# csiro-robotics/syropod_highlevel_controller

Measured on AMD Instinct MI355X. Metric: control-cycles/sec (all legs IK-solved), higher is better.
Workload: dtype f64

## Files before the change

### syropod_highlevel_controller_amd/csrc/shc_cycle.hpp

```cpp
#pragma once

#include "../../include/shc_batch.h"
#include "shc_leg.hpp"

namespace shc {

enum : int { WS_STARTING = 0, WS_MOVING = 1, WS_STOPPING = 2, WS_STOPPED = 3 };
enum : int { SS_SWING = 0, SS_STANCE = 1, SS_FORCE_STANCE = 2, SS_FORCE_STOP = 3 };
enum : int { PS_POSING = 0, PS_STOP_POSING = 1, PS_POSING_COMPLETE = 2 };
enum : int { PM_NONE = 0, PM_SWING = 1, PM_STANCE = 2, PM_STOP = 3 };

constexpr int LW_ACP = 1 << 2, LW_CFS = 1 << 3, LW_PM_SHIFT = 4, LW_NEG = 1 << 6, LW_IKFAIL = 1 << 7, LW_PHASE_SHIFT = 8,
              LW_PHASE_MASK = 0xFFFFF, LW_ZBV = 1 << 28, LW_ATT = 1 << 29, LW_ROTDEF = 1 << 30,
              LW_TARGROT = int(1u << 31);
constexpr int RW_LACP_SHIFT = 2, RW_LCFS_SHIFT = 6, RW_RTDA = 1 << 10, RW_APS_SHIFT = 11;

constexpr int kMaxAutoPosers = 8;
constexpr int kSwingTable = 64;
enum : unsigned { DIRTY_WALK_PLANE = 1, DIRTY_MANUAL = 2, DIRTY_SWING_ORG = 4, DIRTY_STANCE_ORG = 8,
                  DIRTY_TARG_DIR = 16,
                  DIRTY_LAST = DIRTY_TARG_DIR };
enum : unsigned { RT_MANUAL_LIVE = 1, RT_TOUCHDOWN = 2, RT_EXTERNAL = 4, RT_MANUAL_LEGS = 8, RT_EFFORT_LIVE = 16, RT_SKIP_MARKED = 32, RT_POSE_MARKED = 64 };

enum : unsigned { F_MANUAL = 1, F_AUTO = 2, F_INCL = 4, F_IMU = 8, F_ADM = 16, F_TIPF = 32, F_ODOM = 64, F_DYN = 1u << 31,
                  F_ROT = 1u << 30,
                  F_ROUGH = 1u << 29,
                  F_TALIGN = 1u << 28,
                  F_MLEGS = 1u << 27,
                  F_TERRAIN = F_ROUGH | F_TALIGN | F_MLEGS };
template <int NJ, unsigned F>
constexpr bool rot_enabled() { return (F & F_ROT) != 0 && (NJ > 3 || (F & F_MLEGS) != 0); }

struct CycleParams {
  double dt;
  int32_t period, swing_period, stance_period, stance_end, swing_start, swing_end, stance_start;
  int32_t remap_old_period;
  int32_t swing_iterations;
  int32_t stance_iterations;
  double swing_delta_t;
  double inv_dt;
  double dt_over_swing_dt;
  double stance_dt;
  double stride_scale;
  double swing_height, swing_width, body_clearance;
  double swing_progress_scaler;
  int32_t swing_c_count;
  int32_t swing_c_valid;
  int32_t velocity_input_mode;
  int32_t manual_posing, auto_posing, inclination_posing, imu_posing, admittance_control, dynamic_stiffness, use_joint_effort;
  int32_t clamp_joint_positions, clamp_joint_velocities, force_normal_touchdown;
  int32_t tip_force;
  int32_t debug_skip;
  int32_t odometry;
  int32_t gravity_aligned;
  int32_t rough_terrain;
  int32_t tip_align;
  int32_t gravity_target;
  int32_t joint_control;
  double step_depth;
  double target_dir[3];
  double max_translation[3], max_rotation[3], max_translation_velocity, max_rotation_velocity;
  double pid_p, pid_i, pid_d;
  double adm_m00, adm_m01, adm_m10, adm_m11, adm_g0, adm_g1;
  double force_gain, virtual_stiffness, swing_stiffness_scaler, load_stiffness_scaler;
  double pose_force_gain, pose_swing_height;
  int32_t n_auto_posers, pose_phase_length, pose_sync, auto_pose_reference_leg;
  alignas(16) int32_t ap_start[kMaxAutoPosers];
  int32_t ap_end[kMaxAutoPosers];
  double ap_amp[kMaxAutoPosers][7];
};

template <int L, int NJ>
struct alignas(16) SharedConsts {
  LegConst<NJ> leg[L];
  alignas(16) double limit[9][4];
  double swing_c[kSwingTable];
  alignas(16) CycleParams P;
};

template <int NJ>
struct Fields {
  static constexpr int NJE = (NJ + 1) & ~1;
  static constexpr int Q = 0, QD = NJ, TIP = 2 * NJ, TVEL = TIP + 3, SORG = TVEL + 3, SVEL = SORG + 3, TORG = SVEL + 3,
                       DFLT = TORG + 3, TARG = DFLT + 3, STRD = TARG + 3,
                       CORE_END = STRD + 3,
                       ADM = CORE_END, ADM_END = ADM + 2,
                       TF = ADM_END, TF_END = TF + 4,
                       FORCE_IN = TF_END, EFFORT_IN = FORCE_IN + 4,
                       POSER_TIP = EFFORT_IN + NJE, MODEL_TIP = POSER_TIP + 4, ADM_DELTA = MODEL_TIP + 4,
                       ORG_DIR = ADM_DELTA + 4, CUR_DIR = ORG_DIR + 3,
                       TARG_DIR = CUR_DIR + 3,
                       DES_TIP = TARG_DIR + 4, DES_DIR = DES_TIP + 4,
                       SEQ_ORG = DES_DIR + 4, SEQ_DIR = SEQ_ORG + 4, SEQ_Q0 = SEQ_DIR + 4,
                       STEP_PLANE = SEQ_Q0 + NJE,
                       MEAS_Q = STEP_PLANE + 4, COUNT = MEAS_Q + NJE;
  static_assert(CORE_END % 2 == 0 && SORG % 2 == 0 && COUNT % 2 == 0, "field groups must align to 16-byte planes");
};
SHC_HD int64_t leg_field_index(int f, int64_t slot, int64_t n_slots) { return (int64_t(f >> 1) * n_slots + slot) * 2 + (f & 1); }
struct RobotFields {
  static constexpr int VLIN = 0, VANG = 2, PLANE = 3, PNORM = 6, PLANE_PREV = 9, PNORM_PREV = 12, OWPP = 15, VIN = 22, WIN = 24,
                       CORE_END = 25;
  static constexpr int MPOSE = 25, TVI = 32, RVI = 35, MANUAL_END = 38;
  static constexpr int ABSE = 38, VERR = 41, GYRO = 44, IMU_END = 47;
  static constexpr int IMUQ = 47, IMUQ_END = 51;
  static constexpr int APREV = 51, APREV_END = 55;
  static constexpr int CPOSE = 55, CPOSE_END = 62;
  static constexpr int WPP = 62, WPP_END = 69;
  static constexpr int ODOM = 69, ODOM_END = 73;
  static constexpr int INCL = 73, INCL_END = 75;
  static constexpr int TALIGN = 75, OTALIGN = 82, COUNT = 89;
  static constexpr int I_WORD = 0, I_APOSER = 1, I_POSE_PHASE = 2, I_RESET_MODE = 3, I_COUNT = 4;
};

struct ExtFields {
  static constexpr int T_POSE = 0, T_TRANSFORM = 7, T_CLEARANCE = 14, T_FLAGS = 15,
                       D_POSE = 16, D_TRANSFORM = 23, D_FLAGS = 30,
                       P_POSE = 32, P_TRANSFORM = 39, P_CLEARANCE = 46, P_FLAGS = 47, COUNT = 48;
};

enum : int { LS_WALKING = 0, LS_MANUAL = 1, LS_WALKING_TO_MANUAL = -1, LS_MANUAL_TO_WALKING = -2 };
struct ManualRobot {
  int32_t leg_state[SHC_MAX_LEGS];
  int32_t manual_leg_count, primary_leg, secondary_leg;
  int32_t skip_cycle;
  double primary_velocity[3], secondary_velocity[3];
  double primary_position[3], secondary_position[3];
};

struct DevState {
  double *legd;
  int32_t *legi;
  double *robd;
  int32_t *robi;
  int64_t n_slots, n_rob_pad, n_robots;
  double *ext;
  ManualRobot *manual;
  const double *span;
};

struct SpanTable {
  static constexpr int kPlanes = 14;
  static constexpr int kStride = 2 + 2 * kPlanes;
};
SHC_HD double set_precision3(double v) { return round_to_int(v * 1000.0) / 1000.0; }
SHC_HD double stance_span_change_y(const double *table, int leg, double default_shift_z) {
  const double *t = table + leg * SpanTable::kStride;
  const int n = int(t[0]);
  const double target = set_precision3(default_shift_z);
  int lower = -1, upper = -1;
  for (int k = 0; k < n; ++k) {
    const double h = t[2 + 2 * k];
    if (h > target && (upper < 0 || h < t[2 + 2 * upper])) upper = k;
    if (h <= target && (lower < 0 || h > t[2 + 2 * lower])) lower = k;
  }
  if (lower < 0 || upper < 0) return 0.0;
  const double uh = set_precision3(t[2 + 2 * upper]), lh = set_precision3(t[2 + 2 * lower]);
  const double i = (target - lh) / (uh - lh);
  const double radius = t[3 + 2 * lower] * (1.0 - i) + t[3 + 2 * upper] * i;
  return radius * t[1];
}

#if defined(__HIPCC__)

template <int L, int NJ, unsigned F>
constexpr bool phase_fences() {
#if defined(SHC_FENCE)
  return true;
#else
  constexpr bool exact = (F & (0x80000000u  | 0x40000000u )) == 0;
  constexpr bool octo_tipf = L == 8 && NJ == 5 && (F & 32u ) != 0 && (F & 16u ) == 0;
  return exact && ((NJ == 4 && (L == 4 || L == 8)) || octo_tipf);
#endif
}
#define SHC_PHASE_FENCE() do { if constexpr (phase_fences<L, NJ, F>()) __builtin_amdgcn_sched_barrier(0); } while (0)
#if defined(SHC_RES2_TIMING) && !defined(SHC_RES2_BUSY_ONLY)
__shared__ long long shc_ticks_lds[96];
__shared__ long long shc_acc_lds[96];
#define SHC_TICK(i) do { __builtin_amdgcn_sched_barrier(0); if (blockIdx.x == 1 && (threadIdx.x & 127) == 0) shc_ticks_lds[(threadIdx.x >> 7) * 32 + (i)] = __builtin_readcyclecounter(); __builtin_amdgcn_sched_barrier(0); } while (0)
#else
#define SHC_TICK(i) do {} while (0)
#endif
#ifdef SHC_ABLATE
#define SHC_DBG(P) ((P).debug_skip)
#else
#define SHC_DBG(P) 0
#endif
__device__ __forceinline__ int uni(int v) { return __builtin_amdgcn_readfirstlane(v); }

template <unsigned F>
struct Feat {
  __device__ __forceinline__ static bool manual(const CycleParams &P) { return (F & F_DYN) ? P.manual_posing != 0 : (F & F_MANUAL) != 0; }
  __device__ __forceinline__ static bool autop(const CycleParams &P) { return (F & F_DYN) ? P.auto_posing != 0 : (F & F_AUTO) != 0; }
  __device__ __forceinline__ static bool incl(const CycleParams &P) { return (F & F_DYN) ? P.inclination_posing != 0 : (F & F_INCL) != 0; }
  __device__ __forceinline__ static bool imu(const CycleParams &P) { return (F & F_DYN) ? P.imu_posing != 0 : (F & F_IMU) != 0; }
  __device__ __forceinline__ static bool adm(const CycleParams &P) { return (F & F_DYN) ? P.admittance_control != 0 : (F & F_ADM) != 0; }
  __device__ __forceinline__ static bool tipf(const CycleParams &P) { return (F & F_DYN) ? P.tip_force != 0 : (F & F_TIPF) != 0; }
  __device__ __forceinline__ static bool odom(const CycleParams &P) { return (F & F_DYN) ? P.odometry != 0 : (F & F_ODOM) != 0; }
};

template <int L>
struct Group {
  int base;
  __device__ __forceinline__ int get(int v, int j) const { return __shfl(v, base + j, 64); }
  __device__ __forceinline__ double get(double v, int j) const { return __shfl(v, base + j, 64); }
  __device__ __forceinline__ double sum(double v) const {
    double s = 0.0;
#pragma unroll
    for (int j = 0; j < L; ++j) s += get(v, j);
    return s;
  }
};

template <int RPW>
struct RobTile {
  double *d;
  int32_t *i;
  int grp;
  __device__ __forceinline__ double get(int f) const { return d[f * RPW + grp]; }
  __device__ __forceinline__ V3 get3(int f) const { return V3{d[f * RPW + grp], d[(f + 1) * RPW + grp], d[(f + 2) * RPW + grp]}; }
  __device__ __forceinline__ Quat getq(int f) const {
    return Quat{d[f * RPW + grp], d[(f + 1) * RPW + grp], d[(f + 2) * RPW + grp], d[(f + 3) * RPW + grp]};
  }
  __device__ __forceinline__ Pose getpose(int f) const { return Pose{get3(f), getq(f + 3)}; }
  __device__ __forceinline__ void put(int f, double v) const { d[f * RPW + grp] = v; }
  __device__ __forceinline__ void put3(int f, V3 v) const {
    d[f * RPW + grp] = v.x;
    d[(f + 1) * RPW + grp] = v.y;
    d[(f + 2) * RPW + grp] = v.z;
  }
  __device__ __forceinline__ void putq(int f, Quat q) const {
    d[f * RPW + grp] = q.w;
    d[(f + 1) * RPW + grp] = q.x;
    d[(f + 2) * RPW + grp] = q.y;
    d[(f + 3) * RPW + grp] = q.z;
  }
  __device__ __forceinline__ void putpose(int f, const Pose &p) const {
    put3(f, p.p);
    putq(f + 3, p.r);
  }
  __device__ __forceinline__ int geti(int f) const { return i[f * RPW + grp]; }
  __device__ __forceinline__ void puti(int f, int v) const { i[f * RPW + grp] = v; }
};

template <int NJ>
struct LegRegs {
  static constexpr bool kKeepJacobian = NJ <= 3;
  double q[NJ], qd[NJ];
  double sn[NJ], cs[NJ];
  V3 lin[NJ], pe;
  V3 tip, tvel, targ, strd;
  double adm0, adm1;
  double stiff;
  V3 tf, tipx;
  V3 org_dir, cur_dir, targ_dir;
  int word;
};

enum : int { PK_SORG = 0, PK_SVEL = 3, PK_TORG = 6, PK_DFLT = 9, PK_COUNT = 12 };
#ifndef SHC_PARK_REGS
struct Park {
  double *d;
  int lane;
  __device__ __forceinline__ V3 get3(int f) const { return V3{d[f * 64 + lane], d[(f + 1) * 64 + lane], d[(f + 2) * 64 + lane]}; }
  __device__ __forceinline__ void put3(int f, V3 v) const {
    d[f * 64 + lane] = v.x;
    d[(f + 1) * 64 + lane] = v.y;
    d[(f + 2) * 64 + lane] = v.z;
  }
  __device__ __forceinline__ double at(int k) const { return d[k * 64 + lane]; }
  __device__ __forceinline__ void set(int k, double v) const { d[k * 64 + lane] = v; }
};
#else
struct Park {
  double *d;
  int lane;
  mutable double r[12];
  __device__ __forceinline__ V3 get3(int f) const { return V3{r[f], r[f + 1], r[f + 2]}; }
  __device__ __forceinline__ void put3(int f, V3 v) const { r[f] = v.x, r[f + 1] = v.y, r[f + 2] = v.z; }
  __device__ __forceinline__ double at(int k) const { return r[k]; }
  __device__ __forceinline__ void set(int k, double v) const { r[k] = v; }
};
#endif

__device__ __forceinline__ V3 external_default(const double *ext, int64_t ns, uint32_t slot, V3 terrain_following) {
  if (ext == nullptr) return terrain_following;
  const double2 *X = reinterpret_cast<const double2 *>(ext);
  if ((int(X[(ExtFields::D_FLAGS / 2) * ns + slot].x) & 1) == 0) return terrain_following;
  double v[14];
#pragma unroll
  for (int k = 0; k < 7; ++k) {
    const double2 d = X[(ExtFields::D_POSE / 2 + k) * ns + slot];
    v[2 * k] = d.x, v[2 * k + 1] = d.y;
  }
  return V3{v[0], v[1], v[2]} + rotate(Quat{v[3], v[4], v[5], v[6]}, -V3{v[7], v[8], v[9]});
}

struct LegOut {
  V3 poser_tip, model_tip, adm_delta;
};

__device__ __forceinline__ double swing_progress_of(int word, const CycleParams &P) {
  int pm = (word >> LW_PM_SHIFT) & 3;
  if (pm != PM_SWING) return -1.0;
  int phase = (word >> LW_PHASE_SHIFT) & LW_PHASE_MASK;
  return clampd(double(phase - P.swing_start + 1) / double(P.swing_end - P.swing_start), 0.0, 1.0);
}

__device__ __forceinline__ int bearing_bracket(double y, double x) {
  if (x == 0.0 && y == 0.0) return 0;
  constexpr double kC = 0.99996192306417128874, kS = 0.0087265354983739347;
  double xr = kC * x - kS * y, yr = kS * x + kC * y;
  double ax = fabs(xr), ay = fabs(yr);
  bool upper = yr > 0.0 || (yr == 0.0 && xr > 0.0);
  if (upper) return xr > 0.0 ? (ay < ax ? 0 : 1) : (ay > ax ? 2 : 3);
  return xr < 0.0 ? (ay < ax ? 4 : 5) : (ay > ax ? 6 : 7);
}

template <int NJ>
struct LegInPlanes {
  const double *legd;
  int64_t ns;
  uint32_t slot;
  __device__ __forceinline__ V3 force() const {
    const double2 f01 = reinterpret_cast<const double2 *>(legd)[(Fields<NJ>::FORCE_IN / 2) * ns + slot];
    const double2 f2_ = reinterpret_cast<const double2 *>(legd)[(Fields<NJ>::FORCE_IN / 2 + 1) * ns + slot];
    return V3{f01.x, f01.y, f2_.x};
  }
  __device__ __forceinline__ void effort(double (&e)[NJ]) const {
#pragma unroll
    for (int i = 0; i < NJ; i += 2) {
      const double2 e2 = reinterpret_cast<const double2 *>(legd)[((Fields<NJ>::EFFORT_IN + i) / 2) * ns + slot];
      e[i] = e2.x;
      if (i + 1 < NJ) e[i + 1] = e2.y;
    }
  }
};
struct NoHook {
  __device__ __forceinline__ void operator()() const {}
};

struct UniFlags {
  int clamp_joint_velocities, clamp_joint_positions, swing_c_count;
  int velocity_input_mode, force_normal_touchdown;
};
__device__ __forceinline__ UniFlags load_uni_flags(const CycleParams &P) {
  const int c = P.clamp_joint_velocities, d = P.clamp_joint_positions, e = P.swing_c_count;
  const int f = P.velocity_input_mode, h = P.force_normal_touchdown;
  return UniFlags{uni(c), uni(d), uni(e), uni(f), uni(h)};
}

struct FrontToBack {
  V3 desired_dir;
  bool rot_def;
  int my_leg_state;
  bool plane_prev_changed;
  bool pose_only;
  V3 odom_vel;
  bool odom_run;
  bool joint_moved;
  V3 held_pe, held_dir;
  bool planes_in_sync = false;
  UniFlags uf;
  int limit_bracket = -1;
  double limit_value[4] = {0.0, 0.0, 0.0, 0.0};
};

struct OdomCache {
  double ha = 0.0, sh = 0.0, ch = 1.0;
  bool valid = false;
};
__device__ __forceinline__ void odometry_advance(double &ox, double &oy, double &ow, double &oz, const CycleParams &P, double vx, double vy, double vw,
                                                 OdomCache *cache = nullptr) {
  double sh, ch;
  const double ha = 0.5 * (vw * P.dt);
  if (cache != nullptr && cache->valid && __all(ha == cache->ha)) {
    sh = cache->sh, ch = cache->ch;
  } else {
    if (__all(fabs(ha) <= 0.5)) sincos_joint<false>(ha, &sh, &ch);
    else sincos_joint(ha, &sh, &ch);
    if (cache != nullptr) cache->ha = ha, cache->sh = sh, cache->ch = ch, cache->valid = true;
  }
  {
#pragma clang fp contract(off)
    const double a = vx * P.dt, b = vy * P.dt;
    double ux = -(oz * b), uy = oz * a;
    ux = ux + ux;
    uy = uy + uy;
    const double nx = ox + fma(-oz, uy, fma(ux, ow, a)), ny = oy + fma(oz, ux, fma(uy, ow, b));
    const double nw = fma(ow, ch, -(oz * sh)), nz = fma(ow, sh, oz * ch);
    ox = nx, oy = ny, ow = nw, oz = nz;
  }
}
template <int RPW>
__device__ __forceinline__ void odometry_step(const RobTile<RPW> &rb, const CycleParams &P, double vx, double vy, double vw, OdomCache *cache = nullptr) {
  using R = RobotFields;
  double ox = rb.get(R::ODOM), oy = rb.get(R::ODOM + 1), ow = rb.get(R::ODOM + 2), oz = rb.get(R::ODOM + 3);
  odometry_advance(ox, oy, ow, oz, P, vx, vy, vw, cache);
  rb.put(R::ODOM, ox);
  rb.put(R::ODOM + 1, oy);
  rb.put(R::ODOM + 2, ow);
  rb.put(R::ODOM + 3, oz);
}

template <int L, int NJ>
__device__ __forceinline__ double walk_plane_control_input(const int own_word, const SharedConsts<L, NJ> &C, const CycleParams &P, const Group<L> g,
                                                           const int swing_c_count_u) {
  double c = 0.0;
  bool sel = false;
  if (swing_c_count_u > 0) {
    const int it_own = min(max(((own_word >> LW_PHASE_SHIFT) & LW_PHASE_MASK) - P.swing_start, 0), P.swing_c_count - 1);
    const bool ok_own = ((own_word >> LW_PM_SHIFT) & 3) == PM_SWING && it_own < P.swing_c_valid;
    const unsigned legs_ok = unsigned((__ballot(ok_own) >> g.base) & ((1ull << L) - 1));
    sel = legs_ok != 0;
    const int last = sel ? 31 - __clz(int(legs_ok)) : 0;
    int it_sel = g.get(it_own, last);
    it_sel = sel ? it_sel : 0;
    if (__any(sel)) c = sel ? C.swing_c[it_sel] : 0.0;
  } else {
    double c_own = -1.0;
    const double sp = swing_progress_of(own_word, P) * P.swing_progress_scaler;
    if (sp >= 0 && sp <= 1.0) c_own = smooth_step(sp);
#pragma unroll
    for (int j = 0; j < L; ++j) {
      const double cj = g.get(c_own, j);
      if (cj >= 0.0) {
        c = cj;
        sel = true;
      }
    }
  }
  return sel ? c : -1.0;
}

template <int L, int NJ>
__device__ __forceinline__ double walk_plane_control_candidate(const int own_word, const SharedConsts<L, NJ> &C, const CycleParams &P, const int swing_c_count_u) {
  if (swing_c_count_u > 0) {
    const int it_own = min(max(((own_word >> LW_PHASE_SHIFT) & LW_PHASE_MASK) - P.swing_start, 0), P.swing_c_count - 1);
    const bool ok_own = ((own_word >> LW_PM_SHIFT) & 3) == PM_SWING && it_own < P.swing_c_valid;
    const double c = C.swing_c[it_own];
    return ok_own ? c : -1.0;
  }
  const double sp = swing_progress_of(own_word, P) * P.swing_progress_scaler;
  return (sp >= 0 && sp <= 1.0) ? smooth_step(sp) : -1.0;
}

template <int L>
__device__ __forceinline__ V3 quat_to_euler_zyx_grouped(Quat q, const Group<L> g, const int leg) {
  static_assert(L >= 3, "three lanes per robot");
  double tx = 2.0 * q.x, ty = 2.0 * q.y, tz = 2.0 * q.z;
  double twx = tx * q.w, twy = ty * q.w, twz = tz * q.w;
  double txx = tx * q.x, txy = ty * q.x, txz = tz * q.x;
  double tyy = ty * q.y, tyz = tz * q.y, tzz = tz * q.z;
  double m00 = 1.0 - (tyy + tzz), m01 = txy - twz, m02 = txz + twy;
  double m10 = txy + twz, m11 = 1.0 - (txx + tzz), m12 = tyz - twx;
  double m20 = txz - twy, m21 = tyz + twx, m22 = 1.0 - (txx + tyy);
  const double c2 = sqrt(m22 * m22 + m21 * m21);
  const bool neg = m10 < 0.0 || (m10 == 0.0 && __builtin_signbit(m10) && __builtin_signbit(m00));
  const bool second = leg == 1;
  const double t = atan2(second ? -m20 : m10, second ? (neg ? -c2 : c2) : m00);
  double r0 = g.get(t, 0), r1 = g.get(t, 1);
  if (__builtin_expect(__any((r0 < 0.0) != neg), 0)) r1 = atan2(-m20, r0 < 0.0 ? -c2 : c2);
  if (r0 < 0.0) r0 += kPi;
  double s1, c1;
  sincos_joint(r0, &s1, &c1);
  double r2 = atan2(s1 * m02 - c1 * m12, c1 * m11 - s1 * m01);
  if (fabs(r1) > kPi / 2 || fabs(r2) > kPi / 2) {
    r0 -= kPi;
    if (r1 > kPi / 2.0) r1 = -r1 + kPi;
    else if (r1 < kPi / 2.0) r1 = -r1 - kPi;
    if (r2 > kPi / 2.0) r2 -= kPi;
    else if (r2 < kPi / 2.0) r2 += kPi;
  }
  return V3{r2, r1, r0};
}
template <int L>
__device__ __forceinline__ Quat euler_to_quat_zyx_grouped(V3 e, const Group<L> g, const int leg) {
  static_assert(L >= 3, "three lanes per robot");
  double sn, cs;
  sincos_joint(0.5 * (leg == 0 ? e.x : (leg == 1 ? e.y : e.z)), &sn, &cs);
  const double sx = g.get(sn, 0), cx = g.get(cs, 0), sy = g.get(sn, 1), cy = g.get(cs, 1), sz = g.get(sn, 2), cz = g.get(cs, 2);
  Quat qx{cx, sx, 0, 0}, qy{cy, 0, sy, 0}, qz{cz, 0, 0, sz};
  return (qz * qy) * qx;
}

template <int L, int NJ, unsigned F, bool OWN_WORD = false>
__device__ __forceinline__ Pose cycle_pose(LegRegs<NJ> &s, const SharedConsts<L, NJ> &C, const CycleParams &P, const LegConst<NJ> &lc, const RobTile<64 / L> &rb,
                                           const Group<L> g, const int leg, const int (&lw)[L], int &rword, const int walk_state, unsigned &dirty, const bool manual_live,
                                           Pose &auto_pose, Pose &leg_auto, const V3 plane_prev, const V3 pnorm_prev, const int swing_c_count_u,
                                           const int own_word = 0, Pose *owpp_cache = nullptr, const double *c_given = nullptr) {
  static_assert(!OWN_WORD || ((F & (F_DYN | F_AUTO | F_TALIGN)) == 0), "the other legs' words are needed by auto posing and the tip-align pose");
  using R = RobotFields;
  using FT = Feat<F>;
  const V3 UZ{0, 0, 1};
  Pose cp;
  {
    Pose wpp;
    {
      double c = 0.0;
      bool sel = false;
      if constexpr (OWN_WORD) {
        const double ce = c_given != nullptr ? *c_given : walk_plane_control_input<L, NJ>(own_word, C, P, g, swing_c_count_u);
        sel = ce >= 0.0;
        c = sel ? ce : 0.0;
      } else if (swing_c_count_u > 0) {
        int it_sel = 0;
#pragma unroll
        for (int j = 0; j < L; ++j) {
          const int it = min(max(((lw[j] >> LW_PHASE_SHIFT) & LW_PHASE_MASK) - P.swing_start, 0), P.swing_c_count - 1);
          const bool ok = ((lw[j] >> LW_PM_SHIFT) & 3) == PM_SWING && it < P.swing_c_valid;
          it_sel = ok ? it : it_sel;
          sel = sel || ok;
        }
        if (__any(sel)) c = sel ? C.swing_c[it_sel] : 0.0;
      } else {
        double c_own = -1.0;
        {
          double sp = swing_progress_of(s.word, P) * P.swing_progress_scaler;
          if (sp >= 0 && sp <= 1.0) c_own = smooth_step(sp);
        }
#pragma unroll
        for (int j = 0; j < L; ++j) {
          double cj = g.get(c_own, j);
          if (cj >= 0.0) {
            c = cj;
            sel = true;
          }
        }
      }
      V3 wplane = sel ? plane_prev : V3{0, 0, 0};
      V3 wnorm = sel ? pnorm_prev : UZ;
      Pose owpp = owpp_cache != nullptr ? *owpp_cache : rb.getpose(R::OWPP);
      bool flat = wnorm.x == 0.0 && wnorm.y == 0.0 && wnorm.z == 1.0 && owpp.r.w == 1.0 && owpp.r.x == 0.0 && owpp.r.y == 0.0 &&
                  owpp.r.z == 0.0;
      if (__builtin_expect(__all(flat), 1)) {
        double s0 = 1.0 - c;
        V3 npp{0.0, 0.0, P.body_clearance + wplane.z};
        wpp.p = npp * c + owpp.p * s0;
        wpp.r = Quat{s0 * 1.0 + c * 1.0, s0 * 0.0 + c * 0.0, s0 * 0.0 + c * 0.0, s0 * 0.0 + c * 0.0};
      } else {
        Pose np;
        np.r = correct_rotation(from_two_vectors(UZ, wnorm), quat_identity());
        np.p = rotate(np.r, V3{0, 0, P.body_clearance});
        np.p.z += wplane.z;
        wpp = interpolate_pose(owpp, c, np);
      }
      if (c == 1.0) {
        const bool same = wpp.p.x == owpp.p.x && wpp.p.y == owpp.p.y && wpp.p.z == owpp.p.z && wpp.r.w == owpp.r.w && wpp.r.x == owpp.r.x &&
                          wpp.r.y == owpp.r.y && wpp.r.z == owpp.r.z;
        if (__any(!same)) {
          rb.putpose(R::OWPP, wpp);
          if (owpp_cache != nullptr) *owpp_cache = wpp;
          dirty |= DIRTY_WALK_PLANE;
        }
      }
      rb.putpose(R::WPP, wpp);
    }
    cp = wpp;
    Quat manual_r = quat_identity();
    if (FT::manual(P) && manual_live) {
      V3 tvi_in = rb.get3(R::TVI), rvi_in = rb.get3(R::RVI);
      int reset_mode = rb.geti(R::I_RESET_MODE);
      bool idle = reset_mode == 0 && tvi_in.x == 0.0 && tvi_in.y == 0.0 && tvi_in.z == 0.0 && rvi_in.x == 0.0 && rvi_in.y == 0.0 &&
                  rvi_in.z == 0.0;
      Pose mpose = rb.getpose(R::MPOSE);
      if (__any(!idle)) {
        if (!idle) {
          if (reset_mode == 5) {
            mpose = pose_identity();
          } else {
            double cpos[3] = {mpose.p.x, mpose.p.y, mpose.p.z};
            V3 ce = quat_to_euler(mpose.r, true);
            double crot[3] = {ce.x, ce.y, ce.z};
            double tvi[3] = {tvi_in.x, tvi_in.y, tvi_in.z}, rvi[3] = {rvi_in.x, rvi_in.y, rvi_in.z};
            bool rt[3] = {false, false, false}, rr[3] = {false, false, false};
            switch (reset_mode) {
              case 1: rt[2] = true; rr[2] = true; break;
              case 2: rt[0] = true; rt[1] = true; break;
              case 3: rr[0] = true; rr[1] = true; break;
              case 4: rt[0] = rt[1] = rt[2] = true; rr[0] = rr[1] = rr[2] = true; break;
              default: break;
            }
            double dpos[3], drot[3];
#pragma unroll
            for (int i = 0; i < 3; ++i) {
#pragma clang fp contract(off)
              if (rt[i]) {
                double diff = cpos[i] - 0.0;
                if (diff < 0) tvi[i] = 1.0; else if (diff > 0) tvi[i] = -1.0;
              }
              if (rr[i]) {
                double diff = crot[i] - 0.0;
                if (diff < 0) rvi[i] = 1.0; else if (diff > 0) rvi[i] = -1.0;
              }
              double tv = tvi[i] * P.max_translation_velocity;
              double rv = rvi[i] * P.max_rotation_velocity;
              double dp = cpos[i] + tv * P.dt;
              double dr = crot[i] + rv * P.dt;
              double tl = signd(tv) * P.max_translation[i];
              if (rt[i] && 0.0 < P.max_translation[i] && 0.0 > -P.max_translation[i]) tl = 0.0;
              bool ptv = signd(tv) > 0;
              if ((ptv && dp > tl) || (!ptv && dp < tl)) tv = (tl - cpos[i]) / P.dt;
              double rl = signd(rv) * P.max_rotation[i];
              if (rr[i] && 0.0 < P.max_rotation[i] && 0.0 > -P.max_rotation[i]) rl = 0.0;
              bool prv = signd(rv) > 0;
              if ((prv && dr > rl) || (!prv && dr < rl)) rv = (rl - crot[i]) / P.dt;
              dpos[i] = cpos[i] + tv * P.dt;
              drot[i] = crot[i] + rv * P.dt;
            }
            rb.put3(R::TVI, V3{tvi[0], tvi[1], tvi[2]});
            rb.put3(R::RVI, V3{rvi[0], rvi[1], rvi[2]});
            mpose.p = V3{dpos[0], dpos[1], dpos[2]};
            mpose.r = correct_rotation(euler_to_quat(V3{drot[0], drot[1], drot[2]}, true), quat_identity());
          }
          rb.putpose(R::MPOSE, mpose);
        }
        dirty |= DIRTY_MANUAL;
      }
      manual_r = mpose.r;
      bool unposed = mpose.p.x == 0.0 && mpose.p.y == 0.0 && mpose.p.z == 0.0 && mpose.r.w == 1.0 && mpose.r.x == 0.0 &&
                     mpose.r.y == 0.0 && mpose.r.z == 0.0;
      if (!__all(unposed)) cp = add_pose(cp, mpose);
    }
    if (FT::incl(P)) {
      Quat aprev = FT::autop(P) ? rb.getq(R::APREV) : quat_identity();
      Quat comb = normalized(manual_r * aprev);
      Quat removed = normalized(rb.getq(R::IMUQ) * inverse(comb));
      V3 e = quat_to_euler(removed, false);
      double lon = clampd(-P.body_clearance * tan(e.y), -P.max_translation[0], P.max_translation[0]);
      double lat = clampd(P.body_clearance * tan(e.x), -P.max_translation[1], P.max_translation[1]);
      cp = add_pose(cp, Pose{V3{lon, lat, 0.0}, quat_identity()});
      if ((F & F_MLEGS) != 0) {
        rb.put(R::INCL, lon);
        rb.put(R::INCL + 1, lat);
      }
    }
    if (FT::imu(P)) {
      Quat cur = correct_rotation(rb.getq(R::IMUQ), quat_identity());
      Quat tgt = correct_rotation(manual_r, quat_identity());
#ifdef SHC_POSE_R5
      Quat err = normalized(cur * inverse(tgt));
#else
      const double tgt_n2 = dot(tgt, tgt);
      Quat err = normalized(cur * (__all(tgt_n2 == 1.0) ? conj(tgt) : inverse(tgt)));
#endif
#ifdef SHC_POSE_R5
      V3 pe = quat_to_euler(err, false);
#else
      V3 pe = quat_to_euler_zyx_grouped<L>(err, g, leg);
#endif
      pe.z = 0.0;
      V3 abse = rb.get3(R::ABSE) + pe * P.dt;
      V3 verr = (-rb.get3(R::GYRO)) * 0.15 + rb.get3(R::VERR) * (1 - 0.15);
      rb.put3(R::ABSE, abse);
      rb.put3(R::VERR, verr);
      V3 corr = -(verr * P.pid_d + pe * P.pid_p + abse * P.pid_i);
      corr.x = clampd(corr.x, -P.max_rotation[0], P.max_rotation[0]);
      corr.y = clampd(corr.y, -P.max_rotation[1], P.max_rotation[1]);
      bool tgt_identity = tgt.w == 1.0 && tgt.x == 0.0 && tgt.y == 0.0 && tgt.z == 0.0;
      corr.z = 0.0;
      if (__any(!tgt_identity)) {
        if (!tgt_identity) corr.z = quat_to_euler(tgt, false).z;
      }
#ifdef SHC_POSE_R5
      Quat ir = correct_rotation(euler_to_quat(corr, false), tgt);
#else
      Quat ir = correct_rotation(euler_to_quat_zyx_grouped<L>(corr, g, leg), tgt);
#endif
      cp = add_pose(cp, Pose{V3{0, 0, 0}, ir});
    } else if (FT::autop(P)) {
      int ref = lw[P.auto_pose_reference_leg];
      bool zbv = (ref & LW_ZBV) != 0;
      int aps = (rword >> RW_APS_SHIFT) & 3;
      if (walk_state == WS_STARTING || walk_state == WS_MOVING) aps = PS_POSING;
      else if ((zbv && walk_state == WS_STOPPING) || walk_state == WS_STOPPED) aps = PS_STOP_POSING;
      int master_phase;
      if (P.pose_sync) {
        master_phase = (ref >> LW_PHASE_SHIFT) & LW_PHASE_MASK;
        rb.puti(R::I_POSE_PHASE, master_phase);
      } else {
        master_phase = rb.geti(R::I_POSE_PHASE);
        rb.puti(R::I_POSE_PHASE, (master_phase + 1) % P.pose_phase_length);
      }
      int aposer = rb.geti(R::I_APOSER);
      int complete = 0;
      for (int i = 0; i < P.n_auto_posers; ++i) {
        int fl = (aposer >> (4 * i)) & 15;
        bool start_check = fl & 1, end1 = fl & 2, end2 = fl & 4, allow = fl & 8;
        int phase = master_phase, sp = P.ap_start[i], ep = P.ap_end[i];
        if (sp > ep) {
          ep += P.pose_phase_length;
          if (phase < sp) phase += P.pose_phase_length;
        }
        start_check = !P.pose_sync || (!start_check && aps == PS_POSING && phase == sp);
        end1 = end1 || (aps == PS_STOP_POSING && phase == sp);
        end2 = end2 || (aps == PS_STOP_POSING && phase == ep && end1);
        if (!allow && start_check) {
          allow = true;
          end1 = end2 = false;
        } else if (allow && P.pose_sync && end1 && end2) {
          allow = false;
          start_check = false;
        }
        aposer = (aposer & ~(15 << (4 * i))) | ((int(start_check) | int(end1) << 1 | int(end2) << 2 | int(allow) << 3) << (4 * i));
        complete += allow ? 0 : 1;
        if (phase >= sp && phase < ep && allow) {
          int iteration = phase - sp + 1, num = ep - sp;
          bool first_half = iteration <= num / 2;
          double delta_t = 1.0 / (num / 2.0);
          int offset = int(first_half ? 0 : num / 2.0);
          double t = (iteration - offset) * delta_t;
          double u = 1.0 - t;
          double wgt = first_half ? (4.0 * t * t * t * u + t * t * t * t) : (u * u * u * u + 4.0 * t * u * u * u);
          V3 pos;
          if (P.ap_amp[i][3] != 0.0) {
            V3 e = quat_to_euler(rb.getq(R::IMUQ), false);
            V3 gv{0, 0, kGravity};
            gv = rotate(angle_axis_y(-e.y), gv);
            gv = rotate(angle_axis_x(-e.x), gv);
            pos = normalized(gv) * (P.ap_amp[i][3] * wgt);
          } else {
            pos = V3{P.ap_amp[i][0] * wgt, P.ap_amp[i][1] * wgt, P.ap_amp[i][2] * wgt};
          }
          V3 rot{P.ap_amp[i][4] * wgt, P.ap_amp[i][5] * wgt, P.ap_amp[i][6] * wgt};
          auto_pose = add_pose(auto_pose, Pose{pos, euler_to_quat(rot, false)});
        }
      }
      rb.puti(R::I_APOSER, aposer);
      if (complete == P.n_auto_posers) aps = PS_POSING_COMPLETE;
      rword = (rword & ~(3 << RW_APS_SHIFT)) | (aps << RW_APS_SHIFT);
      {
        int sp = lc.neg_start, ep = lc.neg_end, np = master_phase;
        if (sp > ep) {
          ep += P.pose_phase_length;
          if (np < sp) np += P.pose_phase_length;
        }
        int st = s.word & 3;
        bool neg = (s.word & LW_NEG) != 0;
        if (st != SS_FORCE_STANCE && st != SS_FORCE_STOP && np == sp) neg = true;
        if (np < sp || np > ep) neg = false;
        s.word = neg ? (s.word | LW_NEG) : (s.word & ~LW_NEG);
        leg_auto = auto_pose;
        if (neg) {
          int iteration = np - sp + 1, num = ep - sp;
          bool first_half = iteration <= num / 2;
          double ci = 1.0;
          if (lc.neg_ratio > 0.0) {
            if (first_half) ci = fmin(1.0, iteration / (num * lc.neg_ratio));
            else ci = fmin(1.0, (num - iteration) / (num * lc.neg_ratio));
          }
          ci = smooth_step(ci);
          Pose negation = interpolate_pose(pose_identity(), ci, auto_pose);
          leg_auto = remove_pose(auto_pose, negation);
        }
      }
      cp = add_pose(cp, auto_pose);
      if (FT::incl(P)) rb.putq(R::APREV, auto_pose.r);
    }
    if ((F & F_TALIGN) != 0 && uni(P.tip_align)) {
      Chain<NJ> ch0;
      chain_from_sincos<NJ>(lc, s.sn, s.cs, ch0);
      V3 last_joint = ch0.p[NJ - 1];
      if constexpr (NJ > 3) {
#pragma unroll
        for (int k = NJ - 2; k >= 2; --k) last_joint = lc.jactive[k + 1] != 0.0 ? last_joint : ch0.p[k];
      }
      const V3 t2j_own = base_rotate(lc, last_joint - ch0.pe);
      Pose ta = rb.getpose(R::TALIGN), ota = rb.getpose(R::OTALIGN);
      const V3 n = pnorm_prev;
      const Quat wrot = from_two_vectors(UZ, n);
#pragma unroll
      for (int j = 0; j < L; ++j) {
        const V3 t2j{g.get(t2j_own.x, j), g.get(t2j_own.y, j), g.get(t2j_own.z, j)};
        const double sp = swing_progress_of(lw[j], P);
        if (sp != -1.0) {
          const double link_length = norm(-t2j);
          V3 a = rotate(wrot, t2j), b = n * link_length;
          const V3 to_alignment = -(a - b * (dot(a, b) / dot(b, b)));
          a = ta.p;
          b = n;
          V3 target = (a - b * (dot(a, b) / dot(b, b))) + to_alignment;
          target.x = clampd(target.x, -P.max_translation[0], P.max_translation[1]);
          target.y = clampd(target.y, -P.max_translation[1], P.max_translation[1]);
          target.z = clampd(target.z, -P.max_translation[2], P.max_translation[1]);
          double c = smooth_step(sp);
          if (sp < 0.5) {
            c = smooth_step(c * 2.0);
            ta = interpolate_pose(ota, c, pose_identity());
          } else {
            c = smooth_step((c - 0.5) * 2.0);
            ta = interpolate_pose(pose_identity(), c, Pose{target, quat_identity()});
          }
          if (sp == 1.0) ota = ta;
        }
      }
      rb.putpose(R::TALIGN, ta);
      rb.putpose(R::OTALIGN, ota);
      cp = add_pose(cp, ta);
    }
    rb.putpose(R::CPOSE, cp);
  }
  return cp;
}

template <int NJ, typename IN>
__device__ __forceinline__ void cycle_admittance(LegRegs<NJ> &s, LegOut &out, const CycleParams &P, const IN &in) {
  const V3 force_in = in.force();
  V3 f = (P.use_joint_effort ? s.tf : force_in) * P.pose_force_gain;
  double fi[3] = {f.x, f.y, f.z}, d[3];
#pragma unroll
  for (int i = 0; i < 3; ++i) {
    double u = fmax(fi[i], 0.0);
    double x0 = P.adm_m00 * s.adm0 + P.adm_m01 * s.adm1 + P.adm_g0 * u;
    double x1 = P.adm_m10 * s.adm0 + P.adm_m11 * s.adm1 + P.adm_g1 * u;
    s.adm0 = x0;
    s.adm1 = x1;
    d[i] = clampd(-x0, -0.2, 0.2);
  }
  out.adm_delta = projection(V3{d[0], d[1], d[2]}, s.tipx);
}

template <int L, int NJ, unsigned F, bool ADM_HERE, typename IN, bool ODOM_HERE = true, bool POSE_HERE = true, typename POSEWAIT = NoHook>
__device__ __forceinline__ void cycle_front(LegRegs<NJ> &s, LegOut &out, const SharedConsts<L, NJ> &C, const RobTile<64 / L> &rb, const Park &pk,
                                            const Group<L> g, int leg, const double *__restrict__ legd, int64_t ns, uint32_t slot, unsigned &dirty,
                                            const bool manual_live, const bool touchdown_detection, double *ext, const ManualRobot *mr, const IN &in,
                                            FrontToBack &fb, const double *span = nullptr, const POSEWAIT &pose_wait = POSEWAIT()) {
  using R = RobotFields;
  using FT = Feat<F>;
  static_assert(POSE_HERE || ((F & F_DYN) == 0 && (F & F_AUTO) == 0 && (F & F_TERRAIN) == 0), "the pose can run elsewhere only without auto posing / terrain paths");
  int zero = 0;
  asm volatile("" : "+v"(zero));
  const CycleParams &P = (&C.P)[zero];
  const LegConst<NJ> &lc = C.leg[leg + zero];
  const V3 UZ{0, 0, 1};
  constexpr bool rot_on = rot_enabled<NJ, F>();
  constexpr bool rot_walk = rot_on && NJ > 3;
  bool rot_def = (s.word & LW_ROTDEF) != 0;
  bool targ_rot = (s.word & LW_TARGROT) != 0;
  fb.odom_run = false;
  fb.plane_prev_changed = false;
  fb.joint_moved = false;
  SHC_TICK(2);

  int rword = rb.geti(R::I_WORD);
  int walk_state = rword & 3;
  const double vin_x = rb.get(R::VIN), vin_y = rb.get(R::VIN + 1), win = rb.get(R::WIN);
  bool may_stop = walk_state == WS_STOPPING;
  if (walk_state == WS_MOVING) {
    const double ax = fabs(vin_x), ay = fabs(vin_y), aw = win;
    may_stop = !(aw != 0.0 || ax > 1e-100 || ay > 1e-100);
  }
  s.word &= ~(LW_ZBV | LW_ATT);
  if (!(SHC_DBG(P) & 128) && __any(may_stop)) {
    int w = s.word;
    if (dot(s.strd, s.strd) == 0.0) w |= LW_ZBV;
    const V3 pnp = rb.get3(R::PNORM_PREV);
    V3 err = s.tip - s.targ;
    if (__all(pnp.x == 0.0 && pnp.y == 0.0 && pnp.z == 1.0)) err.z = 0.0;
    else err = rejection(err, pnp);
    if (dot(err, err) < kTipTolerance * kTipTolerance) w |= LW_ATT;
    s.word = w;
  }
  int lw[L];
  const bool lw_early = POSE_HERE || uni(FT::adm(P) ? 1 : 0) != 0;
  if (lw_early) {
#pragma unroll
    for (int j = 0; j < L; ++j) lw[j] = g.get(s.word, j);
  } else {
#pragma unroll
    for (int j = 0; j < L; ++j) lw[j] = 0;
  }

  SHC_PHASE_FENCE();
  SHC_TICK(3);
  int my_leg_state = LS_WALKING;
  bool frozen = false;
  if ((F & F_MLEGS) != 0 && mr != nullptr) {
    my_leg_state = mr->leg_state[leg];
#pragma unroll
    for (int j = 0; j < L; ++j) frozen = frozen || g.get(my_leg_state, j) != LS_WALKING;
  }

  Pose cp;
  Pose auto_pose = pose_identity();
  Pose leg_auto = pose_identity();
  if (POSE_HERE && !(SHC_DBG(P) & 1)) {
    cp = cycle_pose<L, NJ, F>(s, C, P, lc, rb, g, leg, lw, rword, walk_state, dirty, manual_live, auto_pose, leg_auto, rb.get3(R::PLANE_PREV), rb.get3(R::PNORM_PREV),
                              fb.uf.swing_c_count);
  } else if (POSE_HERE) {
    cp = rb.getpose(R::CPOSE);
  }
  SHC_PHASE_FENCE();
  SHC_TICK(4);
  int pose_state = (rword >> RW_APS_SHIFT) & 3;

  out.adm_delta = V3{0, 0, 0};
  if (FT::adm(P)) {
    if (uni(P.dynamic_stiffness) && walk_state != WS_STOPPED) {
      const bool swing = (s.word & 3) == SS_SWING;
      const double k = P.virtual_stiffness;
      const double ref = fabs((s.tip.z - pk.get3(PK_DFLT).z) / P.pose_swing_height);
      const double load = swing ? k * (ref * (P.load_stiffness_scaler - 1)) : 0.0;
      double v = swing ? k * (ref * (P.swing_stiffness_scaler - 1) + 1) : k;
      const int lo = leg == 0 ? L - 1 : leg - 1, hi = leg == L - 1 ? 0 : leg + 1;
#pragma unroll
      for (int i = 0; i < L; ++i) {
        const double li = g.get(load, i);
        const bool si = (lw[i] & 3) == SS_SWING;
        if (si && (i == lo || i == hi) && (!swing || i > leg)) v += li;
      }
      s.stiff = v;
    }
    if (ADM_HERE) cycle_admittance<NJ>(s, out, P, in);
  }
  if ((F & F_MLEGS) != 0 && fb.pose_only) {
    rb.puti(R::I_WORD, rword);
    return;
  }

  SHC_PHASE_FENCE();
  double lim[4] = {0.05, 0.3, 0.02, 0.1};
  if (!(SHC_DBG(P) & 2)) {
    double sx = vin_x + win * (-s.tip.y), sy = vin_y + win * s.tip.x;
    int idx = bearing_bracket(sy, sx);
    if (__all(idx == fb.limit_bracket)) {
#pragma unroll
      for (int k = 0; k < 4; ++k) lim[k] = fb.limit_value[k];
    } else {
#pragma unroll
      for (int k = 0; k < 4; ++k) lim[k] = kUnassigned;
#pragma unroll
      for (int j = 0; j < L; ++j) {
        int ij = g.get(idx, j);
#pragma unroll
        for (int k = 0; k < 4; ++k) lim[k] = fmin(lim[k], C.limit[ij][k]);
      }
      fb.limit_bracket = idx;
#pragma unroll
      for (int k = 0; k < 4; ++k) fb.limit_value[k] = lim[k];
    }
  }
  SHC_PHASE_FENCE();
  SHC_TICK(5);
  double vx = rb.get(R::VLIN), vy = rb.get(R::VLIN + 1), vw = rb.get(R::VANG);
  const double lin_n2 = vin_x * vin_x + vin_y * vin_y;
  double lin_norm;
  const int velocity_input_mode = fb.uf.velocity_input_mode;
  if (velocity_input_mode == 0 && __all(lin_n2 <= 1.0)) lin_norm = lin_n2 != 0.0 ? 0.5 : 0.0;
  else lin_norm = sqrt(lin_n2);
  if (!(SHC_DBG(P) & 32)) {
    double nvx, nvy, nw;
    if (velocity_input_mode == 0) {
      double k = 1.0;
      if (__any(lin_norm > 1.0)) k = lin_norm > 1.0 ? 1.0 / lin_norm : 1.0;
      const double cx = lin_norm > 1.0 ? vin_x * k : vin_x, cy = lin_norm > 1.0 ? vin_y * k : vin_y;
      nw = clampd(win, -1.0, 1.0) * lim[1];
      const double sc = 1.0 - fabs(win);
      nvx = (cx * lim[0]) * sc;
      nvy = (cy * lim[0]) * sc;
    } else {
      const bool over = lin_norm > lim[0];
      const double k = lim[0] / lin_norm;
      const double cx = over ? vin_x * k : vin_x, cy = over ? vin_y * k : vin_y;
      nw = clampd(win, -lim[1], lim[1]);
      const double sc = lim[1] != 0.0 ? (1.0 - fabs(nw / lim[1])) : 0.0;
      nvx = cx * sc;
      nvy = cy * sc;
    }
    if (walk_state == WS_STOPPING) nvx = nvy = nw = 0.0;
    if (frozen) nvx = vx, nvy = vy, nw = vw;
    const double ax = nvx - vx, ay = nvy - vy;
    const double an2 = ax * ax + ay * ay;
    const double an = __all(an2 == 0.0) ? 0.0 : sqrt(an2);
    const double cap = lim[2] * P.dt;
    if (__all(an < cap)) {
      vx += ax;
      vy += ay;
    } else {
      const double inv = an2 > 0.0 ? an : 1.0;
      const double sx_ = (ax / inv) * lim[2] * P.dt, sy_ = (ay / inv) * lim[2] * P.dt;
      vx += an < cap ? ax : sx_;
      vy += an < cap ? ay : sy_;
    }
    const double aa = nw - vw;
    vw += fabs(aa) < lim[3] * P.dt ? aa : signd(aa) * lim[3] * P.dt;
    rb.put(R::VLIN, vx);
    rb.put(R::VLIN + 1, vy);
    rb.put(R::VANG, vw);
  }
  const bool has_cmd = (lin_norm != 0.0) || (win != 0.0);

  SHC_PHASE_FENCE();
  SHC_TICK(6);
  if constexpr ((F & F_DYN) != 0) {
    const int remap_from = uni(P.remap_old_period);
    if (remap_from > 0) {
      if (walk_state == WS_MOVING) {
        int ph = (s.word >> LW_PHASE_SHIFT) & LW_PHASE_MASK, st = s.word & 3;
        const double step_progress = double(ph) / double(remap_from);
        ph = int(step_progress * double(P.period));
        if (st != SS_FORCE_STOP) {
          if (ph >= P.swing_start && ph < P.swing_end && st != SS_FORCE_STANCE) st = SS_SWING;
          else if (ph < P.stance_end || ph >= P.stance_start) st = SS_STANCE;
        }
        s.word = (s.word & ~(3 | (LW_PHASE_MASK << LW_PHASE_SHIFT))) | st | (ph << LW_PHASE_SHIFT);
      }
      if (lw_early) {
#pragma unroll
        for (int j = 0; j < L; ++j) lw[j] = g.get(s.word, j);
      }
    }
  }
  int lacp = (rword >> RW_LACP_SHIFT) & 15, lcfs = (rword >> RW_LCFS_SHIFT) & 15;
  bool rtda = (rword & RW_RTDA) != 0;
  bool early_return = false;
  int my_state = s.word & 3, my_phase = (s.word >> LW_PHASE_SHIFT) & LW_PHASE_MASK;
  bool my_acp = (s.word & LW_ACP) != 0, my_cfs = (s.word & LW_CFS) != 0;
  bool my_update_default = false;
  bool any_stepping = false;
  const bool steady = __all(!frozen && walk_state == WS_MOVING && has_cmd) && !(SHC_DBG(P) & 16384);
  if (steady) {
    my_acp = false;
    any_stepping = ((__ballot((s.word & 3) != SS_FORCE_STOP) >> g.base) & ((1ull << L) - 1)) != 0;
  } else if (SHC_DBG(P) & 16384) {
    my_acp = false;
    any_stepping = true;
  } else if (frozen) {
    early_return = true;
  } else if (walk_state == WS_STOPPED && has_cmd) {
    walk_state = WS_STARTING;
    my_acp = false;
    my_cfs = false;
    my_phase = lc.phase_offset;
    my_state = SS_STANCE;
    if (my_phase >= P.swing_start && my_phase < P.swing_end) my_state = SS_SWING;
    early_return = true;
  } else {
    if (walk_state == WS_STARTING && lacp == L && lcfs == L) {
      lacp = 0;
      lcfs = 0;
      walk_state = WS_MOVING;
    } else if (walk_state == WS_MOVING && !has_cmd) {
      walk_state = WS_STOPPING;
    } else if (walk_state == WS_STOPPING && lacp == L && pose_state == PS_POSING_COMPLETE) {
      lacp = 0;
      walk_state = WS_STOPPED;
    }
    if (__all(walk_state == WS_MOVING)) {
      my_acp = false;
      any_stepping = ((__ballot((s.word & 3) != SS_FORCE_STOP) >> g.base) & ((1ull << L) - 1)) != 0;
    } else {
    if (!lw_early) {
#pragma unroll
      for (int j = 0; j < L; ++j) lw[j] = g.get(s.word, j);
    }
#pragma unroll
    for (int j = 0; j < L; ++j) {
      int wj = lw[j];
      int st = wj & 3, ph = (wj >> LW_PHASE_SHIFT) & LW_PHASE_MASK;
      bool acp = (wj & LW_ACP) != 0, cfs = (wj & LW_CFS) != 0, upd = false;
      if (walk_state == WS_STARTING) {
        if (lacp == L) {
          if (ph == P.swing_end && !cfs) {
            cfs = true;
            lcfs++;
          }
        }
        if (!acp) {
          if (C.leg[j].starts_in_swing && ph != P.swing_end) {
            st = SS_FORCE_STANCE;
          } else {
            lacp++;
            acp = true;
          }
        }
      } else if (walk_state == WS_MOVING) {
        acp = false;
      } else if (walk_state == WS_STOPPING) {
        if ((wj & LW_ZBV) && !acp && ph == P.swing_end) {
          if ((wj & LW_ATT) || rtda) {
            rtda = false;
            upd = true;
            st = SS_FORCE_STOP;
            acp = true;
            lacp++;
          } else {
            rtda = true;
          }
        }
      } else {
        st = SS_FORCE_STOP;
        ph = 0;
      }
      any_stepping = any_stepping || (st != SS_FORCE_STOP);
      if (j == leg) {
        my_state = st;
        my_phase = ph;
        my_acp = acp;
        my_cfs = cfs;
        my_update_default = upd;
      }
    }
    }
  }
  if (POSE_HERE || !steady) {
    rword = (rword & ~(3 | (15 << RW_LACP_SHIFT) | (15 << RW_LCFS_SHIFT) | RW_RTDA)) | walk_state | (lacp << RW_LACP_SHIFT) |
            (lcfs << RW_LCFS_SHIFT) | (rtda ? RW_RTDA : 0);
    rb.puti(R::I_WORD, rword);
  }
  SHC_TICK(7);
  int my_pm = (s.word >> LW_PM_SHIFT) & 3;
  SHC_PHASE_FENCE();

  if (!early_return) {
    bool default_changed = false;
    if (__any(my_update_default)) {
      if (my_update_default) {
        if (!POSE_HERE) pose_wait();
        Pose wpp = rb.getpose(R::WPP);
        const double span_y = ((F & F_ROUGH) != 0 && span != nullptr) ? stance_span_change_y(span, leg, pk.get3(PK_DFLT).z) : lc.span_shift;
        V3 idp = transform_vector(wpp, V3{lc.stance_x, lc.stance_y + span_y, 0.0});
        V3 proj = projection(pk.get3(PK_TORG) - idp, rb.get3(R::PNORM_PREV));
        pk.put3(PK_DFLT, external_default(ext, ns, slot, idp + proj));
        default_changed = true;
        dirty |= DIRTY_STANCE_ORG;
      }
    }
    bool standard = (my_state == SS_SWING) || my_cfs;
    int msp = standard ? P.stance_period : lc.first_stance_period;
    int stance_iter = standard ? P.stance_iterations : lc.first_stance_iterations;
    int mss = standard ? P.stance_start : lc.phase_offset;
    double stance_dt = standard ? P.stance_dt : lc.first_stance_dt;
    (void)stance_iter;
    const V3 dflt = pk.get3(PK_DFLT);
    s.targ = dflt + s.strd * 0.5;
    bool stepping = my_state != SS_FORCE_STOP;
    const bool rough = (F & F_ROUGH) != 0 && uni(P.rough_terrain) != 0;
    bool rough_update_default = false;
    V3 model_tip_prev{0, 0, 0};
    if (rough) {
      if (LegRegs<NJ>::kKeepJacobian) {
        model_tip_prev = tip_robot_frame(lc, s.pe);
      } else {
        Chain<NJ> ch0;
        chain_from_sincos<NJ>(lc, s.sn, s.cs, ch0);
        model_tip_prev = tip_robot_frame(lc, ch0.pe);
      }
    }
    const int force_normal_touchdown = fb.uf.force_normal_touchdown;
#ifdef SHC_NO_STRAIGHT
    const bool straight = false;
#else
    const bool straight = (F & F_ROUGH) == 0 && !(SHC_DBG(P) & 4) && force_normal_touchdown == 0;
#endif
    if (straight) {
      const V3 sorg_p = pk.get3(PK_SORG), svel_p = pk.get3(PK_SVEL), torg_p = pk.get3(PK_TORG);
      const bool swing = my_state == SS_SWING;
      const bool step_sw = stepping && swing, step_st = stepping && !swing;
      const V3 sv{vx - vw * s.tip.y, vy + vw * s.tip.x, 0.0};
      const V3 strd_new = scaled(sv, P.stride_scale);
      s.strd = sel3(stepping, strd_new, s.strd);
      V3 pn = rb.get3(R::PNORM);
      const bool flat_n = pn.x == 0.0 && pn.y == 0.0 && pn.z == 1.0;
      if (!__all(flat_n)) pn = normalized(pn);
      const V3 clearance = scaled(pn, P.swing_height);
      const int it_sw = my_phase - P.swing_start + 1;
      const bool first_half = it_sw <= P.swing_iterations / 2;
      const bool first_sw = step_sw && it_sw == 1;
      const V3 sorg = sel3(first_sw, s.tip, sorg_p), svel = sel3(first_sw, s.tvel, svel_p);
      pk.put3(PK_SORG, sorg);
      pk.put3(PK_SVEL, svel);
      dirty |= first_sw ? unsigned(DIRTY_SWING_ORG) : 0u;
      V3 mid{(sorg.x + s.targ.x) / 2.0, (sorg.y + s.targ.y) / 2.0, fmax(sorg.z, s.targ.z)};
      mid = mid + clearance;
      mid.y += (lc.stance_y > 0.0) ? P.swing_width : -P.swing_width;
      const V3 sep1 = scaled(svel * 0.25, P.dt_over_swing_dt);
      const V3 n1_0 = sorg, n1_1 = sorg + sep1, n1_2 = sorg + scaled(sep1, 2.0);
      const V3 n1_3{(mid.x + n1_2.x) / 2.0, (mid.y + n1_2.y) / 2.0, mid.z};
      const V3 n1_4 = mid;
      const V3 fv = scaled(-s.strd, stance_dt * P.inv_dt);
      const V3 sep2 = scaled(fv * 0.25, P.dt_over_swing_dt);
      const V3 n2_0 = n1_4, n2_1 = n1_4 - (n1_3 - n1_4), n2_2 = s.targ - scaled(sep2, 2.0), n2_3 = s.targ - sep2, n2_4 = s.targ;
      const double t_sw = first_half ? P.swing_delta_t * it_sw : P.swing_delta_t * (it_sw - P.swing_iterations / 2);
      const V3 b0 = sel3(first_half, n1_0, n2_0), b1 = sel3(first_half, n1_1, n2_1), b2 = sel3(first_half, n1_2, n2_2), b3 = sel3(first_half, n1_3, n2_3),
               b4 = sel3(first_half, n1_4, n2_4);
      const V3 dpos_sw = scaled(quartic_bezier_dot(b0, b1, b2, b3, b4, t_sw), P.swing_delta_t);
      int it_st = my_phase + (P.period - mss);
      if (it_st >= P.period) it_st -= P.period;
      if (it_st < 0 || it_st >= P.period) it_st = mod_i(it_st, P.period);
      it_st += 1;
      const bool first_st = step_st && it_st == 1;
      const V3 torg = sel3(first_st, s.tip, torg_p);
      pk.put3(PK_TORG, torg);
      dirty |= first_st ? unsigned(DIRTY_STANCE_ORG) : 0u;
      const double stride_scaler = standard ? 1.0 : lc.first_stride_scaler;
      const V3 sep = scaled((-s.strd) * stride_scaler, 0.25);
      const double t_st = it_st * stance_dt;
      const V3 dpos_st = scaled(quartic_bezier_dot(torg, torg + sep, torg + scaled(sep, 2.0), torg + scaled(sep, 3.0), torg + scaled(sep, 4.0), t_st), stance_dt);
      const V3 dpos = sel3(swing, dpos_sw, dpos_st);
      const V3 tip_new = s.tip + dpos, tvel_new = dpos * P.inv_dt;
      s.tip = sel3(stepping, tip_new, s.tip);
      s.tvel = sel3(stepping, tvel_new, s.tvel);
    } else if (stepping && !(SHC_DBG(P) & 4)) {
      V3 sv{vx - vw * s.tip.y, vy + vw * s.tip.x, 0.0};
      s.strd = scaled(sv, P.stride_scale);
      V3 pn = rb.get3(R::PNORM);
      bool flat_n = pn.x == 0.0 && pn.y == 0.0 && pn.z == 1.0;
      if (!__all(flat_n)) pn = normalized(pn);
      V3 clearance = scaled(pn, P.swing_height);
      V3 dpos;
      if (my_state == SS_SWING) {
        int iteration = my_phase - P.swing_start + 1;
        bool first_half = iteration <= P.swing_iterations / 2;
        V3 sorg, svel;
        if (iteration == 1) {
          sorg = s.tip;
          svel = s.tvel;
          pk.put3(PK_SORG, sorg);
          pk.put3(PK_SVEL, svel);
          dirty |= DIRTY_SWING_ORG;
          rough_update_default = rough;
        } else {
          sorg = pk.get3(PK_SORG);
          svel = pk.get3(PK_SVEL);
        }
        bool ground_contact = false;
        if (rough) {
          const double2 sp01 = reinterpret_cast<const double2 *>(legd)[(Fields<NJ>::STEP_PLANE / 2) * ns + slot];
          const double2 sp23 = reinterpret_cast<const double2 *>(legd)[(Fields<NJ>::STEP_PLANE / 2 + 1) * ns + slot];
          ground_contact = sp23.y != 0.0;
          bool external = false;
          if (ext != nullptr) {
            const double2 *X = reinterpret_cast<const double2 *>(ext);
            const double2 cf = X[(ExtFields::T_CLEARANCE / 2) * ns + slot];
            const int flags = int(cf.y);
            external = (flags & 1) != 0;
            if (external) {
              double v[14];
#pragma unroll
              for (int k = 0; k < 7; ++k) {
                const double2 d = X[(ExtFields::T_POSE / 2 + k) * ns + slot];
                v[2 * k] = d.x, v[2 * k + 1] = d.y;
              }
              s.targ = V3{v[0], v[1], v[2]} + rotate(Quat{v[3], v[4], v[5], v[6]}, -V3{v[7], v[8], v[9]});
              if (rot_walk) {
                const Quat tr = Quat{v[3], v[4], v[5], v[6]} * inverse(Quat{v[10], v[11], v[12], v[13]});
                targ_rot = !(tr.w == 0.0 && tr.x == 0.0 && tr.y == 0.0 && tr.z == 0.0);
                if (targ_rot) s.targ_dir = rotate(tr, V3{1, 0, 0}), dirty |= DIRTY_TARG_DIR;
              }
              clearance = normalized(clearance) * cf.x;
              if (flags & 2) {
                const double time_to_swing_end = (P.swing_iterations - iteration) * P.dt;
                s.targ = s.targ - V3{vx, vy, 0.0} * time_to_swing_end;
              }
            }
          }
          if (external) {
          } else if (touchdown_detection) {
            if (ground_contact) {
              const V3 step_plane_position = V3{sp01.x, sp01.y, sp23.x} - model_tip_prev;
              const V3 difference = (s.tip + step_plane_position) - s.targ;
              s.targ = s.targ + projection(difference, rb.get3(R::PNORM));
            } else {
              s.targ.z -= P.step_depth;
            }
          }
        }
        V3 mid{(sorg.x + s.targ.x) / 2.0, (sorg.y + s.targ.y) / 2.0, fmax(sorg.z, s.targ.z)};
        mid = mid + clearance;
        mid.y += (lc.stance_y > 0.0) ? P.swing_width : -P.swing_width;
        V3 sep1 = scaled(svel * 0.25, P.dt_over_swing_dt);
        V3 n1_0 = sorg, n1_1 = sorg + sep1, n1_2 = sorg + scaled(sep1, 2.0);
        V3 n1_3{(mid.x + n1_2.x) / 2.0, (mid.y + n1_2.y) / 2.0, mid.z};
        V3 n1_4 = mid;
        V3 fv = scaled(-s.strd, stance_dt * P.inv_dt);
        V3 sep2 = scaled(fv * 0.25, P.dt_over_swing_dt);
        V3 n2_0 = n1_4, n2_1 = n1_4 - (n1_3 - n1_4), n2_2 = s.targ - scaled(sep2, 2.0), n2_3 = s.targ - sep2, n2_4 = s.targ;
        if (rough && ground_contact && !first_half) {
          n2_0 = s.tip, n2_1 = s.tip + sep2, n2_2 = s.tip + scaled(sep2, 2.0), n2_3 = s.tip + scaled(sep2, 3.0), n2_4 = s.tip + scaled(sep2, 4.0);
        }
        if (force_normal_touchdown && !(rough && ground_contact)) {
          V3 bo = s.targ - scaled(sep2, 4.0);
          bo.z = fmax(sorg.z, s.targ.z);
          bo = bo + clearance;
          n1_4 = bo;
          n2_0 = bo;
          n2_2 = s.targ - scaled(sep2, 2.0);
          V3 half = scaled(n2_2 - bo, 0.5);
          n1_3 = n2_0 - half;
          n2_1 = n2_0 + half;
        }
        if (first_half) {
          double t = P.swing_delta_t * iteration;
          dpos = scaled(quartic_bezier_dot(n1_0, n1_1, n1_2, n1_3, n1_4, t), P.swing_delta_t);
        } else {
          double t = P.swing_delta_t * (iteration - P.swing_iterations / 2);
          dpos = scaled(quartic_bezier_dot(n2_0, n2_1, n2_2, n2_3, n2_4, t), P.swing_delta_t);
        }
      } else {
        int iteration = my_phase + (P.period - mss);
        if (iteration >= P.period) iteration -= P.period;
        if (iteration < 0 || iteration >= P.period) iteration = mod_i(iteration, P.period);
        iteration += 1;
        V3 torg;
        if (iteration == 1) {
          torg = s.tip;
          pk.put3(PK_TORG, torg);
          dirty |= DIRTY_STANCE_ORG;
          rough_update_default = rough;
          if (ext != nullptr) {
            double &flags = ext[((ExtFields::T_CLEARANCE / 2) * ns + slot) * 2 + 1];
            flags = double(int(flags) & ~1);
          }
        } else {
          torg = pk.get3(PK_TORG);
        }
        double stride_scaler = standard ? 1.0 : lc.first_stride_scaler;
        (void)msp;
        V3 sep = scaled((-s.strd) * stride_scaler, 0.25);
        double t = iteration * stance_dt;
        dpos = scaled(quartic_bezier_dot(torg, torg + sep, torg + scaled(sep, 2.0), torg + scaled(sep, 3.0), torg + scaled(sep, 4.0), t), stance_dt);
      }
      s.tip = s.tip + dpos;
      s.tvel = dpos * P.inv_dt;
      if (rough && __any(rough_update_default)) {
        if (rough_update_default) {
          if (!POSE_HERE) pose_wait();
          Pose wpp = rb.getpose(R::WPP);
          const double span_y = span != nullptr ? stance_span_change_y(span, leg, pk.get3(PK_DFLT).z) : 0.0;
          V3 idp = transform_vector(wpp, V3{lc.stance_x, lc.stance_y + span_y, 0.0});
          V3 proj = projection(pk.get3(PK_TORG) - idp, rb.get3(R::PNORM));
          V3 new_default = external_default(ext, ns, slot, idp + proj);
          pk.put3(PK_DFLT, new_default);
          default_changed = true;
          dirty |= DIRTY_STANCE_ORG;
        }
      }
    }
    SHC_TICK(16);
    if (rot_on) {
      const int pm0 = (s.word >> LW_PM_SHIFT) & 3;
      const double sp = swing_progress_of(s.word, P);
      bool more_than_3_joints = NJ > 3;
      if constexpr (NJ > 3) more_than_3_joints = lc.jactive[3] != 0.0;
      if (rot_walk && more_than_3_joints && (pm0 == PM_STANCE || pm0 == PM_STOP || sp >= 0.5)) {
        if (uni(P.gravity_target) && !targ_rot) {
          V3 gv{0, 0, kGravity};
          if (FT::imu(P) || FT::incl(P) || FT::autop(P)) {
            const V3 e = quat_to_euler(rb.getq(R::IMUQ), false);
            gv = rotate(angle_axis_y(-e.y), gv);
            gv = rotate(angle_axis_x(-e.x), gv);
          }
          s.targ_dir = normalized(gv);
          dirty |= DIRTY_TARG_DIR;
          targ_rot = true;
        }
        if (!targ_rot) {
          rot_def = false;
        } else {
          s.cur_dir = s.targ_dir;
          if (sp >= 0.5) {
            const double c = smooth_step(fmin(1.0, 2.0 * (sp - 0.5)));
            s.cur_dir = normalized(lerp3(s.org_dir, s.targ_dir, c));
          }
          rot_def = true;
        }
      } else {
        s.org_dir = s.tipx;
        rot_def = false;
      }
    }
    my_phase = my_phase + 1 == P.period ? 0 : my_phase + 1;
    if (my_phase > P.period) my_phase = my_phase % P.period;
    if (my_state != SS_FORCE_STOP) {
      if (my_phase >= P.swing_start && my_phase < P.swing_end && my_state != SS_FORCE_STANCE) my_state = SS_SWING;
      else if (my_phase < P.stance_end || my_phase >= P.stance_start) my_state = SS_STANCE;
    }
    if (my_state == SS_SWING) my_pm = PM_SWING;
    else if (my_state == SS_STANCE) my_pm = PM_STANCE;
    else if (my_state == SS_FORCE_STOP) my_pm = PM_STOP;
    if (!fb.planes_in_sync) {
      const V3 pl = rb.get3(R::PLANE), pn_ = rb.get3(R::PNORM), plp = rb.get3(R::PLANE_PREV), pnp_ = rb.get3(R::PNORM_PREV);
      const bool same = pl.x == plp.x && pl.y == plp.y && pl.z == plp.z && pn_.x == pnp_.x && pn_.y == pnp_.y && pn_.z == pnp_.z;
      if (any_stepping) {
        if (__any(!same)) {
          rb.put3(R::PLANE_PREV, pl);
          rb.put3(R::PNORM_PREV, pn_);
          dirty |= DIRTY_WALK_PLANE;
          fb.plane_prev_changed = true;
        }
      }
      fb.planes_in_sync = __all(same || any_stepping);
    }
    if (__any(default_changed)) {
      fb.planes_in_sync = false;
      dirty |= DIRTY_WALK_PLANE;
      const V3 nd = pk.get3(PK_DFLT);
      double x = nd.x, y = nd.y, z = nd.z;
      double sxx = g.sum(x * x), sxy = g.sum(x * y), sx = g.sum(x), syy = g.sum(y * y), sy = g.sum(y);
      double sxz = g.sum(x * z), syz = g.sum(y * z), sz = g.sum(z);
      double a00 = sxx, a01 = sxy, a02 = sx, a11 = syy, a12 = sy, a22 = double(L);
      double c00 = a11 * a22 - a12 * a12, c01 = a02 * a12 - a01 * a22, c02 = a01 * a12 - a02 * a11;
      double c11 = a00 * a22 - a02 * a02, c12 = a01 * a02 - a00 * a12, c22 = a00 * a11 - a01 * a01;
      double det = a00 * c00 + a01 * c01 + a02 * c02;
      double pa = (c00 * sxz + c01 * syz + c02 * sz) / det;
      double pb = (c01 * sxz + c11 * syz + c12 * sz) / det;
      double pc = (c02 * sxz + c12 * syz + c22 * sz) / det;
      rb.put3(R::PLANE, V3{pa, pb, pc});
      rb.put3(R::PNORM, normalized(V3{-pa, -pb, 1.0}));
    }
    if (FT::odom(P) && !(SHC_DBG(P) & 1024)) {
      if (ODOM_HERE) odometry_step(rb, P, vx, vy, vw);
      fb.odom_vel = V3{vx, vy, vw};
      fb.odom_run = true;
    }
  }
  if ((F & F_MLEGS) != 0 && mr != nullptr && my_leg_state == LS_MANUAL) {
    const bool primary = leg == mr->primary_leg, secondary = !primary && leg == mr->secondary_leg;
    V3 vin{0, 0, 0}, pin{0, 0, 0};
    if (primary) {
      vin = V3{mr->primary_velocity[0], mr->primary_velocity[1], mr->primary_velocity[2]};
      pin = V3{mr->primary_position[0], mr->primary_position[1], mr->primary_position[2]};
    } else if (secondary) {
      vin = V3{mr->secondary_velocity[0], mr->secondary_velocity[1], mr->secondary_velocity[2]};
      pin = V3{mr->secondary_position[0], mr->secondary_position[1], mr->secondary_position[2]};
    }
    if (norm(vin) != 0.0 && uni(P.joint_control) != 0) {
      bool three_joints = NJ == 3;
      if constexpr (NJ > 3) three_joints = lc.jactive[3] == 0.0;
      if constexpr (rot_on) if (three_joints) {
        Chain<NJ> ch;
        chain_from_sincos<NJ>(lc, s.sn, s.cs, ch);
        fb.joint_moved = true;
        fb.held_pe = ch.pe;
        fb.held_dir = s.tipx;
        s.q[0] += vin.y * P.max_rotation_velocity * P.dt;
        s.q[2] += vin.x * P.max_rotation_velocity * P.dt;
        joint_sincos<NJ>(lc, s.q, s.sn, s.cs);
        chain_from_sincos<NJ>(lc, s.sn, s.cs, ch);
        s.tip = tip_robot_frame(lc, ch.pe);
        s.cur_dir = base_rotate(lc, ch.xe);
        rot_def = true;
      }
    } else if (norm(vin) != 0.0) {
      V3 prev_tip;
      if (LegRegs<NJ>::kKeepJacobian) {
        prev_tip = tip_robot_frame(lc, s.pe);
      } else {
        Chain<NJ> ch0;
        chain_from_sincos<NJ>(lc, s.sn, s.cs, ch0);
        prev_tip = tip_robot_frame(lc, ch0.pe);
      }
      const double2 d01 = reinterpret_cast<const double2 *>(legd)[(Fields<NJ>::DES_TIP / 2) * ns + slot];
      const double2 d23 = reinterpret_cast<const double2 *>(legd)[(Fields<NJ>::DES_TIP / 2 + 1) * ns + slot];
      const V3 ik_error = V3{d01.x, d01.y, d23.x} - prev_tip;
      V3 change = vin * (P.max_translation_velocity * P.dt);
      if (norm(ik_error) >= kIkTolerance) change = (-normalized(ik_error)) * norm(change);
      s.tip = s.tip + change;
      rot_def = false;
    }
    if (norm(pin) != 0.0 && uni(P.joint_control) == 0) {
      s.tip = pin;
      rot_def = false;
    }
  }
  s.word = (s.word & ~(3 | LW_ACP | LW_CFS | (3 << LW_PM_SHIFT) | (LW_PHASE_MASK << LW_PHASE_SHIFT) | LW_ZBV | LW_ATT | LW_IKFAIL | LW_ROTDEF | LW_TARGROT)) |
           my_state | (my_acp ? LW_ACP : 0) | (my_cfs ? LW_CFS : 0) | (my_pm << LW_PM_SHIFT) | (my_phase << LW_PHASE_SHIFT) |
           (rot_def ? LW_ROTDEF : 0) | (targ_rot ? LW_TARGROT : 0);

  SHC_PHASE_FENCE();
  SHC_TICK(8);
  V3 desired_dir{1, 0, 0};
  {
    if (!POSE_HERE && !(SHC_DBG(P) & 32768)) {
      pose_wait();
      SHC_TICK(17);
      cp = rb.getpose(R::CPOSE);
    } else if (!POSE_HERE) {
      cp = pose_identity();
    }
    Pose bp = cp;
    if (FT::autop(P) && !FT::imu(P)) {
      bp = remove_pose(bp, auto_pose);
      bp = add_pose(bp, leg_auto);
    }
    out.poser_tip = (SHC_DBG(P) & 256) ? s.tip : inverse_transform_vector(bp, s.tip);
    if ((F & F_MLEGS) != 0 && (my_leg_state == LS_MANUAL || my_leg_state == LS_WALKING_TO_MANUAL)) out.poser_tip = s.tip;
    if (rot_on && rot_def) desired_dir = rotate(inverse(bp.r), s.cur_dir);
    if (rot_on && rot_def && (F & F_MLEGS) != 0 && (my_leg_state == LS_MANUAL || my_leg_state == LS_WALKING_TO_MANUAL)) desired_dir = s.cur_dir;
  }

  fb.desired_dir = desired_dir;
  fb.rot_def = rot_def;
  fb.my_leg_state = my_leg_state;
  SHC_PHASE_FENCE();
  SHC_TICK(15);
}

template <int L, int NJ, unsigned F, typename IN>
__device__ __forceinline__ void cycle_back(LegRegs<NJ> &s, LegOut &out, const SharedConsts<L, NJ> &C, int leg, const double *__restrict__ legd, int64_t ns,
                                           uint32_t slot, const ManualRobot *mr, const IN &in, const FrontToBack &fb) {
  using FT = Feat<F>;
  int zero = 0;
  asm volatile("" : "+v"(zero));
  const CycleParams &P = (&C.P)[zero];
  const LegConst<NJ> &lc = C.leg[leg + zero];
  constexpr bool rot_on = rot_enabled<NJ, F>();
  const V3 desired_dir = fb.desired_dir;
  const bool rot_def = fb.rot_def;
  const int my_leg_state = fb.my_leg_state;
  {
    SHC_TICK(9);
    V3 desired = out.poser_tip + out.adm_delta;
    if ((F & F_MLEGS) != 0 && (my_leg_state == LS_MANUAL || my_leg_state == LS_WALKING_TO_MANUAL))
      desired = out.poser_tip;
    if ((F & F_MLEGS) != 0 && mr != nullptr) {
      double *dd = const_cast<double *>(legd);
      reinterpret_cast<double2 *>(dd)[(Fields<NJ>::DES_TIP / 2) * ns + slot] = double2{desired.x, desired.y};
      dd[((Fields<NJ>::DES_TIP / 2 + 1) * ns + slot) * 2] = desired.z;
    }
    Chain<NJ> chain;
    bool retried = false;
    if (rot_on) {
      const bool cv = fb.uf.clamp_joint_velocities != 0, cp_ = fb.uf.clamp_joint_positions != 0;
      chain_from_sincos<NJ>(lc, s.sn, s.cs, chain);
      V3 current_dir = chain.xe;
      double dq[NJ];
      V3 lin[NJ];
      if ((F & F_MLEGS) != 0 && fb.joint_moved) {
        current_dir = base_rotate_inv(lc, fb.held_dir);
        jacobian_columns<NJ>(chain, lin);
        ik_step_cols<NJ>(lc, lin, fb.held_pe, s.q, s.qd, desired, dq);
      } else {
        ik_step<NJ>(lc, chain, s.q, s.qd, desired, dq);
      }
      if (rot_def) {
        update_joints<NJ>(lc, dq, P.dt, P.inv_dt, false, cp_, s.q, s.qd);
        joint_sincos<NJ>(lc, s.q, s.sn, s.cs);
        chain_from_sincos<NJ>(lc, s.sn, s.cs, chain);
        jacobian_columns<NJ>(chain, lin);
        ik_step_rotation<NJ>(lc, chain, lin, s.q, s.qd, tip_rotation_delta(current_dir, base_rotate_inv(lc, desired_dir)), dq);
      }
      double success = update_joints<NJ>(lc, dq, P.dt, P.inv_dt, cv, cp_, s.q, s.qd);
      joint_sincos<NJ>(lc, s.q, s.sn, s.cs);
      chain_from_sincos<NJ>(lc, s.sn, s.cs, chain);
      {
        V3 e = tip_robot_frame(lc, chain.pe) - desired;
        if (fabs(e.x) > kIkTolerance || fabs(e.y) > kIkTolerance || fabs(e.z) > kIkTolerance) {
          success = 0.0;
          s.word |= LW_IKFAIL;
        }
      }
      if (rot_def && success == 0.0) {
        retried = true;
        ik_step<NJ>(lc, chain, s.q, s.qd, desired, dq);
        update_joints<NJ>(lc, dq, P.dt, P.inv_dt, cv, cp_, s.q, s.qd);
        joint_sincos<NJ>(lc, s.q, s.sn, s.cs);
      }
    } else if (!(SHC_DBG(P) & 8)) {
      double dq[NJ];
      if (LegRegs<NJ>::kKeepJacobian) {
        ik_step_cols<NJ>(lc, s.lin, s.pe, s.q, s.qd, desired, dq);
      } else {
        chain_from_sincos<NJ>(lc, s.sn, s.cs, chain);
        ik_step<NJ>(lc, chain, s.q, s.qd, desired, dq);
      }
      update_joints<NJ>(lc, dq, P.dt, P.inv_dt, fb.uf.clamp_joint_velocities != 0, fb.uf.clamp_joint_positions != 0, s.q, s.qd);
    }
    SHC_PHASE_FENCE();
    SHC_TICK(10);
    if (!(SHC_DBG(P) & 16) && !rot_on) joint_sincos<NJ>(lc, s.q, s.sn, s.cs);
    if (!(SHC_DBG(P) & 512)) chain_from_sincos<NJ>(lc, s.sn, s.cs, chain);
    V3 lin[NJ];
    jacobian_columns<NJ>(chain, lin);
    if (LegRegs<NJ>::kKeepJacobian) {
#pragma unroll
      for (int i = 0; i < NJ; ++i) s.lin[i] = lin[i];
      s.pe = chain.pe;
    }
    SHC_PHASE_FENCE();
    SHC_TICK(11);
    out.model_tip = (SHC_DBG(P) & 512) ? desired : tip_robot_frame(lc, chain.pe);
    if (FT::adm(P) || rot_on) s.tipx = base_rotate(lc, chain.xe);
    V3 e = out.model_tip - desired;
    if (fabs(e.x) > kIkTolerance || fabs(e.y) > kIkTolerance || fabs(e.z) > kIkTolerance) s.word |= LW_IKFAIL;
    if (FT::tipf(P) && !(SHC_DBG(P) & 8192)) {
      double effort[NJ];
      in.effort(effort);
      V3 raw = tip_force_cols<NJ>(lc, chain, lin, effort);
      if constexpr (rot_on) {
        const double gk = 0.15 * P.force_gain;
        s.tf = V3{fma(raw.x, gk, s.tf.x * (1 - 0.15)), fma(raw.y, gk, s.tf.y * (1 - 0.15)), fma(raw.z, gk, s.tf.z * (1 - 0.15))};
        if (retried) s.tf = V3{fma(raw.x, gk, s.tf.x * (1 - 0.15)), fma(raw.y, gk, s.tf.y * (1 - 0.15)), fma(raw.z, gk, s.tf.z * (1 - 0.15))};
      } else {
        s.tf = raw * (0.15 * P.force_gain) + s.tf * (1 - 0.15);
      }
    }
  }
  SHC_TICK(12);
}

template <int L, int NJ, unsigned F, typename IN = LegInPlanes<NJ>, typename MID = NoHook>
__device__ __forceinline__ void cycle(LegRegs<NJ> &s, LegOut &out, const SharedConsts<L, NJ> &C, const RobTile<64 / L> &rb, const Park &pk,
                                      const Group<L> g, int leg, const double *__restrict__ legd, int64_t ns, uint32_t slot, unsigned &dirty,
                                      const bool manual_live, const bool touchdown_detection, double *ext, const ManualRobot *mr, const IN &in,
                                      const MID &mid = MID(), const double *span = nullptr, const bool pose_only = false) {
  FrontToBack fb;
  fb.planes_in_sync = false;
  fb.limit_bracket = -1;
  fb.uf = load_uni_flags(C.P);
  fb.pose_only = pose_only;
  cycle_front<L, NJ, F, true>(s, out, C, rb, pk, g, leg, legd, ns, slot, dirty, manual_live, touchdown_detection, ext, mr, in, fb, span);
  if ((F & F_MLEGS) != 0 && pose_only) return;
  mid();
  cycle_back<L, NJ, F>(s, out, C, leg, legd, ns, slot, mr, in, fb);
}

#endif

}
```

### syropod_highlevel_controller_amd/csrc/shc_cycle_kernel.hpp

```cpp
#pragma once

#include "shc_cycle.hpp"
#include "shc_cycle_launch.hpp"

#include <hip/hip_runtime.h>

#include <type_traits>

namespace shc {

#ifndef SHC_WAVES_PER_SIMD
#define SHC_WAVES_PER_SIMD 2
#endif
#ifndef SHC_ROT_WAVES_PER_SIMD
#define SHC_ROT_WAVES_PER_SIMD 1
#endif
#ifndef SHC_TERRAIN_WAVES_PER_SIMD
#define SHC_TERRAIN_WAVES_PER_SIMD 2
#endif

struct LegPlanes {
  double2 *base;
  int64_t ns;
  uint32_t slot;
// ... 628 lines not shown
        }
      }
      if ((++iter & 1023) == 0 && lane == 0) st_sys(&A.host->heartbeat, iter);
    }
    if (leave) break;
    __builtin_amdgcn_s_sleep(1);
  }
}

template <int L, int NJ, unsigned F, bool RES, int HALF = ROLE_ALL, bool BATCH = false>
__device__ __forceinline__ void cycle_wave(const DevState &st, const SharedConsts<L, NJ> *gc, int n_cycles, unsigned rt_flags, const int64_t wave,
                                           const ResidentArgs *ra) {
  static_assert(HALF == ROLE_ALL || (!RES && (F & (F_DYN | F_TERRAIN | F_MLEGS | F_AUTO)) == 0), "half-step launches: feature-exact kernels without auto posing / terrain paths");
  using R = RobotFields;
  using FT = Feat<F>;
  constexpr int RPW = 64 / L;
  __shared__ SharedConsts<L, NJ> C;
  extern __shared__ double wave_lds[];
  constexpr int kWaveDoubles = R::COUNT * RPW + PK_COUNT * 64 + (R::I_COUNT * RPW + 1) / 2;
  SHC_TICK(0);
  const bool manual_live = (rt_flags & RT_MANUAL_LIVE) != 0;
  const bool touchdown_detection = (rt_flags & RT_TOUCHDOWN) != 0;
  const int lane = threadIdx.x & 63;
  const int wib = threadIdx.x >> 6;
  const int64_t rob0 = wave * RPW;
  const int64_t left = st.n_robots - rob0;
  const int robots_here = left < RPW ? (left < 0 ? 0 : int(left)) : RPW;
  int grp = lane / L;
  const int leg = lane - grp * L;
  const bool live = grp < robots_here;
  if (grp >= robots_here) grp = robots_here > 0 ? robots_here - 1 : 0;
  const uint32_t slot = uint32_t(wave * 64 + grp * L + leg);
  double *const my_lds = wave_lds + wib * kWaveDoubles;
  Park pk{my_lds + R::COUNT * RPW, lane};
  LegRegs<NJ> s;
  const CycleParams &GP = gc->P;
  double *tile = my_lds;
  int32_t *tile_i = reinterpret_cast<int32_t *>(my_lds + R::COUNT * RPW + PK_COUNT * 64);
  double *gtile = st.robd + wave * (R::COUNT * RPW);
  int32_t *gtile_i = st.robi + wave * (R::I_COUNT * RPW);
  LegLoad<NJ> ll;
  double th[NJ];
  const bool any_robot = robots_here > 0;
  double2 hand[4] = {double2{0.0, 0.0}, double2{0.0, 0.0}, double2{0.0, 0.0}, double2{0.0, 0.0}};
  double hpose[7] = {0.0, 0.0, 0.0, 1.0, 0.0, 0.0, 0.0};
  double2 qpl[(NJ + 1) / 2];
  int word_back = 0;
  if (any_robot) {
#pragma unroll
    for (int k = 0; k < NJ; ++k) th[k] = gc->leg[leg].link_th[k];
    load_leg_issue<NJ, F, HALF>(ll, st, GP, slot);
    if constexpr (HALF == ROLE_FRONT) {
#pragma unroll
      for (int p = 0; p < (NJ + 1) / 2; ++p) qpl[p] = reinterpret_cast<const double2 *>(st.legd)[p * st.n_slots + slot];
    }
    if constexpr (HALF == ROLE_BACK) {
      word_back = st.legi[slot];
      using FDh = Fields<NJ>;
      static_assert(FDh::TIP % 2 == 0 && FDh::CUR_DIR == FDh::ORG_DIR + 3 && FDh::ORG_DIR % 2 == 0, "plane layout of the walker tip / tip direction");
      const double2 *planes = reinterpret_cast<const double2 *>(st.legd);
      hand[0] = planes[(FDh::TIP / 2) * st.n_slots + slot];
      hand[1] = planes[(FDh::TIP / 2 + 1) * st.n_slots + slot];
      hand[2] = planes[(FDh::ORG_DIR / 2 + 1) * st.n_slots + slot];
      hand[3] = planes[(FDh::ORG_DIR / 2 + 2) * st.n_slots + slot];
#pragma unroll
      for (int k = 0; k < 7; ++k) hpose[k] = gtile[(R::CPOSE + k) * RPW + grp];
    }
  }
  using SC = SharedConsts<L, NJ>;
  static_assert(sizeof(SC) % 16 == 0 && (offsetof(SC, P) + offsetof(CycleParams, ap_start)) % 16 == 0, "const block is copied in 16-byte words");
  constexpr int n16_all = sizeof(SC) / 16;
  constexpr int n16_core = (offsetof(SC, P) + offsetof(CycleParams, ap_start)) / 16;
  const int n16 = FT::autop(GP) ? n16_all : n16_core;
  constexpr int citers = (n16_all + 63) / 64;
  double2 creg[citers];
  {
    const double2 *src = reinterpret_cast<const double2 *>(gc);
    const int nt = blockDim.x;
#pragma unroll
    for (int it = 0; it < citers; ++it) {
      int i = it * nt + threadIdx.x;
      creg[it] = i < n16 ? src[i] : double2{0.0, 0.0};
    }
  }
  double t_core[(R::CORE_END * RPW + 63) / 64], t_man[((R::MANUAL_END - R::MPOSE) * RPW + 63) / 64],
      t_imu[((R::IMU_END - R::ABSE) * RPW + 63) / 64], t_imuq[((R::IMUQ_END - R::IMUQ) * RPW + 63) / 64],
      t_aprev[((R::APREV_END - R::APREV) * RPW + 63) / 64], t_align[((R::COUNT - R::TALIGN) * RPW + 63) / 64], t_odom[((R::ODOM_END - R::ODOM) * RPW + 63) / 64],
      t_cpose[((R::CPOSE_END - R::CPOSE) * RPW + 63) / 64], t_incl[((R::INCL_END - R::INCL) * RPW + 63) / 64];
  const bool skip_marked = (F & F_MLEGS) != 0 && (rt_flags & RT_SKIP_MARKED) != 0 && (rt_flags & RT_MANUAL_LEGS) != 0;
  const bool pose_marked = (F & F_MLEGS) != 0 && (rt_flags & RT_POSE_MARKED) != 0 && (rt_flags & RT_MANUAL_LEGS) != 0;
  constexpr int int_iters = (R::I_COUNT * RPW + 63) / 64;
  int32_t t_int[int_iters];
  if (any_robot && HALF == ROLE_BACK) {
#pragma unroll
    for (int k = 0; k < NJ; ++k) sincos_joint(th[k] + ll.flat[Fields<NJ>::Q + k], &s.sn[k], &s.cs[k]);
    load_leg_finish<NJ, HALF>(s, pk, ll);
    s.word = word_back;
  }
  if (any_robot && HALF != ROLE_BACK) {
    load_rob_fields<RPW, 0, R::CORE_END>(t_core, gtile, lane);
    if (FT::manual(GP) && manual_live) load_rob_fields<RPW, R::MPOSE, R::MANUAL_END>(t_man, gtile, lane);
    if (FT::imu(GP)) load_rob_fields<RPW, R::ABSE, R::IMU_END>(t_imu, gtile, lane);
    if (FT::imu(GP) || FT::incl(GP) || FT::autop(GP)) load_rob_fields<RPW, R::IMUQ, R::IMUQ_END>(t_imuq, gtile, lane);
    if (FT::incl(GP) && FT::autop(GP)) load_rob_fields<RPW, R::APREV, R::APREV_END>(t_aprev, gtile, lane);
    if (FT::odom(GP)) load_rob_fields<RPW, R::ODOM, R::ODOM_END>(t_odom, gtile, lane);
    if (skip_marked || pose_marked) load_rob_fields<RPW, R::CPOSE, R::CPOSE_END>(t_cpose, gtile, lane);
    if (pose_marked && FT::incl(GP)) load_rob_fields<RPW, R::INCL, R::INCL_END>(t_incl, gtile, lane);
    if ((F & F_TALIGN) != 0 && GP.tip_align) load_rob_fields<RPW, R::TALIGN, R::COUNT>(t_align, gtile, lane);
#pragma unroll
    for (int it = 0; it < int_iters; ++it) t_int[it] = it * 64 + lane < R::I_COUNT * RPW ? gtile_i[it * 64 + lane] : 0;
#pragma unroll
    for (int k = 0; k < NJ; ++k) {
      double qk = ll.flat[Fields<NJ>::Q + k];
      if constexpr (HALF == ROLE_FRONT) qk = (k & 1) ? qpl[k / 2].y : qpl[k / 2].x;
      sincos_joint(th[k] + qk, &s.sn[k], &s.cs[k]);
    }
    load_leg_finish<NJ, HALF>(s, pk, ll);
  }
  {
    double2 *dst = reinterpret_cast<double2 *>(&C);
    const int nt = blockDim.x;
#pragma unroll
    for (int it = 0; it < citers; ++it) {
      int i = it * nt + threadIdx.x;
      if (i < n16) dst[i] = creg[it];
    }
  }
  if (any_robot && HALF != ROLE_BACK) {
    put_rob_fields<RPW, 0, R::CORE_END>(t_core, tile, lane);
    if (FT::manual(GP) && manual_live) put_rob_fields<RPW, R::MPOSE, R::MANUAL_END>(t_man, tile, lane);
    if (FT::imu(GP)) put_rob_fields<RPW, R::ABSE, R::IMU_END>(t_imu, tile, lane);
    if (FT::imu(GP) || FT::incl(GP) || FT::autop(GP)) put_rob_fields<RPW, R::IMUQ, R::IMUQ_END>(t_imuq, tile, lane);
    if (FT::incl(GP) && FT::autop(GP)) put_rob_fields<RPW, R::APREV, R::APREV_END>(t_aprev, tile, lane);
    if (FT::odom(GP)) put_rob_fields<RPW, R::ODOM, R::ODOM_END>(t_odom, tile, lane);
    if (skip_marked || pose_marked) put_rob_fields<RPW, R::CPOSE, R::CPOSE_END>(t_cpose, tile, lane);
    if (pose_marked && FT::incl(GP)) put_rob_fields<RPW, R::INCL, R::INCL_END>(t_incl, tile, lane);
    if ((F & F_TALIGN) != 0 && GP.tip_align) put_rob_fields<RPW, R::TALIGN, R::COUNT>(t_align, tile, lane);
#pragma unroll
    for (int it = 0; it < int_iters; ++it)
      if (it * 64 + lane < R::I_COUNT * RPW) tile_i[it * 64 + lane] = t_int[it];
  }
  SHC_TICK(18);
  __syncthreads();
  SHC_TICK(19);
  if (robots_here == 0) return;
  const CycleParams &P = C.P;
  Group<L> g{grp * L};
  RobTile<RPW> rb{tile, tile_i, grp};
  s.tipx = V3{1, 0, 0};
  constexpr bool rot_on = rot_enabled<NJ, F>();
  if (FT::adm(P) || LegRegs<NJ>::kKeepJacobian || rot_on) {
    Chain<NJ> ch;
    chain_from_sincos<NJ>(C.leg[leg], s.sn, s.cs, ch);
    if (LegRegs<NJ>::kKeepJacobian) {
      jacobian_columns<NJ>(ch, s.lin);
      s.pe = ch.pe;
    }
    if (FT::adm(P) || rot_on) s.tipx = base_rotate(C.leg[leg], ch.xe);
  }
  LegOut out;
  SHC_TICK(1);
  unsigned dirty = 0;
  double *const ext = ((F & F_ROUGH) != 0 && (rt_flags & RT_EXTERNAL) != 0) ? st.ext : nullptr;
  const ManualRobot *const mr = ((F & F_MLEGS) != 0 && (rt_flags & RT_MANUAL_LEGS) != 0 && any_robot) ? st.manual + (rob0 + grp) : nullptr;
  const bool marked = mr != nullptr && mr->skip_cycle != 0;
  const bool skip = (skip_marked && marked) || (pose_marked && !marked);
  const bool pose_only = pose_marked && marked;
  ResidentHeld held;
  if constexpr (RES) {
    resident_loop<L, NJ, F, BATCH>(*ra, st, s, out, C, rb, pk, g, leg, slot, lane, wave, live, tile, tile_i, dirty, manual_live, held, touchdown_detection, ext);
  } else if constexpr (HALF == ROLE_FRONT) {
    FrontToBack fb;
    fb.planes_in_sync = false;
    fb.limit_bracket = -1;
    fb.uf = load_uni_flags(C.P);
    fb.pose_only = false;
    cycle_front<L, NJ, F, (F & F_ADM) == 0>(s, out, C, rb, pk, g, leg, st.legd, st.n_slots, slot, dirty, manual_live, touchdown_detection, ext, mr,
                                            LegInPlanes<NJ>{st.legd, st.n_slots, slot}, fb);
  } else if constexpr (HALF == ROLE_BACK) {
    FrontToBack fb;
    fb.uf = load_uni_flags(C.P);
    fb.pose_only = false;
    fb.joint_moved = false;
    fb.my_leg_state = 0;
    fb.rot_def = (s.word & LW_ROTDEF) != 0;
    {
      const Pose bp{V3{hpose[0], hpose[1], hpose[2]}, Quat{hpose[3], hpose[4], hpose[5], hpose[6]}};
      out.poser_tip = inverse_transform_vector(bp, V3{hand[0].x, hand[0].y, hand[1].x});
      fb.desired_dir = V3{1, 0, 0};
      if (fb.rot_def) fb.desired_dir = rotate(inverse(bp.r), V3{hand[2].y, hand[3].x, hand[3].y});
    }
    out.adm_delta = V3{0.0, 0.0, 0.0};
    if (FT::adm(P)) {
      cycle_admittance<NJ>(s, out, P, LegInPlanes<NJ>{st.legd, st.n_slots, slot});
      if (live && !skip) store_admittance_early<NJ>(s, out, st, slot);
    }
    cycle_back<L, NJ, F>(s, out, C, leg, st.legd, st.n_slots, slot, mr, LegInPlanes<NJ>{st.legd, st.n_slots, slot}, fb);
  } else if (!skip) {
    for (int c = 0; c < n_cycles; ++c)
      cycle<L, NJ, F>(s, out, C, rb, pk, g, leg, st.legd, st.n_slots, slot, dirty, manual_live, touchdown_detection, ext, mr,
                      LegInPlanes<NJ>{st.legd, st.n_slots, slot}, NoHook(), (F & F_ROUGH) != 0 ? st.span : nullptr, pose_only);
    if ((F & F_MLEGS) != 0 && pose_only && FT::autop(P) && !FT::imu(P)) {
      const double2 *planes = reinterpret_cast<const double2 *>(st.legd);
      const double2 a = planes[(Fields<NJ>::POSER_TIP / 2) * st.n_slots + slot], b = planes[(Fields<NJ>::POSER_TIP / 2 + 1) * st.n_slots + slot];
      out.poser_tip = V3{a.x, a.y, b.x};
    }
  }
  {
    unsigned d = 0;
#pragma unroll
    for (unsigned b = 1; b <= DIRTY_LAST; b <<= 1)
      if (__any((dirty & b) != 0)) d |= b;
    dirty = d;
  }
  if (live && !skip) store_leg<NJ, F, HALF, HALF != ROLE_ALL>(s, out, pk, st, P, slot, dirty);
  if constexpr (HALF == ROLE_BACK) {
    if (live) st.legi[slot] = s.word;
    return;
  }
  SHC_TICK(13);
  __builtin_amdgcn_wave_barrier();
  store_rob_fields<RPW, 0, R::PLANE>(tile, gtile, lane);
  if (dirty & DIRTY_WALK_PLANE) store_rob_fields<RPW, R::PLANE, R::VIN>(tile, gtile, lane);
  if (FT::manual(P) && manual_live && (dirty & DIRTY_MANUAL)) store_rob_fields<RPW, R::MPOSE, R::MANUAL_END>(tile, gtile, lane);
  if (FT::imu(P)) store_rob_fields<RPW, R::ABSE, R::GYRO>(tile, gtile, lane);
  if (FT::incl(P) && FT::autop(P)) store_rob_fields<RPW, R::APREV, R::APREV_END>(tile, gtile, lane);
  if ((F & F_MLEGS) != 0 && FT::incl(P) && pose_marked) store_rob_fields<RPW, R::INCL, R::INCL_END>(tile, gtile, lane);
  store_rob_fields<RPW, R::CPOSE, R::CPOSE_END>(tile, gtile, lane);
  if (FT::odom(P)) store_rob_fields<RPW, R::ODOM, R::ODOM_END>(tile, gtile, lane);
  if ((F & F_TALIGN) != 0 && P.tip_align) store_rob_fields<RPW, R::TALIGN, R::COUNT>(tile, gtile, lane);
  static_assert((R::I_POSE_PHASE + 1) * RPW <= 64, "the written-back int fields (word, poser latches, pose phase) fit one wave-wide store");
  if (lane < (R::I_POSE_PHASE + 1) * RPW) gtile_i[lane] = tile_i[lane];
  if constexpr (RES) resident_epilogue<L, NJ, F>(*ra, st, slot, lane, live, tile, tile_i, gtile, gtile_i, held);
  SHC_TICK(14);
}

template <int L, int NJ, unsigned F>
__global__ void __launch_bounds__(256, (F & F_ROT) ? SHC_ROT_WAVES_PER_SIMD : ((F & F_DYN) && (F & F_TERRAIN)) ? SHC_TERRAIN_WAVES_PER_SIMD : SHC_WAVES_PER_SIMD) shc_cycle_kernel(DevState st, const SharedConsts<L, NJ> *gc, int n_cycles,
                                                                                             unsigned rt_flags, int64_t wave0) {
  cycle_wave<L, NJ, F, false>(st, gc, n_cycles, rt_flags, wave0 + ((int64_t(blockIdx.x) * blockDim.x + threadIdx.x) >> 6), nullptr);
}

template <int L, int NJ, unsigned F, int HALF>
__global__ void __launch_bounds__(256, 2) shc_cycle_half_kernel(DevState st, const SharedConsts<L, NJ> *gc, unsigned rt_flags, int64_t wave0) {
  cycle_wave<L, NJ, F, false, HALF>(st, gc, 1, rt_flags, wave0 + ((int64_t(blockIdx.x) * blockDim.x + threadIdx.x) >> 6), nullptr);
}

template <int L, int NJ, unsigned F>
__global__ void __launch_bounds__(64, (F & (F_ROT | F_ROUGH)) ? 1 : SHC_WAVES_PER_SIMD) shc_resident_kernel(DevState st, const SharedConsts<L, NJ> *gc, ResidentArgs ra, unsigned rt_flags) {
  if (blockIdx.x == 0) {
    resident_relay<PART_BOTH>(ra);
    return;
  }
  cycle_wave<L, NJ, F, true>(st, gc, 0, rt_flags, int64_t(blockIdx.x) - 1, &ra);
}

template <int L, int NJ, unsigned F>
__global__ void __launch_bounds__(256, (F & F_ROT) ? SHC_ROT_WAVES_PER_SIMD : SHC_WAVES_PER_SIMD) shc_batch_kernel(DevState st, const SharedConsts<L, NJ> *gc, ResidentArgs ra, unsigned rt_flags) {
  cycle_wave<L, NJ, F, true, ROLE_ALL, true>(st, gc, 0, rt_flags, ra.batch_wave0 + ((int64_t(blockIdx.x) * blockDim.x + threadIdx.x) >> 6), &ra);
}

enum : int { IT_REAL = 1, IT_BUBBLE = 2, IT_EXIT = 3 };
template <int RPW>
struct PoseWait {
  unsigned *flag_at;
  unsigned want;
  u64 ticks_per_ms;
  bool *fault;
  __device__ __forceinline__ bool give_up(unsigned &spins, u64 &t0) const {
    __builtin_amdgcn_s_sleep(1);
    if ((++spins & 4095u) == 0) {
      const u64 now = wall_clock64();
      if (t0 == 0) t0 = now;
      else if (now - t0 > 1000 * ticks_per_ms) {
        *fault = true;
        return true;
      }
    }
    return false;
  }
  __device__ __forceinline__ void operator()() const {
    volatile unsigned *flag = flag_at;
    unsigned spins = 0;
    u64 t0 = 0;
    while (*flag != want)
      if (give_up(spins, t0)) break;
    __builtin_amdgcn_fence(__ATOMIC_ACQUIRE, "workgroup");
  }
};
template <int L, int NJ>
struct Resident2Lds {
  double mailbox[2][2][13][64];
  double pose_c[2][2][64];
  unsigned pose_done[2];
  unsigned model_dirty[2], model_seen[2], model_fault[2];
  double stiff[2][64];
  int ikfail[2][64];
  unsigned long long ctrl[4][4];
};
template <int L, int NJ>
struct Resident3Lds : Resident2Lds<L, NJ> {
  int leg_word[2][2][64];
  unsigned back_seen[2];
};

template <int L, int NJ, unsigned F, bool HELPER = false>
__global__ void __launch_bounds__(HELPER ? 384 : 256, 1) shc_resident2_kernel(DevState st, const SharedConsts<L, NJ> *gc, ResidentArgs A, unsigned rt_flags) {
  using R = RobotFields;
  using FD = Fields<NJ>;
  using FT = Feat<F>;
  constexpr int RPW = 64 / L;
  constexpr int kThreads = HELPER ? 384 : 256;
  if (blockIdx.x == 0) {
    if (threadIdx.x < 64) resident_relay<PART_GATE>(A);
    else if (threadIdx.x < 128) resident_relay<PART_DONE>(A);
    return;
  }
  __shared__ SharedConsts<L, NJ> C;
  extern __shared__ double wave_lds[];
  constexpr int kWaveDoubles = R::COUNT * RPW + PK_COUNT * 64 + (R::I_COUNT * RPW + 1) / 2;
  using Lds = std::conditional_t<HELPER, Resident3Lds<L, NJ>, Resident2Lds<L, NJ>>;
  Lds &X = *reinterpret_cast<Lds *>(wave_lds + 2 * kWaveDoubles);
  const bool manual_live = (rt_flags & RT_MANUAL_LIVE) != 0;
  const int lane = threadIdx.x & 63;
  const int wib = __builtin_amdgcn_readfirstlane(threadIdx.x >> 6);
  const int pair = wib & 1;
  const bool walker = HELPER ? (wib >> 1) == 1 : wib < 2, helper = HELPER && wib >= 4, leader = wib == (HELPER ? 4 : 2);
  const int64_t wave = (int64_t(blockIdx.x) - 1) * 2 + pair;
  const bool active = wave < A.n_waves;
  const int64_t rob0 = wave * RPW;
  const int64_t left = st.n_robots - rob0;
  const int robots_here = !active ? 0 : (left < RPW ? (left < 0 ? 0 : int(left)) : RPW);
  int grp = lane / L;
  const int leg = lane - grp * L;
  const bool live = grp < robots_here;
  if (grp >= robots_here) grp = robots_here > 0 ? robots_here - 1 : 0;
  const uint32_t slot = uint32_t((active ? wave : 0) * 64 + grp * L + leg);
  double *const my_lds = wave_lds + pair * kWaveDoubles;
  Park pk{my_lds + R::COUNT * RPW, lane};
  double *tile = my_lds;
  int32_t *tile_i = reinterpret_cast<int32_t *>(my_lds + R::COUNT * RPW + PK_COUNT * 64);
  double *gtile = st.robd + (active ? wave : 0) * (R::COUNT * RPW);
  int32_t *gtile_i = st.robi + (active ? wave : 0) * (R::I_COUNT * RPW);
  const CycleParams &GP = gc->P;
  LegRegs<NJ> s;
  {
    using SC = SharedConsts<L, NJ>;
    constexpr int n16_all = sizeof(SC) / 16;
    constexpr int n16_core = (offsetof(SC, P) + offsetof(CycleParams, ap_start)) / 16;
    const int n16 = FT::autop(GP) ? n16_all : n16_core;
    const double2 *src = reinterpret_cast<const double2 *>(gc);
    double2 *dst = reinterpret_cast<double2 *>(&C);
    for (int i = threadIdx.x; i < n16; i += kThreads) dst[i] = src[i];
  }
  LegLoad<NJ> ll;
  if (active) {
    if (walker) {
      load_leg_issue<NJ, F, ROLE_FRONT>(ll, st, GP, slot);
      for (int i = lane; i < R::COUNT * RPW; i += 64) tile[i] = gtile[i];
      for (int i = lane; i < R::I_COUNT * RPW; i += 64) tile_i[i] = gtile_i[i];
      load_leg_finish<NJ, ROLE_FRONT>(s, pk, ll);
    } else if (!helper) {
      load_leg_issue<NJ, F, ROLE_BACK>(ll, st, GP, slot);
      load_leg_finish<NJ, ROLE_BACK>(s, pk, ll);
    }
  }
  if (leader && lane == 0) {
    X.ctrl[0][0] = IT_BUBBLE;
    X.ctrl[0][1] = X.ctrl[0][2] = 0;
  }
  constexpr bool POSE_SPLIT = (F & (F_DYN | F_AUTO)) == 0;
  if (POSE_SPLIT && walker && lane == 0) X.pose_done[pair] = 0;
  __syncthreads();
  const CycleParams &P = C.P;
  Group<L> g{grp * L};
  RobTile<RPW> rb{tile, tile_i, grp};
  LegOut out;
  out.poser_tip = out.model_tip = out.adm_delta = V3{0, 0, 0};
  s.tipx = V3{1, 0, 0};
  if (active && !walker && !helper) {
#pragma unroll
    for (int k = 0; k < NJ; ++k) sincos_joint(C.leg[leg].link_th[k] + s.q[k], &s.sn[k], &s.cs[k]);
    if (FT::adm(P) || LegRegs<NJ>::kKeepJacobian) {
      Chain<NJ> ch;
      chain_from_sincos<NJ>(C.leg[leg], s.sn, s.cs, ch);
      if (LegRegs<NJ>::kKeepJacobian) {
        jacobian_columns<NJ>(ch, s.lin);
        s.pe = ch.pe;
      }
      if (FT::adm(P)) s.tipx = base_rotate(C.leg[leg], ch.xe);
    }
    s.word = 0;
  }
  unsigned dirty = 0;
  ResidentHeld held;
  const int swing_c_count_u = uni(P.swing_c_count);
  const auto publish_for_pose = [&](unsigned cycle, bool planes) {
    if (planes) {
      const V3 pp = rb.get3(R::PLANE_PREV), pn = rb.get3(R::PNORM_PREV);
#pragma unroll
      for (int par = 0; par < 2; ++par) {
        double *mb = &X.mailbox[pair][par][0][lane];
        mb[7 * 64] = pp.x, mb[8 * 64] = pp.y, mb[9 * 64] = pp.z, mb[10 * 64] = pn.x, mb[11 * 64] = pn.y, mb[12 * 64] = pn.z;
      }
    }
    if constexpr (HELPER) X.leg_word[pair][cycle & 1][lane] = s.word;
    else X.pose_c[pair][cycle & 1][lane] = walk_plane_control_candidate<L, NJ>(s.word, C, P, swing_c_count_u);
  };
  if (POSE_SPLIT && walker && active) publish_for_pose(0, true);
  const int64_t ns = st.n_slots;
  const unsigned out_slot_bytes = unsigned(NJ * ns * 16);
  const __amdgpu_buffer_rsrc_t out_rsrc = __builtin_amdgcn_make_buffer_rsrc(A.out, 0, int(unsigned(A.depth) * out_slot_bytes), 0x00020000);
  const u64 emergency_ticks = 4 * A.idle_ticks + 2000 * A.ticks_per_ms;
  unsigned k = 0, c_front = 0, c_back = 0, oslot = 0;
  bool prev_real = false;
  u64 prev_h0 = 0, prev_h1 = 0;
  u64 gate_pref = leader ? ld_agent(&A.ctl->gate) : 0;
  u64 bubble_since = 0;
  FrontToBack fb{V3{1, 0, 0}, false, LS_WALKING};
  fb.uf = load_uni_flags(C.P);
  OdomCache odom_cache;
  Pose owpp_cache = pose_identity();
  const bool poser = HELPER ? helper : !walker;
  if (POSE_SPLIT && active && poser) owpp_cache = rb.getpose(R::OWPP);
  constexpr bool ODOM_REGS = NJ <= 3;
  constexpr bool ODOM_WALKER = NJ > 3 || (F & (F_ADM | F_IMU | F_INCL | F_AUTO | F_DYN)) != 0;
  static_assert(!HELPER || (POSE_SPLIT && !ODOM_WALKER && ODOM_REGS), "the helper takes the pose and the odometry off the MODEL wavefront");
  const bool odom_mine = ODOM_WALKER ? walker : poser;
  double odom[4] = {0.0, 0.0, 1.0, 0.0};
  if (ODOM_REGS && FT::odom(P) && active && odom_mine) {
#pragma unroll
    for (int i = 0; i < 4; ++i) odom[i] = rb.get(R::ODOM + i);
  }
#ifdef SHC_RES2_TIMING
  long long tm_busy = 0, tm_total0 = __builtin_readcyclecounter(), tm_real = 0;
#ifndef SHC_RES2_BUSY_ONLY
  if (threadIdx.x < 96) shc_acc_lds[threadIdx.x] = 0;
#endif
#endif
#ifdef SHC_RES2_TIMING
#define SHC_R2_ITER_BEGIN() const long long tm0 = __builtin_readcyclecounter(); SHC_TICK(19)
#ifndef SHC_RES2_BUSY_ONLY
#define SHC_R2_PHASES(THREAD, ...)                                                                                                  \
  if (kind == IT_REAL && prev_real && blockIdx.x == 1 && threadIdx.x == (THREAD)) {       \
    const int base = ((THREAD) >> 7) * 32;                                                                                         \
    const int order[] = {__VA_ARGS__};                                                                                             \
    for (int i = 1; i < int(sizeof(order) / sizeof(int)); ++i) shc_acc_lds[base + order[i]] += shc_ticks_lds[base + order[i]] - shc_ticks_lds[base + order[i - 1]]; \
  }
#else
#define SHC_R2_PHASES(THREAD, ...)
#endif
#define SHC_R2_ITER_END(THREAD, ...)                                                         \
  if (kind == IT_REAL && prev_real) tm_busy += __builtin_readcyclecounter() - tm0, ++tm_real; \
  SHC_R2_PHASES(THREAD, __VA_ARGS__)
#else
#define SHC_R2_ITER_BEGIN() do {} while (0)
#define SHC_R2_ITER_END(THREAD, ...) do {} while (0)
#endif
  LegInRing<NJ> in_at;
  int in_src_force = -1000, in_src_effort = -1000;
  const auto leader_decide = [&](const int kind, int &nk, u64 &nh0v, u64 &nh1v) __attribute__((always_inline)) {
    u64 gate;
    if (kind == IT_BUBBLE) {
      __builtin_amdgcn_s_sleep(2);
      gate = uni64(ld_agent(&A.ctl->gate));
    } else {
      gate = uni64(gate_pref);
    }
    const unsigned db = unsigned(gate), sp = unsigned(gate >> 32);
    const unsigned cn = c_front + (kind == IT_REAL ? 1u : 0u);
    nk = cn >= sp ? IT_EXIT : (cn < db ? IT_REAL : IT_BUBBLE);
    if (nk == IT_BUBBLE) {
      const u64 now = wall_clock64();
      if (bubble_since == 0) bubble_since = now;
      else if (now - bubble_since > emergency_ticks) nk = IT_EXIT, held.fault = true;
    } else {
      bubble_since = 0;
    }
    if (nk == IT_REAL) {
      const u64 *hp = reinterpret_cast<const u64 *>(A.headers + (cn & (kResidentHeaders - 1)));
      nh0v = ld_agent(hp);
      nh1v = ld_agent(hp + 1);
    }
    if (kind == IT_BUBBLE) gate_pref = gate;
    else gate_pref = ld_agent(&A.ctl->gate);
  };
  const auto leader_announce = [&](const int nk, const u64 nh0v, const u64 nh1v) __attribute__((always_inline)) {
    X.ctrl[(k + 1) & 3][0] = u64(nk);
    X.ctrl[(k + 1) & 3][1] = nh0v;
    X.ctrl[(k + 1) & 3][2] = nh1v;
  };
  const auto pose_of_cycle = [&](const u64 h0, const u64 h1) __attribute__((always_inline)) {
    if constexpr (!POSE_SPLIT) return;
    else {
    resident_take_inputs<RPW, ROBOT_POSE, false>(A, c_front, h0, h1, wave, lane, tile, tile_i, dirty, held, st.n_robots);
    SHC_TICK(30);
    double pose_c = -1.0;
    if constexpr (HELPER) {
      const double c_own = walk_plane_control_candidate<L, NJ>(X.leg_word[pair][c_front & 1][lane], C, P, swing_c_count_u);
#pragma unroll
      for (int j = 0; j < L; ++j) {
        const double cj = g.get(c_own, j);
        pose_c = cj >= 0.0 ? cj : pose_c;
      }
    } else {
#pragma unroll
      for (int j = 0; j < L; ++j) {
        const double cj = X.pose_c[pair][c_front & 1][g.base + j];
        pose_c = cj >= 0.0 ? cj : pose_c;
      }
    }
    int lw[L] = {};
    const double *mb = &X.mailbox[pair][c_front & 1][0][lane];
    const V3 plane_prev{mb[7 * 64], mb[8 * 64], mb[9 * 64]}, pnorm_prev{mb[10 * 64], mb[11 * 64], mb[12 * 64]};
    int rword_unused = 0;
    Pose ap = pose_identity(), la = pose_identity();
#ifdef SHC_ABLATE
    if (!(P.debug_skip & 2048))
#endif
    (void)cycle_pose<L, NJ, F, true>(s, C, P, C.leg[leg], rb, g, leg, lw, rword_unused, 0, dirty, manual_live, ap, la, plane_prev, pnorm_prev, fb.uf.swing_c_count, 0,
                                     &owpp_cache, &pose_c);
    __builtin_amdgcn_fence(__ATOMIC_RELEASE, "workgroup");
    __builtin_amdgcn_wave_barrier();
    if (lane == 0) *const_cast<volatile unsigned *>(&X.pose_done[pair]) = c_front + 1;
    }
  };
  const auto odometry_of_cycle = [&](const double *mb) __attribute__((always_inline)) {
    const V3 ov{mb[192], mb[256], mb[320]};
    if (__any(mb[384] != 0.0)) {
      if (mb[384] != 0.0) {
        if constexpr (ODOM_REGS) odometry_advance(odom[0], odom[1], odom[2], odom[3], P, ov.x, ov.y, ov.z, &odom_cache);
        else odometry_step(rb, P, ov.x, ov.y, ov.z, &odom_cache);
      }
    }
  };
  constexpr int kWalkerThread = HELPER ? 128 : 0, kModelThread = HELPER ? 0 : 128;
  if (walker) {
    for (;;) {
      SHC_R2_ITER_BEGIN();
      const int kind = __builtin_amdgcn_readfirstlane(int(X.ctrl[k & 3][0]));
      const u64 h0 = uni64(X.ctrl[k & 3][1]), h1 = uni64(X.ctrl[k & 3][2]);
      SHC_TICK(20);
      if (kind == IT_REAL && active) {
        resident_take_inputs<RPW, POSE_SPLIT ? ROBOT_VEL : ROBOT_ALL, false>(A, c_front, h0, h1, wave, lane, tile, tile_i, dirty, held, st.n_robots);
        SHC_TICK(21);
        const PoseWait<RPW> pose_wait{&X.pose_done[pair], c_front + 1, A.ticks_per_ms, &held.fault};
        cycle_front<L, NJ, F, false, LegInRing<NJ>, false, !POSE_SPLIT>(s, out, C, rb, pk, g, leg, st.legd, ns, slot, dirty, manual_live, false, nullptr, nullptr,
                                                                        LegInRing<NJ>{}, fb, nullptr, pose_wait);
#ifdef SHC_ABLATE
        if (!(P.debug_skip & 65536))
#endif
        if (POSE_SPLIT) publish_for_pose(c_front + 1, fb.plane_prev_changed);
        SHC_TICK(29);
        double *mb = &X.mailbox[pair][c_front & 1][0][lane];
        mb[0] = out.poser_tip.x, mb[64] = out.poser_tip.y, mb[128] = out.poser_tip.z;
        if constexpr (ODOM_WALKER) {
          if (FT::odom(P) && __any(fb.odom_run)) {
            if (fb.odom_run) {
              if constexpr (ODOM_REGS) odometry_advance(odom[0], odom[1], odom[2], odom[3], P, fb.odom_vel.x, fb.odom_vel.y, fb.odom_vel.z, &odom_cache);
              else odometry_step(rb, P, fb.odom_vel.x, fb.odom_vel.y, fb.odom_vel.z, &odom_cache);
            }
          }
        } else if (FT::odom(P)) {
          mb[192] = fb.odom_vel.x, mb[256] = fb.odom_vel.y, mb[320] = fb.odom_vel.z, mb[384] = fb.odom_run ? 1.0 : 0.0;
        }
        SHC_TICK(22);
      }
      SHC_TICK(23);
      if (kind == IT_EXIT) break;
      SHC_R2_ITER_END(kWalkerThread, 19, 20, 21, 2, 3, 4, 5, 6, 7, 16, 8, 17, 15, 29, 22, 23);
      if (kind == IT_REAL) ++c_front;
      prev_real = kind == IT_REAL;
      __syncthreads();
      ++k;
    }
  } else if (helper) {
    if constexpr (HELPER) for (;;) {
      SHC_R2_ITER_BEGIN();
      const int kind = __builtin_amdgcn_readfirstlane(int(X.ctrl[k & 3][0]));
      const u64 h0 = uni64(X.ctrl[k & 3][1]), h1 = uni64(X.ctrl[k & 3][2]);
      SHC_TICK(29);
      int nk = IT_EXIT;
      u64 nh0v = 0, nh1v = 0;
      if (leader && kind != IT_EXIT) leader_decide(kind, nk, nh0v, nh1v);
      if (active) {
        SHC_TICK(24);
        if (kind == IT_REAL) pose_of_cycle(h0, h1);
        SHC_TICK(25);
        if (prev_real) {
          if (FT::odom(P)) odometry_of_cycle(&X.mailbox[pair][c_back & 1][0][lane]);
          ++c_back;
        }
        SHC_TICK(26);
      }
      if (leader && kind != IT_EXIT && lane == 0) leader_announce(nk, nh0v, nh1v);
      SHC_TICK(14);
      if (kind == IT_EXIT) break;
      SHC_R2_ITER_END(256, 19, 29, 24, 30, 25, 26, 14);
      if (kind == IT_REAL) ++c_front;
      prev_real = kind == IT_REAL;
      __syncthreads();
      ++k;
    }
  } else {
    for (;;) {
      SHC_R2_ITER_BEGIN();
      const int kind = __builtin_amdgcn_readfirstlane(int(X.ctrl[k & 3][0]));
      const u64 h0 = uni64(X.ctrl[k & 3][1]), h1 = uni64(X.ctrl[k & 3][2]);
      SHC_TICK(29);
      [[maybe_unused]] int nk = IT_EXIT;
      [[maybe_unused]] u64 nh0v = 0, nh1v = 0;
      if constexpr (!HELPER) if (leader && kind != IT_EXIT) leader_decide(kind, nk, nh0v, nh1v);
      if (active) {
        SHC_TICK(24);
        if constexpr (POSE_SPLIT && !HELPER) if (kind == IT_REAL) pose_of_cycle(h0, h1);
        SHC_TICK(25);
        if (prev_real) {
          resident_take_inputs<RPW, ROBOT_NONE, true>(A, c_back, prev_h0, prev_h1, wave, lane, tile, tile_i, dirty, held, st.n_robots);
          if (held.src_force != in_src_force || held.src_effort != in_src_effort) {
            in_at = leg_inputs_in_force<L, NJ>(A, st.legd, held.src_force, held.src_effort, ns, slot, wave * RPW + grp, leg);
            in_src_force = held.src_force, in_src_effort = held.src_effort;
          }
          LegInRing<NJ> in = in_at;
          if (FT::tipf(P)) in.prefetch_effort();
          SHC_TICK(31);
          const double *mb = &X.mailbox[pair][c_back & 1][0][lane];
          out.poser_tip = V3{mb[0], mb[64], mb[128]};
          if constexpr (!ODOM_WALKER && !HELPER) if (FT::odom(P)) odometry_of_cycle(mb);
          out.adm_delta = V3{0, 0, 0};
          if (FT::adm(P)) cycle_admittance<NJ>(s, out, P, in);
          s.word = 0;
          SHC_TICK(26);
          cycle_back<L, NJ, F>(s, out, C, leg, st.legd, ns, slot, nullptr, in, fb);
          SHC_TICK(27);
          asm volatile("s_waitcnt vmcnt(0)" ::: "memory");
          if (lane == 0) st_agent(A.progress + wave, u64(c_back));
          SHC_TICK(13);
          {
            typedef unsigned v4u __attribute__((ext_vector_type(4)));
            double flat[2 * NJ];
#pragma unroll
            for (int i = 0; i < NJ; ++i) flat[FD::Q + i] = s.q[i], flat[FD::QD + i] = s.qd[i];
            const unsigned soff = oslot * out_slot_bytes;
#ifdef SHC_ABLATE
            if (!(P.debug_skip & 4096))
#endif
            if (live) {
#pragma unroll
              for (int p = 0; p < NJ; ++p) {
                const u64 a = u64(__double_as_longlong(flat[2 * p])), b = u64(__double_as_longlong(flat[2 * p + 1]));
                const v4u w = {unsigned(a), unsigned(a >> 32), unsigned(b), unsigned(b >> 32)};
                __builtin_amdgcn_raw_buffer_store_b128(w, out_rsrc, unsigned((int64_t(p) * ns + slot) * 16), soff, 16 );
              }
            }
          }
          ++c_back;
          oslot = oslot + 1 == unsigned(A.depth) ? 0 : oslot + 1;
          SHC_TICK(28);
        }
        if (kind != IT_REAL) {
          asm volatile("s_waitcnt vmcnt(0)" ::: "memory");
          if (lane == 0) st_agent(A.progress + wave, u64(c_back));
        }
      }
      if constexpr (!HELPER) if (leader && kind != IT_EXIT && lane == 0) leader_announce(nk, nh0v, nh1v);
      SHC_TICK(14);
      if (kind == IT_EXIT) break;
      SHC_R2_ITER_END(kModelThread, 19, 29, 24, 30, 25, 31, 26, 9, 10, 11, 12, 27, 13, 28, 14);
      if (kind == IT_REAL) ++c_front;
      prev_real = kind == IT_REAL;
      prev_h0 = h0, prev_h1 = h1;
      __syncthreads();
      ++k;
    }
  }
#undef SHC_R2_ITER_BEGIN
#undef SHC_R2_ITER_END
#undef SHC_R2_PHASES
#ifdef SHC_RES2_TIMING
  if (blockIdx.x == 1 && lane == 0 && pair == 0) {
    unsigned long long *rec = reinterpret_cast<unsigned long long *>(A.ctl) + 8, *dbg = rec + (walker ? 0 : helper ? 72 : 4);
    dbg[0] = tm_busy, dbg[1] = tm_real, dbg[2] = __builtin_readcyclecounter() - tm_total0, dbg[3] = k;
#ifndef SHC_RES2_BUSY_ONLY
    const int from = int(threadIdx.x >> 7) * 32, to = walker ? 8 : helper ? 80 : 40;
    for (int i = 0; i < 32; ++i) rec[to + i] = (unsigned long long)shc_acc_lds[from + i];
#endif
  }
#endif
  if (active && ODOM_REGS && FT::odom(P) && odom_mine) {
#pragma unroll
    for (int i = 0; i < 4; ++i) rb.put(R::ODOM + i, odom[i]);
  }
  if (active) {
    if (walker) {
      X.stiff[pair][lane] = s.stiff;
    } else {
      if (!helper) X.ikfail[pair][lane] = s.word & LW_IKFAIL;
      if constexpr (HELPER) if (!helper && lane == 0) X.back_seen[pair] = held.seen;
      if (poser) {
        if (POSE_SPLIT) {
          unsigned d = 0;
#pragma unroll
          for (unsigned b = 1; b <= DIRTY_LAST; b <<= 1)
            if (__any((dirty & b) != 0)) d |= b;
          if (lane == 0) X.model_dirty[pair] = d, X.model_seen[pair] = held.seen;
        }
        if (lane == 0) X.model_fault[pair] = held.fault ? 1u : 0u;
      }
    }
  }
  __syncthreads();
  if (!active || helper) return;
  if (walker) {
    if (POSE_SPLIT) dirty |= X.model_dirty[pair], held.seen |= X.model_seen[pair];
    if constexpr (HELPER) held.seen |= X.back_seen[pair];
    if (X.model_fault[pair]) held.fault = true;
    if (c_front > 0) s.word = (s.word & ~LW_IKFAIL) | X.ikfail[pair][lane];
    {
      unsigned d = 0;
#pragma unroll
      for (unsigned b = 1; b <= DIRTY_LAST; b <<= 1)
        if (__any((dirty & b) != 0)) d |= b;
      dirty = d;
    }
    if (live) store_leg<NJ, F, ROLE_FRONT>(s, out, pk, st, P, slot, dirty);
    __builtin_amdgcn_wave_barrier();
    store_rob_fields<RPW, 0, R::PLANE>(tile, gtile, lane);
    if (dirty & DIRTY_WALK_PLANE) store_rob_fields<RPW, R::PLANE, R::VIN>(tile, gtile, lane);
    if (FT::manual(P) && manual_live && (dirty & DIRTY_MANUAL)) store_rob_fields<RPW, R::MPOSE, R::MANUAL_END>(tile, gtile, lane);
    if (FT::imu(P)) store_rob_fields<RPW, R::ABSE, R::GYRO>(tile, gtile, lane);
    if (FT::incl(P) && FT::autop(P)) store_rob_fields<RPW, R::APREV, R::APREV_END>(tile, gtile, lane);
    store_rob_fields<RPW, R::CPOSE, R::CPOSE_END>(tile, gtile, lane);
    if (FT::odom(P)) store_rob_fields<RPW, R::ODOM, R::ODOM_END>(tile, gtile, lane);
    if (lane < (R::I_POSE_PHASE + 1) * RPW) gtile_i[lane] = tile_i[lane];
    store_rob_fields<RPW, R::VIN, R::CORE_END>(tile, gtile, lane);
    if (held.seen & (1u << RG_IMU)) {
      store_rob_fields<RPW, R::GYRO, R::IMU_END>(tile, gtile, lane);
      store_rob_fields<RPW, R::IMUQ, R::IMUQ_END>(tile, gtile, lane);
    }
    if ((held.seen & (1u << RG_RESET)) && lane < RPW) gtile_i[R::I_RESET_MODE * RPW + lane] = tile_i[R::I_RESET_MODE * RPW + lane];
    if (lane == 0) {
      if (held.fault) __hip_atomic_fetch_or(&A.ctl->fault, 1ull, __ATOMIC_RELAXED, __HIP_MEMORY_SCOPE_AGENT);
      __hip_atomic_fetch_add(&A.ctl->exited, 1ull, __ATOMIC_RELAXED, __HIP_MEMORY_SCOPE_AGENT);
    }
  } else {
    s.stiff = X.stiff[pair][lane];
    if (live) {
      store_leg<NJ, F, ROLE_BACK>(s, out, pk, st, P, slot, 0);
      carry_leg_inputs<L, NJ>(A, st, held, ns, slot, leg);
    }
  }
}

}
```

### syropod_highlevel_controller_amd/csrc/shc_math.hpp

```cpp
#pragma once

#include <hip/hip_runtime.h>
#include <cmath>
#include <cstdint>

#define SHC_HD __host__ __device__ __forceinline__

namespace shc {

constexpr double kPi = 3.14159265358979323846;
constexpr double kUnassigned = 2147483647.0;
constexpr double kIkTolerance = 0.005;
constexpr double kDls = 0.02;
constexpr double kJointLimitCostWeight = 0.1;
constexpr double kTipTolerance = 0.01;
constexpr double kJointTolerance = 0.01;
constexpr double kGravity = -9.81;

struct V3 {
  double x, y, z;
};
struct Quat {
  double w, x, y, z;
};
struct Pose {
  V3 p;
  Quat r;
};

SHC_HD V3 v3(double x, double y, double z) { return V3{x, y, z}; }
SHC_HD V3 operator+(V3 a, V3 b) { return V3{a.x + b.x, a.y + b.y, a.z + b.z}; }
SHC_HD V3 operator-(V3 a, V3 b) { return V3{a.x - b.x, a.y - b.y, a.z - b.z}; }
SHC_HD V3 operator-(V3 a) { return V3{-a.x, -a.y, -a.z}; }
SHC_HD V3 operator*(V3 a, double s) { return V3{a.x * s, a.y * s, a.z * s}; }
SHC_HD V3 operator*(double s, V3 a) { return V3{a.x * s, a.y * s, a.z * s}; }
SHC_HD V3 scaled(V3 a, double s) {
#pragma clang fp contract(off)
  return V3{a.x * s, a.y * s, a.z * s};
}
SHC_HD double dot(V3 a, V3 b) { return a.x * b.x + a.y * b.y + a.z * b.z; }
SHC_HD V3 sel3(bool c, V3 a, V3 b) { return V3{c ? a.x : b.x, c ? a.y : b.y, c ? a.z : b.z}; }
SHC_HD V3 cross(V3 a, V3 b) { return V3{a.y * b.z - a.z * b.y, a.z * b.x - a.x * b.z, a.x * b.y - a.y * b.x}; }
SHC_HD double norm(V3 a) { return sqrt(dot(a, a)); }
SHC_HD V3 normalized(V3 a) {
  double z = dot(a, a);
  if (z > 0.0) {
    double s = sqrt(z);
    return V3{a.x / s, a.y / s, a.z / s};
  }
  return a;
}
SHC_HD V3 projection(V3 a, V3 b) {
  double bb = dot(b, b);
  if (dot(a, a) == 0.0 || bb == 0.0) return V3{0, 0, 0};
  return b * (dot(a, b) / bb);
}
SHC_HD V3 rejection(V3 a, V3 b) { return a - projection(a, b); }

SHC_HD double clampd(double v, double lo, double hi) { return fmax(lo, fmin(v, hi)); }
SHC_HD double signd(double v) { return v > 0 ? 1.0 : -1.0; }
SHC_HD int mod_i(int a, int b) { return (a % b + b) % b; }
SHC_HD int round_to_int(double x) { return x >= 0 ? int(x + 0.5) : -int(0.5 - x); }
SHC_HD int round_to_even_int(double x) { return (int(x) % 2 == 0) ? int(x) : int(x) + 1; }
SHC_HD double smooth_step(double c) {
  double c3 = c * c * c;
  return c3 * (10.0 + c * (-15.0 + 6.0 * c));
}
SHC_HD double rad2deg(double r) { return (r / (2.0 * kPi)) * 360.0; }
SHC_HD double deg2rad(double d) { return d / 360.0 * 2.0 * kPi; }

SHC_HD double pio2_reduce(double x, double *y, double *yt) {
#pragma clang fp contract(off)
  const double inv_pio2 = 6.36619772367581382433e-01;
  const double pio2_1 = 1.57079632673412561417e+00;
  const double pio2_1t = 6.07710050650619224932e-11;
  const double fn = rint(x * inv_pio2);
  const double r = fma(-fn, pio2_1, x);
  const double w = fn * pio2_1t;
  const double we = fma(fn, pio2_1t, -w);
  const double yy = r - w;
  *y = yy;
  *yt = ((r - yy) - w) - we;
  return fn;
}
template <bool REDUCE = true>
SHC_HD void sincos_joint(double x, double *sn, double *cs) {
  if (!REDUCE) {
    const double z = x * x, v = z * x;
    const double S1 = -1.66666666666666324348e-01, S2 = 8.33333333332248946124e-03, S3 = -1.98412698298579493134e-04,
                 S4 = 2.75573137070700676789e-06, S5 = -2.50507602534068634195e-08, S6 = 1.58969099521155010221e-10;
    const double C1 = 4.16666666666666019037e-02, C2 = -1.38888888888741095749e-03, C3 = 2.48015872894767294178e-05,
                 C4 = -2.75573143513906633035e-07, C5 = 2.08757232129817482790e-09, C6 = -1.13596475577881948265e-11;
    const double rs = S2 + z * (S3 + z * (S4 + z * (S5 + z * S6)));
    *sn = x - ((z * (-(v * rs))) - v * S1);
    const double rc = z * (C1 + z * (C2 + z * (C3 + z * (C4 + z * (C5 + z * C6)))));
    const double hz = 0.5 * z, w1 = 1.0 - hz;
    *cs = w1 + (((1.0 - w1) - hz) + z * rc);
    return;
  }
  double y, yt;
  int n = int(pio2_reduce(x, &y, &yt));
  double z = y * y;
  const double S1 = -1.66666666666666324348e-01, S2 = 8.33333333332248946124e-03, S3 = -1.98412698298579493134e-04,
               S4 = 2.75573137070700676789e-06, S5 = -2.50507602534068634195e-08, S6 = 1.58969099521155010221e-10;
  double v = z * y;
  double rs = S2 + z * (S3 + z * (S4 + z * (S5 + z * S6)));
  double s = y - ((z * (0.5 * yt - v * rs) - yt) - v * S1);
  const double C1 = 4.16666666666666019037e-02, C2 = -1.38888888888741095749e-03, C3 = 2.48015872894767294178e-05,
               C4 = -2.75573143513906633035e-07, C5 = 2.08757232129817482790e-09, C6 = -1.13596475577881948265e-11;
  double rc = z * (C1 + z * (C2 + z * (C3 + z * (C4 + z * (C5 + z * C6)))));
  double hz = 0.5 * z;
  double w1 = 1.0 - hz;
  double c = w1 + (((1.0 - w1) - hz) + (z * rc - y * yt));
  double ss = (n & 1) ? c : s, cc = (n & 1) ? s : c;
  if (n & 2) ss = -ss;
  if ((n + 1) & 2) cc = -cc;
  *sn = ss;
  *cs = cc;
}

SHC_HD Quat quat(double w, double x, double y, double z) { return Quat{w, x, y, z}; }
SHC_HD Quat quat_identity() { return Quat{1, 0, 0, 0}; }
SHC_HD Quat operator*(Quat a, Quat b) {
  return Quat{a.w * b.w - a.x * b.x - a.y * b.y - a.z * b.z, a.w * b.x + a.x * b.w + a.y * b.z - a.z * b.y,
              a.w * b.y + a.y * b.w + a.z * b.x - a.x * b.z, a.w * b.z + a.z * b.w + a.x * b.y - a.y * b.x};
}
SHC_HD Quat conj(Quat q) { return Quat{q.w, -q.x, -q.y, -q.z}; }
SHC_HD double dot(Quat a, Quat b) { return a.w * b.w + a.x * b.x + a.y * b.y + a.z * b.z; }
SHC_HD Quat inverse(Quat q) {
  double n2 = dot(q, q);
  if (n2 > 0.0) return Quat{q.w / n2, -q.x / n2, -q.y / n2, -q.z / n2};
  return Quat{0, 0, 0, 0};
}
SHC_HD Quat normalized(Quat q) {
  double z = dot(q, q);
  if (z > 0.0) {
    double s = sqrt(z);
    return Quat{q.w / s, q.x / s, q.y / s, q.z / s};
  }
  return q;
}
SHC_HD V3 rotate(Quat q, V3 v) {
  V3 qv{q.x, q.y, q.z};
  V3 uv = cross(qv, v);
  uv = uv + uv;
  return v + uv * q.w + cross(qv, uv);
}
SHC_HD Quat correct_rotation(Quat t, Quat ref) {
  return dot(t, ref) < 0.0 ? Quat{-t.w, -t.x, -t.y, -t.z} : t;
}
SHC_HD Quat angle_axis_x(double a) { return Quat{cos(0.5 * a), sin(0.5 * a), 0, 0}; }
SHC_HD Quat angle_axis_y(double a) { return Quat{cos(0.5 * a), 0, sin(0.5 * a), 0}; }
SHC_HD Quat angle_axis_z(double a) { return Quat{cos(0.5 * a), 0, 0, sin(0.5 * a)}; }
SHC_HD Quat euler_to_quat(V3 e, bool intrinsic) {
  double sx, cx, sy, cy, sz, cz;
  sincos_joint(0.5 * e.x, &sx, &cx);
  sincos_joint(0.5 * e.y, &sy, &cy);
  sincos_joint(0.5 * e.z, &sz, &cz);
  Quat qx{cx, sx, 0, 0}, qy{cy, 0, sy, 0}, qz{cz, 0, 0, sz};
  return intrinsic ? (qx * qy) * qz : (qz * qy) * qx;
}
SHC_HD V3 quat_to_euler(Quat q, bool intrinsic) {
  double tx = 2.0 * q.x, ty = 2.0 * q.y, tz = 2.0 * q.z;
  double twx = tx * q.w, twy = ty * q.w, twz = tz * q.w;
  double txx = tx * q.x, txy = ty * q.x, txz = tz * q.x;
  double tyy = ty * q.y, tyz = tz * q.y, tzz = tz * q.z;
  double m00 = 1.0 - (tyy + tzz), m01 = txy - twz, m02 = txz + twy;
  double m10 = txy + twz, m11 = 1.0 - (txx + tzz), m12 = tyz - twx;
  double m20 = txz - twy, m21 = tyz + twx, m22 = 1.0 - (txx + tyy);
  double r0, r1, r2;
  if (intrinsic) {
    r0 = atan2(m12, m22);
    double c2 = sqrt(m00 * m00 + m01 * m01);
    if (r0 > 0.0) {
      r0 -= kPi;
      r1 = atan2(-m02, -c2);
    } else {
      r1 = atan2(-m02, c2);
    }
    double s1, c1;
#ifdef SHC_POSE_R5
    sincos(r0, &s1, &c1);
#else
    sincos_joint(r0, &s1, &c1);
#endif
    r2 = atan2(s1 * m20 - c1 * m10, c1 * m11 - s1 * m21);
    r0 = -r0;
    r1 = -r1;
    r2 = -r2;
  } else {
    r0 = atan2(m10, m00);
    double c2 = sqrt(m22 * m22 + m21 * m21);
    if (r0 < 0.0) {
      r0 += kPi;
      r1 = atan2(-m20, -c2);
    } else {
      r1 = atan2(-m20, c2);
    }
    double s1, c1;
#ifdef SHC_POSE_R5
    sincos(r0, &s1, &c1);
#else
    sincos_joint(r0, &s1, &c1);
#endif
    r2 = atan2(s1 * m02 - c1 * m12, c1 * m11 - s1 * m01);
  }
  if (fabs(r1) > kPi / 2 || fabs(r2) > kPi / 2) {
    r0 -= kPi;
    if (r1 > kPi / 2.0) r1 = -r1 + kPi;
    else if (r1 < kPi / 2.0) r1 = -r1 - kPi;
    if (r2 > kPi / 2.0) r2 -= kPi;
    else if (r2 < kPi / 2.0) r2 += kPi;
  }
  return intrinsic ? V3{r0, r1, r2} : V3{r2, r1, r0};
}
SHC_HD Quat from_two_vectors(V3 a, V3 b) {
  V3 v0 = normalized(a), v1 = normalized(b);
  double c = dot(v1, v0);
  if (c < -1.0 + 1e-12) {
    c = fmax(c, -1.0);
    V3 o = fabs(v0.x) < 0.9 ? V3{1, 0, 0} : V3{0, 1, 0};
    V3 ax = normalized(cross(v0, o));
    double w2 = (1.0 + c) * 0.5;
    double s = sqrt(1.0 - w2);
    return Quat{sqrt(w2), ax.x * s, ax.y * s, ax.z * s};
  }
  V3 ax = cross(v0, v1);
  double s = sqrt((1.0 + c) * 2.0);
  double invs = 1.0 / s;
  return Quat{s * 0.5, ax.x * invs, ax.y * invs, ax.z * invs};
}
SHC_HD Quat quat_from_matrix(const double (&m)[9]) {
  double q[3], w;
  double t = m[0] + m[4] + m[8];
  if (t > 0.0) {
    t = sqrt(t + 1.0);
    w = 0.5 * t;
    t = 0.5 / t;
    q[0] = (m[7] - m[5]) * t;
    q[1] = (m[2] - m[6]) * t;
    q[2] = (m[3] - m[1]) * t;
  } else {
    int i = 0;
    if (m[4] > m[0]) i = 1;
    if (m[8] > m[i * 4]) i = 2;
    const int j = (i + 1) % 3, k = (j + 1) % 3;
    t = sqrt(m[i * 4] - m[j * 4] - m[k * 4] + 1.0);
    q[i] = 0.5 * t;
    t = 0.5 / t;
    w = (m[k * 3 + j] - m[j * 3 + k]) * t;
    q[j] = (m[j * 3 + i] + m[i * 3 + j]) * t;
    q[k] = (m[k * 3 + i] + m[i * 3 + k]) * t;
  }
  return Quat{w, q[0], q[1], q[2]};
}
SHC_HD V3 angle_axis_vector(Quat q) {
  double n = sqrt(q.x * q.x + q.y * q.y + q.z * q.z);
  if (n != 0.0) {
    double angle = 2.0 * atan2(n, fabs(q.w));
    if (q.w < 0.0) n = -n;
    return V3{q.x / n * angle, q.y / n * angle, q.z / n * angle};
  }
  return V3{0, 0, 0};
}
SHC_HD V3 lerp3(V3 a, V3 b, double c) { return b * c + a * (1.0 - c); }
SHC_HD Quat slerp(Quat a, double t, Quat b) {
  const double one = 1.0 - 2.220446049250313e-16;
  double d = dot(a, b);
  double ad = fabs(d);
  double s0, s1;
  if (ad >= one) {
    s0 = 1.0 - t;
    s1 = t;
  } else {
    double th = acos(ad);
    double st = sin(th);
    s0 = sin((1.0 - t) * th) / st;
    s1 = sin(t * th) / st;
  }
  if (d < 0.0) s1 = -s1;
  return Quat{s0 * a.w + s1 * b.w, s0 * a.x + s1 * b.x, s0 * a.y + s1 * b.y, s0 * a.z + s1 * b.z};
}

SHC_HD Pose pose_identity() { return Pose{V3{0, 0, 0}, Quat{1, 0, 0, 0}}; }
SHC_HD V3 transform_vector(const Pose &a, V3 v) { return a.p + rotate(a.r, v); }
SHC_HD V3 inverse_transform_vector(const Pose &a, V3 v) { return rotate(conj(a.r), v - a.p); }
SHC_HD Pose add_pose(const Pose &a, const Pose &b) { return Pose{transform_vector(a, b.p), a.r * b.r}; }
SHC_HD Pose remove_pose(const Pose &a, const Pose &b) { return Pose{transform_vector(a, -b.p), a.r * inverse(b.r)}; }
SHC_HD Pose interpolate_pose(const Pose &a, double c, const Pose &t) {
  return Pose{t.p * c + a.p * (1.0 - c), slerp(a.r, c, t.r)};
}

SHC_HD V3 quartic_bezier(const V3 *p, double t) {
  double s = 1.0 - t;
  double b0 = s * s * s * s, b1 = 4.0 * t * s * s * s, b2 = 6.0 * t * t * s * s, b3 = 4.0 * t * t * t * s, b4 = t * t * t * t;
  return p[0] * b0 + p[1] * b1 + p[2] * b2 + p[3] * b3 + p[4] * b4;
}
SHC_HD V3 fma3(V3 a, double s, V3 c) { return V3{fma(a.x, s, c.x), fma(a.y, s, c.y), fma(a.z, s, c.z)}; }
SHC_HD V3 quartic_bezier_dot(V3 p0, V3 p1, V3 p2, V3 p3, V3 p4, double t) {
  double s = 1.0 - t;
  V3 r = (p1 - p0) * (4.0 * s * s * s);
  r = fma3(p2 - p1, 12.0 * s * s * t, r);
  r = fma3(p3 - p2, 12.0 * s * t * t, r);
  return fma3(p4 - p3, 4.0 * t * t * t, r);
}

template <bool EXACT = false>
SHC_HD double fast_rcp(double x) {
  if (EXACT) return 1.0 / x;
#if defined(__HIP_DEVICE_COMPILE__)
  double r = __builtin_amdgcn_rcp(x);
  r = fma(r, fma(-x, r, 1.0), r);
  r = fma(r, fma(-x, r, 1.0), r);
  return r;
#else
  return 1.0 / x;
#endif
}
template <bool EXACT = false>
SHC_HD double fast_rsqrt(double x) {
  if (EXACT) return 1.0 / sqrt(x);
#if defined(__HIP_DEVICE_COMPILE__)
  double y = __builtin_amdgcn_rsq(x);
  y = fma(0.5 * y, fma(-x * y, y, 1.0), y);
  y = fma(0.5 * y, fma(-x * y, y, 1.0), y);
  return y;
#else
  return 1.0 / sqrt(x);
#endif
}

template <int N, bool EXACT = false>
SHC_HD void spd_solve(double (&a)[N][N], double (&b)[N]) {
  double dinv[N];
#pragma unroll
  for (int k = 0; k < N; ++k) {
    dinv[k] = fast_rcp<EXACT>(a[k][k]);
#pragma unroll
    for (int i = k + 1; i < N; ++i) {
      double l = a[i][k] * dinv[k];
#pragma unroll
      for (int j = k + 1; j <= i; ++j) a[i][j] -= l * a[j][k];
    }
#pragma unroll
    for (int i = k + 1; i < N; ++i) {
      double l = a[i][k] * dinv[k];
      b[i] -= l * b[k];
      a[i][k] = l;
    }
  }
#pragma unroll
  for (int k = 0; k < N; ++k) b[k] *= dinv[k];
#pragma unroll
  for (int k = N - 1; k >= 0; --k) {
#pragma unroll
    for (int i = k + 1; i < N; ++i) b[k] -= a[i][k] * b[i];
  }
}

}
```

### syropod_highlevel_controller_amd/csrc/shc_resident.hpp

```cpp

struct Resident {
  bool active = false;
  int depth = 0;
  ResidentArgs args{};
  ResidentHost *host = nullptr;
  ResidentHost *host_dev = nullptr;
  ResidentCtl *ctl = nullptr;
  unsigned long long *progress = nullptr;
  ResidentHeader *headers = nullptr;
  double *rin = nullptr, *force = nullptr, *effort = nullptr, *out = nullptr, *stage = nullptr;
  int32_t *rini = nullptr;
  size_t stage_bytes = 0;
  static constexpr int kPinSlots = 4;
  unsigned *post_blocks_done = nullptr;
  char *pin = nullptr, *pin_dev = nullptr;
  hipEvent_t pin_ev[kPinSlots] = {};
  unsigned long long pin_uses = 0;
  hipStream_t in_stream = nullptr;
  hipStream_t loop_stream = nullptr;
  hipEvent_t loop_ev = nullptr;
  unsigned long long published = 0;
  unsigned long long posted = 0;
  unsigned long long posts[RG_COUNT] = {};
  std::vector<unsigned long long> post_cycle[RG_COUNT];
// ... 292 lines not shown
  r->helper_wave = two_wave && fit.helper_wave && !(two_role && atoi(two_role) > 0);
  HIP_TRY(hipEventRecord(r->loop_ev, e->stream));
  HIP_TRY(hipStreamWaitEvent(r->loop_stream, r->loop_ev, 0));
  CycleLaunch a = cycle_launch(e);
  a.stream = r->loop_stream, a.resident = &A;
  a.grid = two_wave ? unsigned((e->n_waves + 1) / 2 + 1) : unsigned(e->n_waves + 1), a.block = r->helper_wave ? 384 : two_wave ? 256 : 64;
  {
    const int rc = launch_cycle_for(e, a);
    if (rc != SHC_OK) return rc;
  }
  HIP_TRY(hipGetLastError());
  r->active = true;
  return SHC_OK;
}

static int resident_wait_direct_installed(Resident *r) {
  if (r->direct_last < 0) return SHC_OK;
  const unsigned long long need = (unsigned long long)r->direct_last + 1;
  if (!spin_until([&] { return host_load(&r->host->done) >= need || host_load(&r->host->exited) != 0; }, 5.0))
    return fail(SHC_ERR_TIMEOUT, "resident mode: a direct post is still waiting to run");
  r->direct_last = -1;
  return SHC_OK;
}

static int resident_alive(Resident *r) {
  if (const unsigned long long why = host_load(&r->host->exited))
    return fail(SHC_ERR_TIMEOUT, std::string("resident mode: the device loop has stopped by itself (") +
                                     (why == RESIDENT_EXIT_IDLE ? "idle timeout" : why == RESIDENT_EXIT_MAX ? "max_cycles" : why == RESIDENT_EXIT_FAULT ? "fault" : "stop") +
                                     " after " + std::to_string(host_load(&r->host->done)) + " cycles): call shc_engine_resident_end");
  return SHC_OK;
}

extern "C" int shc_engine_resident_post(shc_engine *e, const shc_cycle_inputs *in, int64_t *cycle) {
  int rc = resident_require(e, true);
  if (rc != SHC_OK) return rc;
  Resident *r = e->res;
  if ((rc = resident_alive(r)) != SHC_OK) return rc;
  if (!in) return fail(SHC_ERR_INVALID_ARG, "inputs is NULL");
  if ((in->linear_xy == nullptr) != (in->angular == nullptr)) return fail(SHC_ERR_INVALID_ARG, "linear_xy and angular are posted together");
  if ((in->imu_orientation_wxyz == nullptr) != (in->imu_angular_velocity == nullptr)) return fail(SHC_ERR_INVALID_ARG, "the two IMU arrays are posted together");
  if ((in->pose_translation_velocity == nullptr) != (in->pose_rotation_velocity == nullptr))
    return fail(SHC_ERR_INVALID_ARG, "the two pose input arrays are posted together");
  unsigned mask = 0;
  if (in->linear_xy) mask |= 1u << RG_VEL;
  if (in->imu_orientation_wxyz) mask |= 1u << RG_IMU;
  if (in->pose_translation_velocity) mask |= 1u << RG_POSE;
  if (in->pose_reset_mode) mask |= 1u << RG_RESET;
  if (in->tip_force) mask |= 1u << RG_FORCE;
  if (in->joint_effort) mask |= 1u << RG_EFFORT;
  if ((mask & ((1u << RG_POSE) | (1u << RG_RESET))) && !(e->rt_flags & RT_MANUAL_LIVE))
    return fail(SHC_ERR_UNSUPPORTED, "pose inputs: give the engine one (shc_engine_set_pose_input / set_pose_reset_mode) before shc_engine_resident_begin");
  if ((mask & (1u << RG_EFFORT)) && !(e->rt_flags & RT_EFFORT_LIVE))
    return fail(SHC_ERR_UNSUPPORTED, "joint efforts: give the engine one (shc_engine_set_joint_effort) before shc_engine_resident_begin");
  const unsigned long long c = r->posted;
  if (c < r->published) return fail(SHC_ERR_INVALID_ARG, "resident mode: this cycle has already been published without inputs");
  if (c >= r->max_cycles) return fail(SHC_ERR_INVALID_ARG, "resident mode: past max_cycles");
  HIP_TRY(hipSetDevice(e->device));
  const double patience = 5.0;
  if (c >= kResidentHeaders && !spin_until([&] { return host_load(&r->host->done) > c - kResidentHeaders; }, patience))
    return fail(SHC_ERR_TIMEOUT, "resident mode: 1024 posted cycles are waiting to run");
  if (in->direct) {
    const int set = in->direct - 1;
    if (set < 0 || set >= kBoundSets) return fail(SHC_ERR_INVALID_ARG, "direct: bound input set 1 .. 4");
    if (mask & ((1u << RG_POSE) | (1u << RG_RESET))) return fail(SHC_ERR_INVALID_ARG, "direct posts carry velocity, IMU, tip force and joint effort; post pose inputs / reset modes the ordinary way");
    if (mask == 0) return fail(SHC_ERR_INVALID_ARG, "direct post without inputs (use shc_engine_resident_publish)");
    const int need[RG_COUNT] = {BND_LIN, BND_IMUQ, -1, -1, BND_FORCE, BND_EFFORT};
    for (int gi = 0; gi < RG_COUNT; ++gi)
      if ((mask & (1u << gi)) && (need[gi] < 0 || !r->args.bound[set][need[gi]]))
        return fail(SHC_ERR_INVALID_ARG, "direct post: that group is not part of the bound input set (shc_engine_resident_bind_inputs before shc_engine_resident_begin)");
    if (r->published < c) {
      const int rc2 = shc_engine_resident_publish(e, int64_t(c - r->published));
      if (rc2 != SHC_OK) return rc2;
    }
    const unsigned long long tag = c + 1;
    volatile unsigned long long *rec = r->host->records + size_t(c & (kResidentHeaders - 1)) * 2;
    rec[1] = (unsigned long long)mask | ((unsigned long long)set << 16) | ((tag & 0xffffull) << 48);
    host_store(const_cast<unsigned long long *>(&rec[0]), tag);
    r->groups_posted |= mask;
    r->posted = r->published = c + 1;
    r->direct_last = (long long)c;
    if (cycle) *cycle = int64_t(c);
    return SHC_OK;
  }
  ResidentPost pp{};
  pp.mask = mask;
  pp.cycle = c;
  for (int gi = 0; gi < RG_COUNT; ++gi) {
    if (!(mask & (1u << gi))) continue;
    const unsigned long long k = r->posts[gi];
    pp.pos[gi] = int(k % r->depth);
    if (k >= (unsigned long long)r->depth) {
      const unsigned long long successor_cycle = r->post_cycle[gi][(k + 1) % r->depth];
      if (!spin_until([&] { return host_load(&r->host->done) >= successor_cycle || host_load(&r->host->exited) != 0; }, patience))
        return fail(SHC_ERR_TIMEOUT, "resident mode: ring_depth posted input sets are waiting to be consumed (publish them)");
    }
  }
  size_t off = 0;
  const int pin_slot = int(r->pin_uses % Resident::kPinSlots);
  if (!in->on_device && r->pin_uses >= (unsigned long long)Resident::kPinSlots) HIP_TRY(hipEventSynchronize(r->pin_ev[pin_slot]));
  auto dev = [&](const void *src, size_t bytes, const void **out) -> int {
    if (in->on_device) {
      *out = src;
      return SHC_OK;
    }
    if (off + bytes > r->stage_bytes) return fail(SHC_ERR_INVALID_ARG, "staging buffer too small");
    const size_t at = size_t(pin_slot) * r->stage_bytes + off;
    memcpy(r->pin + at, src, bytes);
    *out = r->pin_dev + at;
    off += (bytes + 15) & ~size_t(15);
    return SHC_OK;
  };
  const size_t n = size_t(e->n), nl = n * e->L;
#define STAGE(field, member, bytes)                                                              \
  if (in->member) {                                                                              \
    const void *d_;                                                                              \
    if ((rc = dev(in->member, bytes, &d_)) != SHC_OK) return rc;                                 \
    pp.field = reinterpret_cast<decltype(pp.field)>(d_);                                         \
  }
  STAGE(lin, linear_xy, n * 16)
  STAGE(ang, angular, n * 8)
  STAGE(imu_q, imu_orientation_wxyz, n * 32)
  STAGE(imu_w, imu_angular_velocity, n * 24)
  STAGE(tvi, pose_translation_velocity, n * 24)
  STAGE(rvi, pose_rotation_velocity, n * 24)
  STAGE(reset, pose_reset_mode, n * 4)
  STAGE(force, tip_force, nl * 24)
  STAGE(effort, joint_effort, nl * e->NJ * 8)
#undef STAGE
  const int64_t threads = (mask & ((1u << RG_FORCE) | (1u << RG_EFFORT))) ? int64_t(nl) : int64_t(n);
  const bool publish = in->publish != 0;
  if (publish) {
    if ((rc = resident_wait_direct_installed(r)) != SHC_OK) return rc;
    pp.doorbell = c + 1;
    pp.host = r->host_dev;
    pp.blocks_done = r->post_blocks_done;
  }
  resident_post_kernel<<<dim3((unsigned)((threads + 63) / 64)), dim3(64), 0, r->in_stream>>>(pp, r->args, r->headers, r->rin, r->rini, r->force, r->effort,
                                                                                              e->n, e->L, e->NJ, e->n_slots);
  HIP_TRY(hipGetLastError());
  if (!in->on_device) {
    HIP_TRY(hipEventRecord(r->pin_ev[pin_slot], r->in_stream));
    r->pin_uses++;
  }
  for (int gi = 0; gi < RG_COUNT; ++gi)
    if (mask & (1u << gi)) {
      r->post_cycle[gi][r->posts[gi] % r->depth] = c;
      r->posts[gi]++;
    }
  r->groups_posted |= mask;
  r->posted = c + 1;
  if (publish) r->published = c + 1;
  r->stream_doorbell_pending = true;
  if (cycle) *cycle = int64_t(c);
  return SHC_OK;
}

extern "C" int shc_engine_resident_publish(shc_engine *e, int64_t n_cycles) {
  int rc = resident_require(e, true);
  if (rc != SHC_OK) return rc;
  Resident *r = e->res;
  if ((rc = resident_alive(r)) != SHC_OK) return rc;
  if (n_cycles < 0) return fail(SHC_ERR_INVALID_ARG, "n_cycles < 0");
  if (n_cycles == 0) return SHC_OK;
  if (r->published + (unsigned long long)n_cycles > r->max_cycles) return fail(SHC_ERR_INVALID_ARG, "resident mode: past max_cycles");
  if ((rc = resident_wait_direct_installed(r)) != SHC_OK) return rc;
  r->published += (unsigned long long)n_cycles;
  if (r->posted < r->published) r->posted = r->published;
  if (r->stream_doorbell_pending) {
    HIP_TRY(hipSetDevice(e->device));
    if (hipStreamQuery(r->in_stream) == hipSuccess) {
      r->stream_doorbell_pending = false;
    } else {
      resident_doorbell_kernel<<<dim3(1), dim3(1), 0, r->in_stream>>>(r->host_dev, r->published);
      HIP_TRY(hipGetLastError());
      return SHC_OK;
    }
  }
  host_store(&r->host->doorbell, r->published);
  return SHC_OK;
}

extern "C" int shc_engine_resident_wait(shc_engine *e, int64_t cycles, int timeout_ms) {
  int rc = resident_require(e, true);
  if (rc != SHC_OK) return rc;
  Resident *r = e->res;
  if (cycles < 0 || (unsigned long long)cycles > r->published) return fail(SHC_ERR_INVALID_ARG, "resident mode: waiting for cycles that were not published");
  const unsigned long long want = (unsigned long long)cycles;
  if (!spin_until([&] { return host_load(&r->host->done) >= want || host_load(&r->host->exited) != 0; }, timeout_ms > 0 ? timeout_ms * 1e-3 : 10.0))
    return fail(SHC_ERR_TIMEOUT, "resident mode: the published cycles did not complete in time");
  if (host_load(&r->host->done) < want) return fail(SHC_ERR_TIMEOUT, "resident mode: the device loop stopped before these cycles ran");
  return SHC_OK;
}

extern "C" int shc_engine_resident_get_joint_state(shc_engine *e, int64_t cycle, double *q, double *qd, int on_device) {
  int rc = resident_require(e, true);
  if (rc != SHC_OK) return rc;
  Resident *r = e->res;
  const unsigned long long done = host_load(&r->host->done);
  if (cycle < 0 || (unsigned long long)cycle >= done) return fail(SHC_ERR_INVALID_ARG, "resident mode: that cycle has not completed (shc_engine_resident_wait)");
  if (r->published > (unsigned long long)cycle + r->depth)
    return fail(SHC_ERR_INVALID_ARG, "resident mode: that cycle's outputs may have been overwritten (ring_depth newer cycles were published)");
  HIP_TRY(hipSetDevice(e->device));
  const double *slot = r->out + size_t(cycle % r->depth) * size_t(e->NJ) * e->n_slots * 2;
  const int64_t threads = e->n * e->L;
  for (int which = 0; which < 2; ++which) {
    double *dst = which ? qd : q;
    if (!dst) continue;
    double *d = on_device ? dst : r->stage;
    gather_leg_kernel<<<dim3((unsigned)((threads + 63) / 64)), dim3(64), 0, r->in_stream>>>(d, slot, e->n_slots, e->n, e->L, e->NJ,
                                                                                            which ? LEG_FIELD(e, QD) : LEG_FIELD(e, Q));
    HIP_TRY(hipGetLastError());
    if (!on_device) {
      HIP_TRY(hipMemcpyAsync(dst, d, size_t(threads) * e->NJ * 8, hipMemcpyDeviceToHost, r->in_stream));
      HIP_TRY(hipStreamSynchronize(r->in_stream));
    }
  }
  if (on_device) HIP_TRY(hipStreamSynchronize(r->in_stream));
  return SHC_OK;
}

__global__ void resident_wait_done_kernel(const ResidentCtl *ctl, ResidentHost *host, unsigned long long want, unsigned long long timeout_ticks) {
  const unsigned long long t0 = wall_clock64();
  auto done = [&] { return __hip_atomic_load(&ctl->pad[1], __ATOMIC_ACQUIRE, __HIP_MEMORY_SCOPE_AGENT); };
  for (;;) {
    if (done() >= want) return;
    if (__hip_atomic_load(&ctl->pad[2], __ATOMIC_ACQUIRE, __HIP_MEMORY_SCOPE_AGENT) != 0 && done() < want) break;
    if (wall_clock64() - t0 > timeout_ticks) break;
    __builtin_amdgcn_s_sleep(8);
  }
  __hip_atomic_fetch_add(&host->late_reads, 1ull, __ATOMIC_RELAXED, __HIP_MEMORY_SCOPE_SYSTEM);
}

extern "C" int shc_engine_resident_get_joint_state_async(shc_engine *e, int64_t cycle, double *q, double *qd, int timeout_ms) {
  int rc = resident_require(e, true);
  if (rc != SHC_OK) return rc;
  Resident *r = e->res;
  if ((rc = resident_alive(r)) != SHC_OK) return rc;
  if (cycle < 0 || (unsigned long long)cycle >= r->max_cycles) return fail(SHC_ERR_INVALID_ARG, "resident mode: no such cycle (max_cycles)");
  if (r->published > (unsigned long long)cycle + r->depth)
    return fail(SHC_ERR_INVALID_ARG, "resident mode: that cycle's outputs may have been overwritten (ring_depth newer cycles were published)");
  HIP_TRY(hipSetDevice(e->device));
  const unsigned long long ticks = (unsigned long long)(timeout_ms > 0 ? timeout_ms : 5000) * r->wall_khz;
  resident_wait_done_kernel<<<dim3(1), dim3(1), 0, e->stream>>>(r->ctl, r->host_dev, (unsigned long long)cycle + 1, ticks);
  HIP_TRY(hipGetLastError());
  const double *slot = r->out + size_t(cycle % r->depth) * size_t(e->NJ) * e->n_slots * 2;
  const int64_t threads = e->n * e->L;
  for (int which = 0; which < 2; ++which) {
    double *dst = which ? qd : q;
    if (!dst) continue;
    gather_leg_kernel<<<dim3((unsigned)((threads + 63) / 64)), dim3(64), 0, e->stream>>>(dst, slot, e->n_slots, e->n, e->L, e->NJ,
                                                                                         which ? LEG_FIELD(e, QD) : LEG_FIELD(e, Q));
    HIP_TRY(hipGetLastError());
  }
  return SHC_OK;
}

extern "C" int shc_engine_resident_status(shc_engine *e, int64_t *published, int64_t *completed, int32_t *running) {
  int rc = resident_require(e, false);
  if (rc != SHC_OK) return rc;
  Resident *r = e->res;
  const bool active = r && r->active;
  if (published) *published = active ? int64_t(r->published) : 0;
  if (completed) *completed = active ? int64_t(host_load(&r->host->done)) : 0;
  if (running) *running = active && host_load(&r->host->exited) == 0 ? 1 : 0;
  return SHC_OK;
}

extern "C" int shc_engine_resident_end(shc_engine *e, int64_t *cycles_run) {
  int rc = resident_require(e, true);
  if (rc != SHC_OK) return rc;
  Resident *r = e->res;
  HIP_TRY(hipSetDevice(e->device));
  HIP_TRY(hipStreamSynchronize(r->in_stream));
  const int direct_rc = resident_wait_direct_installed(r);
  const std::string direct_msg = direct_rc != SHC_OK ? std::string(shc_last_error()) : std::string();
  if (direct_rc == SHC_OK) host_store(&r->host->doorbell, r->published);
  host_store(&r->host->stop, direct_rc == SHC_OK ? r->published : 0ull);
  const bool answered = spin_until([&] { return host_load(&r->host->exited) != 0; }, r->poisoned ? 5.0 : 30.0);
  if (!answered) {
    r->poisoned = true;
    return fail(SHC_ERR_TIMEOUT, "resident mode: the device loop did not answer the stop request in time; the engine stays in resident mode - call "
                                 "shc_engine_resident_end again");
  }
  hipError_t err = hipStreamSynchronize(r->loop_stream);
  if (err == hipSuccess) err = hipStreamSynchronize(e->stream);
  r->active = false;
  r->poisoned = false;
#ifdef SHC_RES2_TIMING
  if (err == hipSuccess) {
    ResidentCtl c;
    (void)hipMemcpy(&c, r->ctl, sizeof c, hipMemcpyDeviceToHost);
    for (int w = 0; w < (r->helper_wave ? 3 : 2); ++w) {
      const unsigned long long *b = c.dbg + (w == 2 ? 72 : 4 * w);
      fprintf(stderr, "[res2 timing] %s: %.0f clocks busy per steady REAL iteration (%llu of them), loop %llu clocks, %llu iterations\n", w == 0 ? "walker" : w == 1 ? "model " : "helper",
              b[1] ? double(b[0]) / double(b[1]) : 0.0, b[1], b[2], b[3]);
    }
#ifndef SHC_RES2_BUSY_ONLY
    const int order[] = {20, 21, 2, 3, 4, 5, 6, 7, 16, 8, 17, 15, 29, 22, 23};
    const char *wname[] = {"control words (LDS) read", "inputs of the cycle taken", "cycle_front entry", "robot word / command read, stop predicates", "(pose elsewhere)", "getLimit",
                           "velocity shaping", "walk state machine", "stepper (stride, Bezier, tip)", "tip rotation / iteratePhase / planes / leg word", "wait for the pose flag",
                           "pose read + updateStance", "control input for the next pose published", "mailbox written", "to the barrier"};
    const double its = c.dbg[1] ? double(c.dbg[1]) : 1.0;
    fprintf(stderr, "[res2 timing] walker of pair 0, mean clocks per phase:\n");
    for (int i = 0; i < int(sizeof(order) / sizeof(int)); ++i) fprintf(stderr, "[res2 timing]   walker t%-2d %-58s %7.0f\n", order[i], wname[i], double(c.dbg[8 + order[i]]) / its);
    const int morder[] = {29, 24, 30, 25, 31, 26, 9, 10, 11, 12, 27, 13, 28, 14};
    const char *mname[] = {"control words (LDS) read", "leader: gate, what the next iteration is, header prefetch issued", "pose inputs of the cycle taken",
                           "updateCurrentPose of the walker's cycle + flag", "leg inputs in force, joint efforts prefetched", "mailbox read, odometry, admittance",
                           "cycle_back entry (desired tip)", "IK step + joint update", "sin / cos, chain, Jacobian", "model tip, tip force", "cycle_back exit",
                           "wait for the previous stores + progress word", "output-ring stores issued", "control words written (leader: waits for its loads)"};
    const double mits = c.dbg[5] ? double(c.dbg[5]) : 1.0;
    fprintf(stderr, "[res2 timing] model wavefront of pair 0 (the leader), mean clocks per phase:\n");
    for (int i = 0; i < int(sizeof(morder) / sizeof(int)); ++i) {
      if (r->helper_wave && (morder[i] == 30 || morder[i] == 25)) continue;
      fprintf(stderr, "[res2 timing]   model  t%-2d %-58s %7.0f\n", morder[i], mname[i], double(c.dbg[40 + morder[i]]) / mits);
    }
    if (r->helper_wave) {
      const int horder[] = {29, 24, 30, 25, 26, 14};
      const char *hname[] = {"control words (LDS) read", "leader: gate, what the next iteration is, header prefetch issued", "pose inputs of the cycle taken",
                             "leg words reduced, updateCurrentPose of the walker's cycle + flag", "odometry", "control words written (leader: waits for its loads)"};
      const double hits = c.dbg[73] ? double(c.dbg[73]) : 1.0;
      fprintf(stderr, "[res2 timing] helper wavefront of pair 0 (the leader), mean clocks per phase:\n");
      for (int i = 0; i < int(sizeof(horder) / sizeof(int)); ++i) fprintf(stderr, "[res2 timing]   helper t%-2d %-58s %7.0f\n", horder[i], hname[i], double(c.dbg[80 + horder[i]]) / hits);
    }
#endif
  }
#endif
  const unsigned long long reason = host_load(&r->host->exited), done = host_load(&r->host->done);
  if (cycles_run) *cycles_run = int64_t(done);
  if (r->groups_posted & (1u << RG_FORCE)) e->rt_flags |= RT_TOUCHDOWN;
  if (err != hipSuccess) return fail(SHC_ERR_HIP, std::string("hipStreamSynchronize: ") + hipGetErrorString(err));
  if (direct_rc != SHC_OK) return fail(direct_rc, direct_msg + " (the loop was stopped after " + std::to_string(done) + " cycles)");
  if (reason == RESIDENT_EXIT_FAULT || host_load(&r->host->fault) != 0)
    return fail(SHC_ERR_HIP, "resident mode: a wavefront gave up waiting for the relay; restore the engine from a snapshot");
  if (host_load(&r->host->late_reads) != 0)
    return fail(SHC_ERR_TIMEOUT, "resident mode: a stream-ordered read (shc_engine_resident_get_joint_state_async) gave up waiting for its cycle");
  if (!((reason == RESIDENT_EXIT_STOP || reason == RESIDENT_EXIT_MAX) && done == r->published))
    return fail(SHC_ERR_TIMEOUT, std::string("resident mode: the device loop had stopped by itself (") +
                                     (reason == RESIDENT_EXIT_IDLE ? "idle timeout" : reason == RESIDENT_EXIT_MAX ? "max_cycles" : "unknown") + ") after " +
                                     std::to_string(done) + " of " + std::to_string(r->published) + " published cycles");
  return SHC_OK;
}

static int step_k_out_ring(shc_engine *e, int K) {
  const size_t need = size_t(K) * size_t(e->NJ) * size_t(e->n_slots) * 16;
  if (e->k_out && e->k_out_bytes >= need) return SHC_OK;
  if (e->k_out) {
    const int rc = join_side(e);
    if (rc != SHC_OK) return rc;
    HIP_TRY(hipStreamSynchronize(e->stream));
    (void)hipFree(e->k_out);
    e->k_out = nullptr, e->k_out_bytes = 0;
  }
  HIP_TRY(hipMalloc(reinterpret_cast<void **>(&e->k_out), need));
  e->k_out_bytes = need;
  return SHC_OK;
}

__global__ void copy_joint_planes_kernel(double2 *dst, const double2 *src, int64_t count);
static int step_k_serial(shc_engine *e, int K, const shc_cycle_inputs *in) {
  const int64_t n = e->n, slot = int64_t(e->NJ) * e->n_slots;
  for (int k = 0; k < K; ++k) {
    int rc = SHC_OK;
    if (in && in->linear_xy) rc = shc_engine_set_velocity(e, in->linear_xy + k * n * 2, in->angular + k * n, 1);
    if (rc == SHC_OK && in && in->imu_orientation_wxyz) rc = shc_engine_set_imu(e, in->imu_orientation_wxyz + k * n * 4, in->imu_angular_velocity + k * n * 3, 1);
    if (rc == SHC_OK && in && in->tip_force) rc = shc_engine_set_tip_force(e, in->tip_force + k * n * e->L * 3, 1);
    if (rc == SHC_OK && in && in->joint_effort) rc = shc_engine_set_joint_effort(e, in->joint_effort + k * n * e->L * e->NJ, 1);
    if (rc == SHC_OK) rc = shc_engine_step(e, 1);
    if (rc == SHC_OK) rc = join_side(e);
    if (rc != SHC_OK) return rc;
    copy_joint_planes_kernel<<<dim3((unsigned)((slot + 255) / 256)), dim3(256), 0, e->stream>>>(reinterpret_cast<double2 *>(e->k_out) + k * slot,
                                                                                              reinterpret_cast<const double2 *>(e->st.legd), slot);
    HIP_TRY(hipGetLastError());
  }
  e->k_out_cycles = K;
  return SHC_OK;
}

extern "C" int shc_engine_step_k(shc_engine *e, int n_cycles, const shc_cycle_inputs *in) {
  SHC_ENTER(e);
  if (n_cycles < 1 || n_cycles > 4096) return fail(SHC_ERR_INVALID_ARG, "shc_engine_step_k: 1 .. 4096 cycles per launch");
  if (e->starting_up) return fail(SHC_ERR_UNSUPPORTED, "shc_engine_step_k starts from a running engine (finish the start-up first)");
  unsigned mask = 0;
  if (in) {
    if (!in->on_device) return fail(SHC_ERR_INVALID_ARG, "shc_engine_step_k: the K-deep input arrays are device arrays (on_device = 1)");
    if ((in->linear_xy == nullptr) != (in->angular == nullptr)) return fail(SHC_ERR_INVALID_ARG, "linear_xy and angular are given together");
    if ((in->imu_orientation_wxyz == nullptr) != (in->imu_angular_velocity == nullptr)) return fail(SHC_ERR_INVALID_ARG, "the two IMU arrays are given together");
    if (in->pose_translation_velocity || in->pose_rotation_velocity || in->pose_reset_mode)
      return fail(SHC_ERR_UNSUPPORTED, "shc_engine_step_k carries velocity, IMU, tip force and joint effort; give pose inputs / reset modes with their setters before the call (held for the K cycles)");
    if (in->linear_xy) mask |= 1u << RG_VEL;
    if (in->imu_orientation_wxyz) mask |= 1u << RG_IMU;
    if (in->tip_force) mask |= 1u << RG_FORCE;
    if (in->joint_effort) mask |= 1u << RG_EFFORT;
  }
  HIP_TRY(hipSetDevice(e->device));
  const bool split = e->n_waves >= kSplitWaves && !(e->features & SHC_FEAT_SINGLE_STREAM);
  if (!split || ((mask & (1u << RG_EFFORT)) && !(e->rt_flags & RT_EFFORT_LIVE))) {
    const int rc = join_side(e);
    if (rc != SHC_OK) return rc;
  }
  if (mask & (1u << RG_EFFORT)) {
    const int rc = effort_live(e);
    if (rc != SHC_OK) return rc;
  }
  ResidentFit fit;
  {
    const int rc = resident_fit(e, fit);
    if (rc != SHC_OK) return rc;
  }
  if (size_t(e->NJ) * e->n_slots * 16 * size_t(n_cycles) >= (size_t(1) << 31))
    return fail(SHC_ERR_INVALID_ARG, "shc_engine_step_k: cycles x batch - the output ring must stay below 2 GiB (fewer cycles per launch)");
  {
    const int rc = step_k_out_ring(e, n_cycles);
    if (rc != SHC_OK) return rc;
  }
  if (!fit.batch || (e->features & SHC_FEAT_STEP_K_SERIAL)) return step_k_serial(e, n_cycles, in);
  int k0 = 0;
  if (adjust_pending(e)) {
    const int rc = step_k_serial(e, 1, in);
    if (rc != SHC_OK) return rc;
    if (n_cycles == 1) return SHC_OK;
    k0 = 1;
  }
  e->plan_poser_tips_current = false;
  ResidentArgs A{};
  A.kstride[BND_LIN] = e->n * 2, A.kstride[BND_ANG] = e->n, A.kstride[BND_IMUQ] = e->n * 4, A.kstride[BND_IMUW] = e->n * 3;
  A.kstride[BND_FORCE] = e->n * e->L * 3, A.kstride[BND_EFFORT] = e->n * e->L * e->NJ;
  if (in) {
    const auto row = [&](const double *a, int which) { return a ? a + k0 * A.kstride[which] : a; };
    A.bound[0][BND_LIN] = row(in->linear_xy, BND_LIN), A.bound[0][BND_ANG] = row(in->angular, BND_ANG);
    A.bound[0][BND_IMUQ] = row(in->imu_orientation_wxyz, BND_IMUQ), A.bound[0][BND_IMUW] = row(in->imu_angular_velocity, BND_IMUW);
    A.bound[0][BND_FORCE] = row(in->tip_force, BND_FORCE), A.bound[0][BND_EFFORT] = row(in->joint_effort, BND_EFFORT);
  }
  A.out = e->k_out + size_t(k0) * size_t(e->NJ) * e->n_slots * 2;
  A.depth = n_cycles - k0;
  A.max_cycles = unsigned(n_cycles - k0);
  A.batch_cycles = unsigned(n_cycles - k0);
  A.batch_mask = mask;
  A.n_waves = e->n_waves;
  A.idle_ticks = 0, A.ticks_per_ms = 100000;
  A.touchdown_threshold = e->params.touchdown_threshold;
  A.liftoff_threshold = e->params.liftoff_threshold;
  const LaunchGeometry g = launch_geometry(e);
  CycleLaunch a = cycle_launch(e);
  a.block = g.block, a.resident = &A;
  int rc;
  if (!split) {
    a.grid = g.grid(e->n_waves);
    if ((rc = launch_cycle_for(e, a)) != SHC_OK) return rc;
    HIP_TRY(hipGetLastError());
  } else {
    if ((rc = ensure_split_streams(e)) != SHC_OK) return rc;
    HIP_TRY(hipEventRecord(e->ev_main, e->stream));
    for (int h = 0; h < 2; ++h) {
      HIP_TRY(hipStreamWaitEvent(e->half_stream[h], e->ev_main, 0));
      A.batch_wave0 = h ? g.half : 0;
      a.stream = e->half_stream[h];
      a.grid = g.grid(h ? e->n_waves - g.half : g.half);
      if ((rc = launch_cycle_for(e, a)) != SHC_OK) return rc;
      HIP_TRY(hipGetLastError());
    }
    e->main_dirty = false;
    e->side_busy = true;
  }
  e->k_out_cycles = n_cycles;
  if (mask & (1u << RG_FORCE)) e->rt_flags |= RT_TOUCHDOWN;
  return SHC_OK;
}

extern "C" int shc_engine_get_step_k_joint_state(shc_engine *e, int k, double *q, double *qd, int on_device) {
  SHC_ENTER_JOINED(e);
  if (!e->k_out || k < 0 || k >= e->k_out_cycles) return fail(SHC_ERR_INVALID_ARG, "shc_engine_get_step_k_joint_state: cycle 0 .. K - 1 of the latest shc_engine_step_k");
  HIP_TRY(hipSetDevice(e->device));
  const double *slot = e->k_out + size_t(k) * size_t(e->NJ) * e->n_slots * 2;
  const int64_t threads = e->n * e->L;
  for (int which = 0; which < 2; ++which) {
    double *dst = which ? qd : q;
    if (!dst) continue;
    double *d = on_device ? dst : e->d_stage;
    if (!on_device && size_t(threads) * e->NJ * 8 > e->stage_bytes) return fail(SHC_ERR_INVALID_ARG, "staging buffer too small");
    gather_leg_kernel<<<dim3((unsigned)((threads + 63) / 64)), dim3(64), 0, e->stream>>>(d, slot, e->n_slots, e->n, e->L, e->NJ, which ? LEG_FIELD(e, QD) : LEG_FIELD(e, Q));
    HIP_TRY(hipGetLastError());
    if (!on_device) {
      HIP_TRY(hipMemcpyAsync(dst, d, size_t(threads) * e->NJ * 8, hipMemcpyDeviceToHost, e->stream));
      HIP_TRY(hipStreamSynchronize(e->stream));
    }
  }
  return SHC_OK;
}
```

Before: 1.635 billion.

## Move walk velocity front (getLimit, velocity shaping) onto the helper wavefront

When a helper wavefront is present, the velocity-limit lookup and velocity shaping for the walker's cycle move into a new walk_velocity_front routine that runs on the helper in parallel with the walker. The walker precomputes the velocity-independent parts of the stepper (swing and stance nodes, Bezier derivative weights), then waits on a front-done flag before reading the shaped velocity. This takes the command and limit processing off the walker's critical path, at the cost of an extra cross-wave flag handshake. The helper copy uses fma for the bearing rotation and input norm, so its results may differ slightly in the last bits.

```diff
diff --git a/syropod_highlevel_controller_amd/csrc/shc_cycle.hpp b/syropod_highlevel_controller_amd/csrc/shc_cycle.hpp
--- a/syropod_highlevel_controller_amd/csrc/shc_cycle.hpp
+++ b/syropod_highlevel_controller_amd/csrc/shc_cycle.hpp
@@ -306,10 +306,13 @@
   return clampd(double(phase - P.swing_start + 1) / double(P.swing_end - P.swing_start), 0.0, 1.0);
 }
 
+template <bool WRITTEN_OUT = false>
 __device__ __forceinline__ int bearing_bracket(double y, double x) {
   if (x == 0.0 && y == 0.0) return 0;
   constexpr double kC = 0.99996192306417128874, kS = 0.0087265354983739347;
-  double xr = kC * x - kS * y, yr = kS * x + kC * y;
+  double xr, yr;
+  if constexpr (WRITTEN_OUT) xr = fma(kC, x, -(kS * y)), yr = fma(kS, x, kC * y);
+  else xr = kC * x - kS * y, yr = kS * x + kC * y;
   double ax = fabs(xr), ay = fabs(yr);
   bool upper = yr > 0.0 || (yr == 0.0 && xr > 0.0);
   if (upper) return xr > 0.0 ? (ay < ax ? 0 : 1) : (ay > ax ? 2 : 3);
@@ -819,13 +822,31 @@
   out.adm_delta = projection(V3{d[0], d[1], d[2]}, s.tipx);
 }
 
-template <int L, int NJ, unsigned F, bool ADM_HERE, typename IN, bool ODOM_HERE = true, bool POSE_HERE = true, typename POSEWAIT = NoHook>
+template <int L, int NJ, unsigned F>
+__device__ __forceinline__ double walk_velocity_front(const SharedConsts<L, NJ> &C, const CycleParams &P, const RobTile<64 / L> &rb, const Group<L> g, FrontToBack &fb,
+                                                      const double vin_x, const double vin_y, const double win, const double tip_x, const double tip_y,
+                                                      const int walk_state, const bool frozen, double &vx, double &vy, double &vw) {
+  using R = RobotFields;
+#define SHC_FRONT_TIP_X tip_x
+#define SHC_FRONT_TIP_Y tip_y
+#define SHC_FRONT_WRITTEN_OUT true
+#include "shc_walk_front_body.hpp"
+#undef SHC_FRONT_TIP_X
+#undef SHC_FRONT_TIP_Y
+#undef SHC_FRONT_WRITTEN_OUT
+  return lin_norm;
+}
+
+template <int L, int NJ, unsigned F, bool ADM_HERE, typename IN, bool ODOM_HERE = true, bool POSE_HERE = true, bool FRONT_HERE = true, typename POSEWAIT = NoHook,
+          typename FRONTWAIT = NoHook>
 __device__ __forceinline__ void cycle_front(LegRegs<NJ> &s, LegOut &out, const SharedConsts<L, NJ> &C, const RobTile<64 / L> &rb, const Park &pk,
                                             const Group<L> g, int leg, const double *__restrict__ legd, int64_t ns, uint32_t slot, unsigned &dirty,
                                             const bool manual_live, const bool touchdown_detection, double *ext, const ManualRobot *mr, const IN &in,
-                                            FrontToBack &fb, const double *span = nullptr, const POSEWAIT &pose_wait = POSEWAIT()) {
+                                            FrontToBack &fb, const double *span = nullptr, const POSEWAIT &pose_wait = POSEWAIT(),
+                                            const FRONTWAIT &front_wait = FRONTWAIT()) {
   using R = RobotFields;
   using FT = Feat<F>;
+  static_assert(FRONT_HERE || (!POSE_HERE && (F & (F_DYN | F_MLEGS | F_ROUGH | F_TERRAIN)) == 0), "the velocity front can run elsewhere only on the plain feature-exact walker");
   static_assert(POSE_HERE || ((F & F_DYN) == 0 && (F & F_AUTO) == 0 && (F & F_TERRAIN) == 0), "the pose can run elsewhere only without auto posing / terrain paths");
   int zero = 0;
   asm volatile("" : "+v"(zero));
@@ -918,76 +939,20 @@
   }
 
   SHC_PHASE_FENCE();
-  double lim[4] = {0.05, 0.3, 0.02, 0.1};
-  if (!(SHC_DBG(P) & 2)) {
-    double sx = vin_x + win * (-s.tip.y), sy = vin_y + win * s.tip.x;
-    int idx = bearing_bracket(sy, sx);
-    if (__all(idx == fb.limit_bracket)) {
-#pragma unroll
-      for (int k = 0; k < 4; ++k) lim[k] = fb.limit_value[k];
-    } else {
-#pragma unroll
-      for (int k = 0; k < 4; ++k) lim[k] = kUnassigned;
-#pragma unroll
-      for (int j = 0; j < L; ++j) {
-        int ij = g.get(idx, j);
-#pragma unroll
-        for (int k = 0; k < 4; ++k) lim[k] = fmin(lim[k], C.limit[ij][k]);
-      }
-      fb.limit_bracket = idx;
-#pragma unroll
-      for (int k = 0; k < 4; ++k) fb.limit_value[k] = lim[k];
-    }
-  }
-  SHC_PHASE_FENCE();
-  SHC_TICK(5);
-  double vx = rb.get(R::VLIN), vy = rb.get(R::VLIN + 1), vw = rb.get(R::VANG);
-  const double lin_n2 = vin_x * vin_x + vin_y * vin_y;
-  double lin_norm;
-  const int velocity_input_mode = fb.uf.velocity_input_mode;
-  if (velocity_input_mode == 0 && __all(lin_n2 <= 1.0)) lin_norm = lin_n2 != 0.0 ? 0.5 : 0.0;
-  else lin_norm = sqrt(lin_n2);
-  if (!(SHC_DBG(P) & 32)) {
-    double nvx, nvy, nw;
-    if (velocity_input_mode == 0) {
-      double k = 1.0;
-      if (__any(lin_norm > 1.0)) k = lin_norm > 1.0 ? 1.0 / lin_norm : 1.0;
-      const double cx = lin_norm > 1.0 ? vin_x * k : vin_x, cy = lin_norm > 1.0 ? vin_y * k : vin_y;
-      nw = clampd(win, -1.0, 1.0) * lim[1];
-      const double sc = 1.0 - fabs(win);
-      nvx = (cx * lim[0]) * sc;
-      nvy = (cy * lim[0]) * sc;
-    } else {
-      const bool over = lin_norm > lim[0];
-      const double k = lim[0] / lin_norm;
-      const double cx = over ? vin_x * k : vin_x, cy = over ? vin_y * k : vin_y;
-      nw = clampd(win, -lim[1], lim[1]);
-      const double sc = lim[1] != 0.0 ? (1.0 - fabs(nw / lim[1])) : 0.0;
-      nvx = cx * sc;
-      nvy = cy * sc;
-    }
-    if (walk_state == WS_STOPPING) nvx = nvy = nw = 0.0;
-    if (frozen) nvx = vx, nvy = vy, nw = vw;
-    const double ax = nvx - vx, ay = nvy - vy;
-    const double an2 = ax * ax + ay * ay;
-    const double an = __all(an2 == 0.0) ? 0.0 : sqrt(an2);
-    const double cap = lim[2] * P.dt;
-    if (__all(an < cap)) {
-      vx += ax;
-      vy += ay;
-    } else {
-      const double inv = an2 > 0.0 ? an : 1.0;
-      const double sx_ = (ax / inv) * lim[2] * P.dt, sy_ = (ay / inv) * lim[2] * P.dt;
-      vx += an < cap ? ax : sx_;
-      vy += an < cap ? ay : sy_;
-    }
-    const double aa = nw - vw;
-    vw += fabs(aa) < lim[3] * P.dt ? aa : signd(aa) * lim[3] * P.dt;
-    rb.put(R::VLIN, vx);
-    rb.put(R::VLIN + 1, vy);
-    rb.put(R::VANG, vw);
-  }
-  const bool has_cmd = (lin_norm != 0.0) || (win != 0.0);
+  double vx, vy, vw;
+  bool has_cmd;
+  if constexpr (FRONT_HERE) {
+#define SHC_FRONT_TIP_X s.tip.x
+#define SHC_FRONT_TIP_Y s.tip.y
+#define SHC_FRONT_WRITTEN_OUT false
+#include "shc_walk_front_body.hpp"
+#undef SHC_FRONT_TIP_X
+#undef SHC_FRONT_TIP_Y
+#undef SHC_FRONT_WRITTEN_OUT
+    has_cmd = (lin_norm != 0.0) || (win != 0.0);
+  } else {
+    has_cmd = (vin_x * vin_x + vin_y * vin_y != 0.0) || (win != 0.0);
+  }
 
   SHC_PHASE_FENCE();
   SHC_TICK(6);
@@ -1105,7 +1070,7 @@
   if (POSE_HERE || !steady) {
     rword = (rword & ~(3 | (15 << RW_LACP_SHIFT) | (15 << RW_LCFS_SHIFT) | RW_RTDA)) | walk_state | (lacp << RW_LACP_SHIFT) |
             (lcfs << RW_LCFS_SHIFT) | (rtda ? RW_RTDA : 0);
-    rb.puti(R::I_WORD, rword);
+    if (FRONT_HERE) rb.puti(R::I_WORD, rword);
   }
   SHC_TICK(7);
   int my_pm = (s.word >> LW_PM_SHIFT) & 3;
@@ -1152,54 +1117,117 @@
 #else
     const bool straight = (F & F_ROUGH) == 0 && !(SHC_DBG(P) & 4) && force_normal_touchdown == 0;
 #endif
+    if constexpr (!FRONT_HERE) {
+      if (!straight) {
+        front_wait();
+        SHC_TICK(18);
+        vx = rb.get(R::VLIN), vy = rb.get(R::VLIN + 1), vw = rb.get(R::VANG);
+      }
+    }
     if (straight) {
-      const V3 sorg_p = pk.get3(PK_SORG), svel_p = pk.get3(PK_SVEL), torg_p = pk.get3(PK_TORG);
-      const bool swing = my_state == SS_SWING;
-      const bool step_sw = stepping && swing, step_st = stepping && !swing;
-      const V3 sv{vx - vw * s.tip.y, vy + vw * s.tip.x, 0.0};
-      const V3 strd_new = scaled(sv, P.stride_scale);
-      s.strd = sel3(stepping, strd_new, s.strd);
-      V3 pn = rb.get3(R::PNORM);
-      const bool flat_n = pn.x == 0.0 && pn.y == 0.0 && pn.z == 1.0;
-      if (!__all(flat_n)) pn = normalized(pn);
-      const V3 clearance = scaled(pn, P.swing_height);
-      const int it_sw = my_phase - P.swing_start + 1;
-      const bool first_half = it_sw <= P.swing_iterations / 2;
-      const bool first_sw = step_sw && it_sw == 1;
-      const V3 sorg = sel3(first_sw, s.tip, sorg_p), svel = sel3(first_sw, s.tvel, svel_p);
-      pk.put3(PK_SORG, sorg);
-      pk.put3(PK_SVEL, svel);
-      dirty |= first_sw ? unsigned(DIRTY_SWING_ORG) : 0u;
-      V3 mid{(sorg.x + s.targ.x) / 2.0, (sorg.y + s.targ.y) / 2.0, fmax(sorg.z, s.targ.z)};
-      mid = mid + clearance;
-      mid.y += (lc.stance_y > 0.0) ? P.swing_width : -P.swing_width;
-      const V3 sep1 = scaled(svel * 0.25, P.dt_over_swing_dt);
-      const V3 n1_0 = sorg, n1_1 = sorg + sep1, n1_2 = sorg + scaled(sep1, 2.0);
-      const V3 n1_3{(mid.x + n1_2.x) / 2.0, (mid.y + n1_2.y) / 2.0, mid.z};
-      const V3 n1_4 = mid;
-      const V3 fv = scaled(-s.strd, stance_dt * P.inv_dt);
-      const V3 sep2 = scaled(fv * 0.25, P.dt_over_swing_dt);
-      const V3 n2_0 = n1_4, n2_1 = n1_4 - (n1_3 - n1_4), n2_2 = s.targ - scaled(sep2, 2.0), n2_3 = s.targ - sep2, n2_4 = s.targ;
-      const double t_sw = first_half ? P.swing_delta_t * it_sw : P.swing_delta_t * (it_sw - P.swing_iterations / 2);
-      const V3 b0 = sel3(first_half, n1_0, n2_0), b1 = sel3(first_half, n1_1, n2_1), b2 = sel3(first_half, n1_2, n2_2), b3 = sel3(first_half, n1_3, n2_3),
-               b4 = sel3(first_half, n1_4, n2_4);
-      const V3 dpos_sw = scaled(quartic_bezier_dot(b0, b1, b2, b3, b4, t_sw), P.swing_delta_t);
-      int it_st = my_phase + (P.period - mss);
-      if (it_st >= P.period) it_st -= P.period;
-      if (it_st < 0 || it_st >= P.period) it_st = mod_i(it_st, P.period);
-      it_st += 1;
-      const bool first_st = step_st && it_st == 1;
-      const V3 torg = sel3(first_st, s.tip, torg_p);
-      pk.put3(PK_TORG, torg);
-      dirty |= first_st ? unsigned(DIRTY_STANCE_ORG) : 0u;
-      const double stride_scaler = standard ? 1.0 : lc.first_stride_scaler;
-      const V3 sep = scaled((-s.strd) * stride_scaler, 0.25);
-      const double t_st = it_st * stance_dt;
-      const V3 dpos_st = scaled(quartic_bezier_dot(torg, torg + sep, torg + scaled(sep, 2.0), torg + scaled(sep, 3.0), torg + scaled(sep, 4.0), t_st), stance_dt);
-      const V3 dpos = sel3(swing, dpos_sw, dpos_st);
-      const V3 tip_new = s.tip + dpos, tvel_new = dpos * P.inv_dt;
-      s.tip = sel3(stepping, tip_new, s.tip);
-      s.tvel = sel3(stepping, tvel_new, s.tvel);
+      if constexpr (FRONT_HERE) {
+        const V3 sorg_p = pk.get3(PK_SORG), svel_p = pk.get3(PK_SVEL), torg_p = pk.get3(PK_TORG);
+        const bool swing = my_state == SS_SWING;
+        const bool step_sw = stepping && swing, step_st = stepping && !swing;
+        const V3 sv{vx - vw * s.tip.y, vy + vw * s.tip.x, 0.0};
+        const V3 strd_new = scaled(sv, P.stride_scale);
+        s.strd = sel3(stepping, strd_new, s.strd);
+        V3 pn = rb.get3(R::PNORM);
+        const bool flat_n = pn.x == 0.0 && pn.y == 0.0 && pn.z == 1.0;
+        if (!__all(flat_n)) pn = normalized(pn);
+        const V3 clearance = scaled(pn, P.swing_height);
+        const int it_sw = my_phase - P.swing_start + 1;
+        const bool first_half = it_sw <= P.swing_iterations / 2;
+        const bool first_sw = step_sw && it_sw == 1;
+        const V3 sorg = sel3(first_sw, s.tip, sorg_p), svel = sel3(first_sw, s.tvel, svel_p);
+        pk.put3(PK_SORG, sorg);
+        pk.put3(PK_SVEL, svel);
+        dirty |= first_sw ? unsigned(DIRTY_SWING_ORG) : 0u;
+        V3 mid{(sorg.x + s.targ.x) / 2.0, (sorg.y + s.targ.y) / 2.0, fmax(sorg.z, s.targ.z)};
+        mid = mid + clearance;
+        mid.y += (lc.stance_y > 0.0) ? P.swing_width : -P.swing_width;
+        const V3 sep1 = scaled(svel * 0.25, P.dt_over_swing_dt);
+        const V3 n1_0 = sorg, n1_1 = sorg + sep1, n1_2 = sorg + scaled(sep1, 2.0);
+        const V3 n1_3{(mid.x + n1_2.x) / 2.0, (mid.y + n1_2.y) / 2.0, mid.z};
+        const V3 n1_4 = mid;
+        const V3 fv = scaled(-s.strd, stance_dt * P.inv_dt);
+        const V3 sep2 = scaled(fv * 0.25, P.dt_over_swing_dt);
+        const V3 n2_0 = n1_4, n2_1 = n1_4 - (n1_3 - n1_4), n2_2 = s.targ - scaled(sep2, 2.0), n2_3 = s.targ - sep2, n2_4 = s.targ;
+        const double t_sw = first_half ? P.swing_delta_t * it_sw : P.swing_delta_t * (it_sw - P.swing_iterations / 2);
+        const V3 b0 = sel3(first_half, n1_0, n2_0), b1 = sel3(first_half, n1_1, n2_1), b2 = sel3(first_half, n1_2, n2_2), b3 = sel3(first_half, n1_3, n2_3),
+                 b4 = sel3(first_half, n1_4, n2_4);
+        const V3 dpos_sw = scaled(quartic_bezier_dot(b0, b1, b2, b3, b4, t_sw), P.swing_delta_t);
+        int it_st = my_phase + (P.period - mss);
+        if (it_st >= P.period) it_st -= P.period;
+        if (it_st < 0 || it_st >= P.period) it_st = mod_i(it_st, P.period);
+        it_st += 1;
+        const bool first_st = step_st && it_st == 1;
+        const V3 torg = sel3(first_st, s.tip, torg_p);
+        pk.put3(PK_TORG, torg);
+        dirty |= first_st ? unsigned(DIRTY_STANCE_ORG) : 0u;
+        const double stride_scaler = standard ? 1.0 : lc.first_stride_scaler;
+        const V3 sep = scaled((-s.strd) * stride_scaler, 0.25);
+        const double t_st = it_st * stance_dt;
+        const V3 dpos_st = scaled(quartic_bezier_dot(torg, torg + sep, torg + scaled(sep, 2.0), torg + scaled(sep, 3.0), torg + scaled(sep, 4.0), t_st), stance_dt);
+        const V3 dpos = sel3(swing, dpos_sw, dpos_st);
+        const V3 tip_new = s.tip + dpos, tvel_new = dpos * P.inv_dt;
+        s.tip = sel3(stepping, tip_new, s.tip);
+        s.tvel = sel3(stepping, tvel_new, s.tvel);
+      } else {
+        const V3 sorg_p = pk.get3(PK_SORG), svel_p = pk.get3(PK_SVEL), torg_p = pk.get3(PK_TORG);
+        const bool swing = my_state == SS_SWING;
+        const bool step_sw = stepping && swing, step_st = stepping && !swing;
+        V3 pn = rb.get3(R::PNORM);
+        const bool flat_n = pn.x == 0.0 && pn.y == 0.0 && pn.z == 1.0;
+        if (!__all(flat_n)) pn = normalized(pn);
+        const V3 clearance = scaled(pn, P.swing_height);
+        const int it_sw = my_phase - P.swing_start + 1;
+        const bool first_half = it_sw <= P.swing_iterations / 2;
+        const bool first_sw = step_sw && it_sw == 1;
+        const V3 sorg = sel3(first_sw, s.tip, sorg_p), svel = sel3(first_sw, s.tvel, svel_p);
+        pk.put3(PK_SORG, sorg);
+        pk.put3(PK_SVEL, svel);
+        dirty |= first_sw ? unsigned(DIRTY_SWING_ORG) : 0u;
+        V3 mid{(sorg.x + s.targ.x) / 2.0, (sorg.y + s.targ.y) / 2.0, fmax(sorg.z, s.targ.z)};
+        mid = mid + clearance;
+        mid.y += (lc.stance_y > 0.0) ? P.swing_width : -P.swing_width;
+        const V3 sep1 = scaled(svel * 0.25, P.dt_over_swing_dt);
+        const V3 n1_0 = sorg, n1_1 = sorg + sep1, n1_2 = sorg + scaled(sep1, 2.0);
+        const V3 n1_3{(mid.x + n1_2.x) / 2.0, (mid.y + n1_2.y) / 2.0, mid.z};
+        const V3 n1_4 = mid;
+        const V3 n2_0 = n1_4, n2_1 = n1_4 - (n1_3 - n1_4), n2_4 = s.targ;
+        const double t_sw = first_half ? P.swing_delta_t * it_sw : P.swing_delta_t * (it_sw - P.swing_iterations / 2);
+        const BezierDotWeights w_sw = quartic_bezier_dot_weights(t_sw);
+        int it_st = my_phase + (P.period - mss);
+        if (it_st >= P.period) it_st -= P.period;
+        if (it_st < 0 || it_st >= P.period) it_st = mod_i(it_st, P.period);
+        it_st += 1;
+        const bool first_st = step_st && it_st == 1;
+        const V3 torg = sel3(first_st, s.tip, torg_p);
+        pk.put3(PK_TORG, torg);
+        dirty |= first_st ? unsigned(DIRTY_STANCE_ORG) : 0u;
+        const double stride_scaler = standard ? 1.0 : lc.first_stride_scaler;
+        const double t_st = it_st * stance_dt;
+        const BezierDotWeights w_st = quartic_bezier_dot_weights(t_st);
+        front_wait();
+        SHC_TICK(18);
+        vx = rb.get(R::VLIN), vy = rb.get(R::VLIN + 1), vw = rb.get(R::VANG);
+        const V3 sv{vx - vw * s.tip.y, vy + vw * s.tip.x, 0.0};
+        const V3 strd_new = scaled(sv, P.stride_scale);
+        s.strd = sel3(stepping, strd_new, s.strd);
+        const V3 fv = scaled(-s.strd, stance_dt * P.inv_dt);
+        const V3 sep2 = scaled(fv * 0.25, P.dt_over_swing_dt);
+        const V3 n2_2 = s.targ - scaled(sep2, 2.0), n2_3 = s.targ - sep2;
+        const V3 b0 = sel3(first_half, n1_0, n2_0), b1 = sel3(first_half, n1_1, n2_1), b2 = sel3(first_half, n1_2, n2_2), b3 = sel3(first_half, n1_3, n2_3),
+                 b4 = sel3(first_half, n1_4, n2_4);
+        const V3 dpos_sw = scaled(quartic_bezier_dot(b0, b1, b2, b3, b4, w_sw), P.swing_delta_t);
+        const V3 sep = scaled((-s.strd) * stride_scaler, 0.25);
+        const V3 dpos_st = scaled(quartic_bezier_dot(torg, torg + sep, torg + scaled(sep, 2.0), torg + scaled(sep, 3.0), torg + scaled(sep, 4.0), w_st), stance_dt);
+        const V3 dpos = sel3(swing, dpos_sw, dpos_st);
+        const V3 tip_new = s.tip + dpos, tvel_new = dpos * P.inv_dt;
+        s.tip = sel3(stepping, tip_new, s.tip);
+        s.tvel = sel3(stepping, tvel_new, s.tvel);
+      }
     } else if (stepping && !(SHC_DBG(P) & 4)) {
       V3 sv{vx - vw * s.tip.y, vy + vw * s.tip.x, 0.0};
       s.strd = scaled(sv, P.stride_scale);
@@ -1414,6 +1442,12 @@
       fb.odom_run = true;
     }
   }
+  if constexpr (!FRONT_HERE) {
+    if (!steady) {
+      front_wait();
+      rb.puti(R::I_WORD, rword);
+    }
+  }
   if ((F & F_MLEGS) != 0 && mr != nullptr && my_leg_state == LS_MANUAL) {
     const bool primary = leg == mr->primary_leg, secondary = !primary && leg == mr->secondary_leg;
     V3 vin{0, 0, 0}, pin{0, 0, 0};
diff --git a/syropod_highlevel_controller_amd/csrc/shc_cycle_kernel.hpp b/syropod_highlevel_controller_amd/csrc/shc_cycle_kernel.hpp
--- a/syropod_highlevel_controller_amd/csrc/shc_cycle_kernel.hpp
+++ b/syropod_highlevel_controller_amd/csrc/shc_cycle_kernel.hpp
@@ -954,6 +954,8 @@
 struct Resident3Lds : Resident2Lds<L, NJ> {
   int leg_word[2][2][64];
   unsigned back_seen[2];
+  double tip_xy[2][2][2][64];
+  unsigned front_done[2];
 };
 
 template <int L, int NJ, unsigned F, bool HELPER = false>
@@ -977,7 +979,7 @@
   const int lane = threadIdx.x & 63;
   const int wib = __builtin_amdgcn_readfirstlane(threadIdx.x >> 6);
   const int pair = wib & 1;
-  const bool walker = HELPER ? (wib >> 1) == 1 : wib < 2, helper = HELPER && wib >= 4, leader = wib == (HELPER ? 4 : 2);
+  const bool walker = wib < 2, helper = HELPER && wib >= 4, leader = wib == (HELPER ? 4 : 2);
   const int64_t wave = (int64_t(blockIdx.x) - 1) * 2 + pair;
   const bool active = wave < A.n_waves;
   const int64_t rob0 = wave * RPW;
@@ -1023,6 +1025,7 @@
   }
   constexpr bool POSE_SPLIT = (F & (F_DYN | F_AUTO)) == 0;
   if (POSE_SPLIT && walker && lane == 0) X.pose_done[pair] = 0;
+  if constexpr (HELPER) if (walker && lane == 0) X.front_done[pair] = 0;
   __syncthreads();
   const CycleParams &P = C.P;
   Group<L> g{grp * L};
@@ -1056,7 +1059,10 @@
         mb[7 * 64] = pp.x, mb[8 * 64] = pp.y, mb[9 * 64] = pp.z, mb[10 * 64] = pn.x, mb[11 * 64] = pn.y, mb[12 * 64] = pn.z;
       }
     }
-    if constexpr (HELPER) X.leg_word[pair][cycle & 1][lane] = s.word;
+    if constexpr (HELPER) {
+      X.leg_word[pair][cycle & 1][lane] = s.word;
+      X.tip_xy[pair][cycle & 1][0][lane] = s.tip.x, X.tip_xy[pair][cycle & 1][1][lane] = s.tip.y;
+    }
     else X.pose_c[pair][cycle & 1][lane] = walk_plane_control_candidate<L, NJ>(s.word, C, P, swing_c_count_u);
   };
   if (POSE_SPLIT && walker && active) publish_for_pose(0, true);
@@ -1177,6 +1183,37 @@
     if (lane == 0) *const_cast<volatile unsigned *>(&X.pose_done[pair]) = c_front + 1;
     }
   };
+  const auto front_of_cycle = [&](const u64 h0, const u64 h1) __attribute__((always_inline)) {
+    if constexpr (HELPER) {
+      __builtin_amdgcn_s_setprio(3);
+      double vin_x, vin_y, win;
+      if (h0 == u64(c_front) + 1 && (unsigned(h1) & (1u << RG_VEL)) != 0) {
+        const int field = lane / RPW;
+        const int64_t rob = wave * RPW + (lane - field * RPW);
+        double v = 0.0;
+        if (unsigned(h1) & kResidentDirect) {
+          const int set = int((h1 >> 16) & 3);
+          const double *lin = bound_array(A, set, BND_LIN), *ang = bound_array(A, set, BND_ANG);
+          if (lane < 3 * RPW && rob < st.n_robots) v = field < 2 ? ld_agent_f64(lin + rob * 2 + field) : ld_agent_f64(ang + rob);
+        } else {
+          const int pos = int((h1 >> (16 + 8 * RG_VEL)) & 0xff);
+          const double *rec = A.rin + ((int64_t(pos) * A.n_waves + wave) * RIN_COUNT + RIN_VEL) * RPW;
+          if (lane < 3 * RPW) v = ld_agent_f64(rec + lane);
+        }
+        vin_x = __shfl(v, grp), vin_y = __shfl(v, RPW + grp), win = __shfl(v, 2 * RPW + grp);
+      } else {
+        vin_x = rb.get(R::VIN), vin_y = rb.get(R::VIN + 1), win = rb.get(R::WIN);
+      }
+      const int rword = rb.geti(R::I_WORD);
+      const double tip_x = X.tip_xy[pair][c_front & 1][0][lane], tip_y = X.tip_xy[pair][c_front & 1][1][lane];
+      double vx, vy, vw;
+      (void)walk_velocity_front<L, NJ, F>(C, P, rb, g, fb, vin_x, vin_y, win, tip_x, tip_y, rword & 3, false, vx, vy, vw);
+      __builtin_amdgcn_fence(__ATOMIC_RELEASE, "workgroup");
+      __builtin_amdgcn_wave_barrier();
+      if (lane == 0) *const_cast<volatile unsigned *>(&X.front_done[pair]) = c_front + 1;
+      __builtin_amdgcn_s_setprio(0);
+    }
+  };
   const auto odometry_of_cycle = [&](const double *mb) __attribute__((always_inline)) {
     const V3 ov{mb[192], mb[256], mb[320]};
     if (__any(mb[384] != 0.0)) {
@@ -1186,7 +1223,7 @@
       }
     }
   };
-  constexpr int kWalkerThread = HELPER ? 128 : 0, kModelThread = HELPER ? 0 : 128;
+  constexpr int kWalkerThread = 0, kModelThread = 128;
   if (walker) {
     for (;;) {
       SHC_R2_ITER_BEGIN();
@@ -1197,8 +1234,14 @@
         resident_take_inputs<RPW, POSE_SPLIT ? ROBOT_VEL : ROBOT_ALL, false>(A, c_front, h0, h1, wave, lane, tile, tile_i, dirty, held, st.n_robots);
         SHC_TICK(21);
         const PoseWait<RPW> pose_wait{&X.pose_done[pair], c_front + 1, A.ticks_per_ms, &held.fault};
-        cycle_front<L, NJ, F, false, LegInRing<NJ>, false, !POSE_SPLIT>(s, out, C, rb, pk, g, leg, st.legd, ns, slot, dirty, manual_live, false, nullptr, nullptr,
-                                                                        LegInRing<NJ>{}, fb, nullptr, pose_wait);
+        if constexpr (HELPER) {
+          const PoseWait<RPW> front_wait{&X.front_done[pair], c_front + 1, A.ticks_per_ms, &held.fault};
+          cycle_front<L, NJ, F, false, LegInRing<NJ>, false, !POSE_SPLIT, false>(s, out, C, rb, pk, g, leg, st.legd, ns, slot, dirty, manual_live, false, nullptr, nullptr,
+                                                                                 LegInRing<NJ>{}, fb, nullptr, pose_wait, front_wait);
+        } else {
+          cycle_front<L, NJ, F, false, LegInRing<NJ>, false, !POSE_SPLIT>(s, out, C, rb, pk, g, leg, st.legd, ns, slot, dirty, manual_live, false, nullptr, nullptr,
+                                                                          LegInRing<NJ>{}, fb, nullptr, pose_wait);
+        }
 #ifdef SHC_ABLATE
         if (!(P.debug_skip & 65536))
 #endif
@@ -1220,7 +1263,11 @@
       }
       SHC_TICK(23);
       if (kind == IT_EXIT) break;
-      SHC_R2_ITER_END(kWalkerThread, 19, 20, 21, 2, 3, 4, 5, 6, 7, 16, 8, 17, 15, 29, 22, 23);
+      if constexpr (HELPER) {
+        SHC_R2_ITER_END(kWalkerThread, 19, 20, 21, 2, 3, 4, 6, 7, 18, 16, 8, 17, 15, 29, 22, 23);
+      } else {
+        SHC_R2_ITER_END(kWalkerThread, 19, 20, 21, 2, 3, 4, 5, 6, 7, 16, 8, 17, 15, 29, 22, 23);
+      }
       if (kind == IT_REAL) ++c_front;
       prev_real = kind == IT_REAL;
       __syncthreads();
@@ -1237,6 +1284,8 @@
       if (leader && kind != IT_EXIT) leader_decide(kind, nk, nh0v, nh1v);
       if (active) {
         SHC_TICK(24);
+        if (kind == IT_REAL) front_of_cycle(h0, h1);
+        SHC_TICK(1);
         if (kind == IT_REAL) pose_of_cycle(h0, h1);
         SHC_TICK(25);
         if (prev_real) {
@@ -1248,7 +1297,7 @@
       if (leader && kind != IT_EXIT && lane == 0) leader_announce(nk, nh0v, nh1v);
       SHC_TICK(14);
       if (kind == IT_EXIT) break;
-      SHC_R2_ITER_END(256, 19, 29, 24, 30, 25, 26, 14);
+      SHC_R2_ITER_END(256, 19, 29, 24, 1, 30, 25, 26, 14);
       if (kind == IT_REAL) ++c_front;
       prev_real = kind == IT_REAL;
       __syncthreads();
diff --git a/syropod_highlevel_controller_amd/csrc/shc_math.hpp b/syropod_highlevel_controller_amd/csrc/shc_math.hpp
--- a/syropod_highlevel_controller_amd/csrc/shc_math.hpp
+++ b/syropod_highlevel_controller_amd/csrc/shc_math.hpp
@@ -304,6 +304,19 @@
   r = fma3(p3 - p2, 12.0 * s * t * t, r);
   return fma3(p4 - p3, 4.0 * t * t * t, r);
 }
+struct BezierDotWeights {
+  double w0, w1, w2, w3;
+};
+SHC_HD BezierDotWeights quartic_bezier_dot_weights(double t) {
+  double s = 1.0 - t;
+  return BezierDotWeights{4.0 * s * s * s, 12.0 * s * s * t, 12.0 * s * t * t, 4.0 * t * t * t};
+}
+SHC_HD V3 quartic_bezier_dot(V3 p0, V3 p1, V3 p2, V3 p3, V3 p4, const BezierDotWeights &w) {
+  V3 r = (p1 - p0) * w.w0;
+  r = fma3(p2 - p1, w.w1, r);
+  r = fma3(p3 - p2, w.w2, r);
+  return fma3(p4 - p3, w.w3, r);
+}
 
 template <bool EXACT = false>
 SHC_HD double fast_rcp(double x) {
diff --git a/syropod_highlevel_controller_amd/csrc/shc_resident.hpp b/syropod_highlevel_controller_amd/csrc/shc_resident.hpp
--- a/syropod_highlevel_controller_amd/csrc/shc_resident.hpp
+++ b/syropod_highlevel_controller_amd/csrc/shc_resident.hpp
@@ -618,7 +618,11 @@
                            "pose read + updateStance", "control input for the next pose published", "mailbox written", "to the barrier"};
     const double its = c.dbg[1] ? double(c.dbg[1]) : 1.0;
     fprintf(stderr, "[res2 timing] walker of pair 0, mean clocks per phase:\n");
-    for (int i = 0; i < int(sizeof(order) / sizeof(int)); ++i) fprintf(stderr, "[res2 timing]   walker t%-2d %-58s %7.0f\n", order[i], wname[i], double(c.dbg[8 + order[i]]) / its);
+    for (int i = 0; i < int(sizeof(order) / sizeof(int)); ++i) {
+      if (r->helper_wave && order[i] == 5) continue;
+      if (r->helper_wave && order[i] == 16) fprintf(stderr, "[res2 timing]   walker t%-2d %-58s %7.0f\n", 18, "stepper, first half + wait for the front", double(c.dbg[8 + 18]) / its);
+      fprintf(stderr, "[res2 timing]   walker t%-2d %-58s %7.0f\n", order[i], r->helper_wave && order[i] == 6 ? "command predicate" : wname[i], double(c.dbg[8 + order[i]]) / its);
+    }
     const int morder[] = {29, 24, 30, 25, 31, 26, 9, 10, 11, 12, 27, 13, 28, 14};
     const char *mname[] = {"control words (LDS) read", "leader: gate, what the next iteration is, header prefetch issued", "pose inputs of the cycle taken",
                            "updateCurrentPose of the walker's cycle + flag", "leg inputs in force, joint efforts prefetched", "mailbox read, odometry, admittance",
@@ -631,8 +635,8 @@
       fprintf(stderr, "[res2 timing]   model  t%-2d %-58s %7.0f\n", morder[i], mname[i], double(c.dbg[40 + morder[i]]) / mits);
     }
     if (r->helper_wave) {
-      const int horder[] = {29, 24, 30, 25, 26, 14};
-      const char *hname[] = {"control words (LDS) read", "leader: gate, what the next iteration is, header prefetch issued", "pose inputs of the cycle taken",
+      const int horder[] = {29, 24, 1, 30, 25, 26, 14};
+      const char *hname[] = {"control words (LDS) read", "leader: gate, what the next iteration is, header prefetch issued", "front: command, getLimit, velocity shaping + flag", "pose inputs of the cycle taken",
                              "leg words reduced, updateCurrentPose of the walker's cycle + flag", "odometry", "control words written (leader: waits for its loads)"};
       const double hits = c.dbg[73] ? double(c.dbg[73]) : 1.0;
       fprintf(stderr, "[res2 timing] helper wavefront of pair 0 (the leader), mean clocks per phase:\n");
diff --git a/syropod_highlevel_controller_amd/csrc/shc_walk_front_body.hpp b/syropod_highlevel_controller_amd/csrc/shc_walk_front_body.hpp
--- /dev/null
+++ b/syropod_highlevel_controller_amd/csrc/shc_walk_front_body.hpp
@@ -0,0 +1,71 @@
+  double lim[4] = {0.05, 0.3, 0.02, 0.1};
+  if (!(SHC_DBG(P) & 2)) {
+    double sx = vin_x + win * (-SHC_FRONT_TIP_Y), sy = vin_y + win * SHC_FRONT_TIP_X;
+    int idx = bearing_bracket<SHC_FRONT_WRITTEN_OUT>(sy, sx);
+    if (__all(idx == fb.limit_bracket)) {
+#pragma unroll
+      for (int k = 0; k < 4; ++k) lim[k] = fb.limit_value[k];
+    } else {
+#pragma unroll
+      for (int k = 0; k < 4; ++k) lim[k] = kUnassigned;
+#pragma unroll
+      for (int j = 0; j < L; ++j) {
+        int ij = g.get(idx, j);
+#pragma unroll
+        for (int k = 0; k < 4; ++k) lim[k] = fmin(lim[k], C.limit[ij][k]);
+      }
+      fb.limit_bracket = idx;
+#pragma unroll
+      for (int k = 0; k < 4; ++k) fb.limit_value[k] = lim[k];
+    }
+  }
+  SHC_PHASE_FENCE();
+  SHC_TICK(5);
+  vx = rb.get(R::VLIN), vy = rb.get(R::VLIN + 1), vw = rb.get(R::VANG);
+  double lin_n2;
+  if constexpr (SHC_FRONT_WRITTEN_OUT) lin_n2 = fma(vin_x, vin_x, vin_y * vin_y);
+  else lin_n2 = vin_x * vin_x + vin_y * vin_y;
+  double lin_norm;
+  const int velocity_input_mode = fb.uf.velocity_input_mode;
+  if (velocity_input_mode == 0 && __all(lin_n2 <= 1.0)) lin_norm = lin_n2 != 0.0 ? 0.5 : 0.0;
+  else lin_norm = sqrt(lin_n2);
+  if (!(SHC_DBG(P) & 32)) {
+    double nvx, nvy, nw;
+    if (velocity_input_mode == 0) {
+      double k = 1.0;
+      if (__any(lin_norm > 1.0)) k = lin_norm > 1.0 ? 1.0 / lin_norm : 1.0;
+      const double cx = lin_norm > 1.0 ? vin_x * k : vin_x, cy = lin_norm > 1.0 ? vin_y * k : vin_y;
+      nw = clampd(win, -1.0, 1.0) * lim[1];
+      const double sc = 1.0 - fabs(win);
+      nvx = (cx * lim[0]) * sc;
+      nvy = (cy * lim[0]) * sc;
+    } else {
+      const bool over = lin_norm > lim[0];
+      const double k = lim[0] / lin_norm;
+      const double cx = over ? vin_x * k : vin_x, cy = over ? vin_y * k : vin_y;
+      nw = clampd(win, -lim[1], lim[1]);
+      const double sc = lim[1] != 0.0 ? (1.0 - fabs(nw / lim[1])) : 0.0;
+      nvx = cx * sc;
+      nvy = cy * sc;
+    }
+    if (walk_state == WS_STOPPING) nvx = nvy = nw = 0.0;
+    if (frozen) nvx = vx, nvy = vy, nw = vw;
+    const double ax = nvx - vx, ay = nvy - vy;
+    const double an2 = ax * ax + ay * ay;
+    const double an = __all(an2 == 0.0) ? 0.0 : sqrt(an2);
+    const double cap = lim[2] * P.dt;
+    if (__all(an < cap)) {
+      vx += ax;
+      vy += ay;
+    } else {
+      const double inv = an2 > 0.0 ? an : 1.0;
+      const double sx_ = (ax / inv) * lim[2] * P.dt, sy_ = (ay / inv) * lim[2] * P.dt;
+      vx += an < cap ? ax : sx_;
+      vy += an < cap ? ay : sy_;
+    }
+    const double aa = nw - vw;
+    vw += fabs(aa) < lim[3] * P.dt ? aa : signd(aa) * lim[3] * P.dt;
+    rb.put(R::VLIN, vx);
+    rb.put(R::VLIN + 1, vy);
+    rb.put(R::VANG, vw);
+  }
```

Result: faster. 1.773 billion (median of 6 runs) (+8.4%).
